# A-SHOJAEI/adverse-weather-semantic-segmentation-robustness-benchmark

Measured on AMD Instinct MI355X. Metric: images/sec (1024x2048, 5 weather conds, ensemble eval), higher is better.
Workload: dtype f32 (results float32; attention, gemm_1x1, winograd_3x3, segformer_head on 3xf16 split operands: 22-bit operands, f32 accumulate)

## Files before the change

adverse_weather_semantic_segmentation_robustness_benchmark_amd/_native.py:

```python
from __future__ import annotations

import ctypes as C
from pathlib import Path

import numpy as np
import torch

_PKG = Path(__file__).resolve().parent
LIB_PATH = _PKG / "libawseg_hip.so"

U8, I64 = 0, 1
COMBINE_WEIGHTED, COMBINE_MAXCONF, COMBINE_MEAN = 0, 1, 2
LOSS_CE, LOSS_FOCAL = 0, 1
ACT_NONE, ACT_RELU, ACT_GELU = 0, 1, 2
MAX_CLASSES = 32

c_i, c_i64, c_u64, c_f, c_d, c_p = C.c_int, C.c_int64, C.c_uint64, C.c_float, C.c_double, C.c_void_p

FOG_JOB = np.dtype([("image", "<i4"), ("_pad", "<i4"), ("beta", "<f8"), ("atmos", "<f8"), ("seed", "<u8")], align=True)
NIGHT_JOB = np.dtype([("image", "<i4"), ("_pad", "<i4"), ("brightness", "<f8"), ("intensity", "<f8"), ("seed", "<u8")], align=True)
PRIM_JOB = np.dtype([("image", "<i4"), ("prim_offset", "<i4"), ("prim_count", "<i4"), ("blur_ksize", "<i4"), ("intensity", "<f8")], align=True)
WEATHER_JOB = np.dtype([("kind", "<i4"), ("image", "<i4"), ("a", "<f8"), ("b", "<f8"), ("seed", "<u8"), ("prim_offset", "<i4"), ("prim_count", "<i4")], align=True)
WEATHER_CLEAN, WEATHER_FOG, WEATHER_RAIN, WEATHER_SNOW, WEATHER_NIGHT = 0, 1, 2, 3, 4
assert FOG_JOB.itemsize == 32 and NIGHT_JOB.itemsize == 32 and PRIM_JOB.itemsize == 24 and WEATHER_JOB.itemsize == 40

SIGNATURES = {
    "awseg_abi_version": (c_i, []),
    "awseg_header_hash": (C.c_uint64, []),
    "awseg_error_string": (C.c_char_p, [c_i]),
    "awseg_device_count": (c_i, []),
    "awseg_metrics_workspace": (c_i64, [c_i64, c_i, c_i64]),
    "awseg_confusion_accumulate": (c_i, [c_p, c_i, c_p, c_i, c_i64, c_i, c_i, c_i, c_p, c_p, c_p, c_p]),
    "awseg_argmax": (c_i, [c_p, c_i64, c_i, c_i64, c_p, c_i, c_p]),
    "awseg_combine_argmax_confusion": (c_i, [c_p, c_p, c_i64, c_i, c_i64, c_i, c_p, c_p, c_p, c_p, c_i, c_p, c_i, c_i,
                                            c_i, c_p, c_p, c_i, c_p, c_p, c_p]),
    "awseg_argmax_confusion": (c_i, [c_p, c_i64, c_i, c_i64, c_p, c_i, c_p, c_i, c_i, c_i, c_p, c_p, c_i, c_p, c_p, c_p]),
    "awseg_normalize": (c_i, [c_p, c_i64, c_i, c_i, c_p, c_i, c_p, c_p, c_p, c_p]),
    "awseg_synthetic_depth": (c_i, [c_i, c_i, c_p, c_i, c_p, c_p, c_p, c_p]),
    "awseg_conv3x3_winograd_nhwc": (c_i, [c_p, c_i, c_i, c_i, c_i, c_i, c_i, c_p, c_p, c_p, c_i, c_p, c_p, c_p, c_p]),
    "awseg_gemm_bias_act": (c_i, [c_p, c_p, c_p, c_p, c_i, c_p, c_i64, c_i, c_i, c_p, C.c_size_t, c_p]),
    "awseg_gemm_tune": (c_i, [c_p, c_p, c_p, c_i, c_i, c_p, c_i64, c_i, c_i, c_p, C.c_size_t, c_p]),
    "awseg_gemm_split_weights": (c_i, [c_p, c_i, c_i, c_p, c_p]),
    "awseg_gemm_split_weight_halfs": (c_i64, [c_i, c_i]),
    "awseg_gemm_split_bias_act": (c_i, [c_p, c_p, c_p, c_p, c_i, c_p, c_i64, c_i, c_i, c_p]),
    "awseg_gemm_bf16_weights": (c_i, [c_p, c_i, c_i, c_p, c_p]),
    "awseg_gemm_bf16_weight_halfs": (c_i64, [c_i, c_i]),
    "awseg_gemm_bf16_bias_act": (c_i, [c_p, c_p, c_p, c_p, c_i, c_p, c_i64, c_i, c_i, c_p]),
    "awseg_conv3x3_winograd_bf16_nhwc": (c_i, [c_p, c_i, c_i, c_i, c_i, c_i, c_i, c_p, c_p, c_p, c_i, c_p, c_p, c_p, c_p]),
    "awseg_attention_d32_bf16": (c_i, [c_p, c_p, c_p, c_p, c_i, c_i, c_i, c_i, c_f, c_p]),
    "awseg_attention_d32_split_workspace": (c_i64, [c_i, c_i, c_i]),
    "awseg_attention_d32_split_ws": (c_i, [c_p, c_p, c_p, c_i, c_p, c_i, c_i, c_i, c_i, c_f, c_p, c_p]),
    "awseg_attention_d32_packed_kv": (c_i, [c_p, c_p, c_p, c_i, c_i, c_i, c_i, c_f, c_i, c_p]),
    "awseg_dwconv3x3_upcat_nhwc": (c_i, [c_p, c_i, c_i, c_i, c_p, c_i, c_i64, c_i, c_i, c_p, c_p, c_p]),
    "awseg_winograd_split_weight_halfs": (c_i64, [c_i, c_i]),
    "awseg_conv3x3_winograd_split_nhwc": (c_i, [c_p, c_i, c_i, c_i, c_i, c_i, c_i, c_p, c_p, c_p, c_i, c_p, c_p, c_p, c_p]),
    "awseg_upconv_forms_floats": (c_i64, [c_i, c_i, c_i]),
    "awseg_upconv_forms": (c_i, [c_p, c_i, c_i, c_i, c_i, c_p, c_p, c_p]),
    "awseg_depth_head_fused": (c_i, [c_p, c_i, c_i, c_i, c_i, c_p, c_i, c_p, c_p, c_p, c_p, c_p]),
    "awseg_im2col_nhwc": (c_i, [c_p, c_i64, c_i, c_i, c_i, c_i, c_i, c_i, c_i, c_i, c_i, c_p, c_p]),
    "awseg_attention_d32": (c_i, [c_p, c_p, c_p, c_p, c_i, c_i, c_i, c_i, c_f, c_p]),
    "awseg_attention_d32_split": (c_i, [c_p, c_p, c_p, c_p, c_i, c_i, c_i, c_i, c_f, c_p]),
    "awseg_depth_upsample_combine": (c_i, [c_p, c_p, c_i, c_i, c_i, c_i, c_i, c_p, c_p, c_p, c_p]),
    "awseg_lut3_apply": (c_i, [c_p, c_i, c_i, c_i, c_p, c_i, c_p, c_p, c_p]),
    "awseg_local_contrast": (c_i, [c_p, c_i, c_i, c_i, c_p, c_p]),
    "awseg_depth_estimate_workspace": (C.c_size_t, [c_i]),
    "awseg_depth_estimate": (c_i, [c_p, c_i, c_i, c_i, c_p, c_p, c_p, c_p, c_p]),
    "awseg_fog_apply": (c_i, [c_p, c_i, c_i, c_p, c_i, c_p, c_p, c_p, c_p, c_p, c_p]),
    "awseg_fog_fused": (c_i, [c_p, c_i, c_i, c_p, c_i, c_p, c_p, c_p, c_p, c_p, c_p, c_p, c_p]),
    "awseg_night_apply": (c_i, [c_p, c_i, c_i, c_p, c_i, c_p, c_p, c_p, c_p, c_p, c_p, c_p]),
    "awseg_rain_apply": (c_i, [c_p, c_i, c_i, c_p, c_i, c_p, c_p, c_p, c_p, c_p, c_p, c_p]),
    "awseg_snow_apply": (c_i, [c_p, c_i, c_i, c_p, c_i, c_p, c_p, c_p, c_p, c_p, c_p, c_p]),
    "awseg_weather_batch": (c_i, [c_p, c_i, c_i, c_p, c_i, c_p, c_p, c_p, c_p, c_p, c_p, c_p, c_p, c_p, c_p]),
    "awseg_streak_workspace": (c_i64, [c_i, c_i, c_i]),
    "awseg_fog_density_field": (c_i, [c_p, c_i, c_i64, c_u64, c_p, c_p, c_p]),
    "awseg_loss_partials": (c_i64, [c_i64, c_i64]),
    "awseg_fog_ce_forward": (c_i, [c_p, c_p, c_i, c_p, c_i64, c_i, c_i64, c_i, c_f, c_p, c_p, c_p, c_p, c_p]),
    "awseg_fog_ce_backward": (c_i, [c_p, c_p, c_i, c_p, c_i64, c_i, c_i64, c_i, c_f, c_p, c_p, c_p]),
    "awseg_density_workspace": (c_i64, [c_i64, c_i64]),
    "awseg_fog_density_from_depth": (c_i, [c_p, c_i64, c_i, c_i, c_p, c_p, c_p]),
    "awseg_segformer_head_fused": (c_i, [c_p, c_i64, c_i, c_i, c_i, c_i, c_i, c_p, c_p, c_p, c_p, c_i, c_p, c_p]),
    "awseg_segformer_head_fused_split": (c_i, [c_p, c_i64, c_i, c_i, c_i, c_i, c_i, c_p, c_p, c_p, c_p, c_i, c_p, c_p]),
    "awseg_upconv3x3_bn_relu": (c_i, [c_p, c_i64, c_i, c_i, c_i, c_i, c_i, c_p, c_p, c_p, c_i, c_p]),
    "awseg_upconv3x3_linear": (c_i, [c_p, c_i64, c_i, c_i, c_i, c_i, c_i, c_p, c_p, c_i, c_p]),
    "awseg_upconv3x3_adjoint": (c_i, [c_p, c_i64, c_i, c_i, c_i, c_i, c_i, c_p, c_p]),
    "awseg_aspp_depthwise3": (c_i, [c_p, c_i64, c_i, c_i, c_i, c_p, c_i, c_i, c_i, c_p, c_p]),
    "awseg_aspp_depthwise3_mean": (c_i, [c_p, c_i64, c_i, c_i, c_i, c_p, c_i, c_i, c_i, c_p, c_p, c_p]),
    "awseg_dwconv3x3_nhwc": (c_i, [c_p, c_i64, c_i, c_i, c_i, c_i, c_p, c_p, c_i, c_p, c_p]),
    "awseg_bias_act_nhwc": (c_i, [c_p, c_i64, c_i, c_p, c_p, c_i, c_p]),
    "awseg_layernorm_rows": (c_i, [c_p, c_i64, c_i, c_p, c_p, c_f, c_p, c_p]),
    "awseg_ensemble_eval_stats": (c_i, [c_p, c_p, c_i64, c_i, c_i64, c_i, c_p, c_p, c_p, c_i, c_p, c_p, c_i, c_p, c_i, c_p, c_i,
                                       c_f, c_f, c_p, c_p]),
    "awseg_gemm_split_pieces_bias_act": (c_i, [c_p, c_i, c_i, c_p, c_p, c_p, c_i, c_p, c_i64, c_i, c_p]),
    "awseg_gemm_split_dual_bias_act": (c_i, [c_p, c_i, c_p, c_i, c_i64, c_i, c_i, c_i, c_p, c_p, c_p, c_i, c_p, c_i64, c_i, c_p]),
    "awseg_conv_gemm_split_bias_act": (c_i, [c_p, c_i64, c_i, c_i, c_i, c_i, c_i, c_i, c_i, c_i, c_p, c_p, c_p, c_i, c_p, c_i, c_p]),
    "awseg_conv_rows_gemm_split_bias_act": (c_i, [c_p, c_i64, c_i, c_i, c_i, c_i, c_i, c_i, c_i, c_p, c_p, c_p, c_i, c_p, c_i, c_p]),
    "awseg_bn_train_workspace": (c_i64, [c_i, c_i, c_i64]),
    "awseg_bn_train_stats": (c_i, [c_p, c_i, c_i, c_i64, c_p, c_p, c_p, c_p]),
    "awseg_bn_relu_dropout_forward": (c_i, [c_p, c_i, c_i, c_i64, c_p, c_p, c_p, c_p, c_p, c_p, c_p]),
    "awseg_bn_relu_dropout_backward": (c_i, [c_p, c_p, c_i, c_i, c_i64, c_p, c_p, c_p, c_p, c_p, c_p, c_p, c_p, c_p, c_i, c_p]),
    "awseg_dwconv3x3_wgrad_workspace": (c_i64, [c_i64, c_i, c_i, c_i]),
    "awseg_dwconv3x3_wgrad_nhwc": (c_i, [c_p, c_p, c_i64, c_i, c_i, c_i, c_i, c_p, c_p, c_p, c_p]),
    "awseg_mixffn_fused": (c_i, [c_p, c_i, c_i, c_i, c_i, c_p, c_p, c_f, c_p, c_i, c_p, c_p, c_p, c_p, c_i, c_p, c_p, c_p, c_p]),
    "awseg_maxpool3x3s2_nhwc": (c_i, [c_p, c_i64, c_i, c_i, c_i, c_p, c_p]),
    "awseg_maxpool3x3s2_bias_relu_nhwc": (c_i, [c_p, c_i64, c_i, c_i, c_i, c_p, c_p, c_p]),
    "awseg_upsample_bilinear": (c_i, [c_p, c_i64, c_i, c_i, c_i, c_i, c_i, c_p, c_p]),
    "awseg_stem_image": (c_i, [c_p, c_i, c_i, c_i, c_i, c_i64, c_i64, c_i64, c_p, c_i, c_p]),
    "awseg_rowdot_sigmoid": (c_i, [c_p, c_i64, c_i, c_p, c_p, c_i, c_p, c_p]),
    "awseg_aspp_pool_branch_workspace": (c_i64, [c_i, c_i]),
    "awseg_aspp_pool_branch": (c_i, [c_p, c_i, c_i, c_p, c_p, c_i, c_p, c_p, c_i, c_p, c_p, c_p]),
    "awseg_upsample_bilinear_strided": (c_i, [c_p, c_i64, c_i, c_i, c_i, c_i64, c_i64, c_i64, c_i64, c_i, c_i, c_i, c_p, c_p]),
    "awseg_combine_confusion_stats": (c_i, [c_p, c_p, c_i64, c_i, c_i64, c_i, c_p, c_p, c_p, c_i, c_i, c_i, c_p, c_p, c_i, c_p, c_p, c_i,
                                           c_p, c_i, c_p, c_i, c_f, c_f, c_p, c_p]),
    "awseg_combine_confusion_stats_pred": (c_i, [c_p, c_p, c_i64, c_i, c_i64, c_i, c_p, c_p, c_p, c_i, c_i, c_i, c_p, c_p, c_i, c_p, c_p,
                                                c_i, c_p, c_i, c_p, c_i, c_f, c_f, c_p, c_p, c_p]),
    "awseg_consistency_workspace": (c_i64, [c_i64, c_i, c_i64]),
    "awseg_prediction_consistency": (c_i, [c_p, c_p, c_i, c_i64, c_i64, c_p, c_p, c_i, c_i, c_i, c_p, c_p, c_i, c_p, c_p, c_p]),
    "awseg_ece_accumulate": (c_i, [c_p, c_i64, c_i, c_i64, c_p, c_i, c_p, c_p, c_i, c_p, c_i, c_p, c_p]),
    "awseg_temperature_grid_stats": (c_i, [c_p, c_i64, c_i, c_i64, c_p, c_i, c_p, c_p, c_i, c_p, c_i, c_p, c_i, c_p]),
    "awseg_ensemble_temperature_grid_stats": (c_i, [c_p, c_p, c_i64, c_i, c_i64, c_i, c_p, c_p, c_p, c_i, c_p, c_p, c_i, c_p, c_i,
                                                   c_p, c_i, c_p]),
    "awseg_ensemble_weight_grid_stats": (c_i, [c_p, c_p, c_i64, c_i, c_i64, c_p, c_i, c_p, c_i, c_i, c_p, c_p, c_i, c_p]),
    "awseg_depth_eval_stats": (c_i, [c_p, c_p, c_i, c_i, c_i, c_i, c_i, c_p, c_p, c_f, c_p, c_p, c_i, c_p]),
    "awseg_ensemble_failure_stats": (c_i, [c_p, c_p, c_p, c_i64, c_i, c_i64, c_i, c_p, c_p, c_p, c_i, c_p, c_p, c_i, c_p]),
    "awseg_failure_stats": (c_i, [c_p, c_i64, c_i, c_i64, c_p, c_i, c_p, c_p, c_i, c_p]),
    "awseg_boundary_workspace": (c_i64, [c_i64, c_i, c_i, c_i, c_i]),
    "awseg_boundary_stats": (c_i, [c_p, c_p, c_i, c_i, c_i64, c_i, c_i, c_i, c_p, c_i, c_p, c_p, c_i, c_p, c_p, c_p]),
    "awseg_segment_workspace": (c_i64, [c_i64, c_i, c_i]),
    "awseg_segment_stats": (c_i, [c_p, c_p, c_i, c_i, c_i64, c_i, c_i, c_i, c_p, c_i, c_p, c_p, c_p, c_i, c_p, c_p, c_p, c_p, c_p]),
    "awseg_frame_iou_workspace": (c_i64, [c_i64, c_i, c_i64]),
    "awseg_frame_iou_counts": (c_i, [c_p, c_p, c_i, c_i, c_i64, c_i64, c_i, c_p, c_p, c_i64, c_p, c_p, c_p]),
    "awseg_bootstrap_counts": (c_i, [c_p, c_p, c_i64, c_i64, c_i64, c_i64, c_u64, c_i64, c_i64, c_p, c_p, c_p]),
    "awseg_change_strata": (c_i, [c_p, c_p, c_i, c_i64, c_i, c_i64, c_p, c_p, c_p, c_i, c_p, c_p, c_p]),
    "awseg_strata_workspace": (c_i64, [c_i64, c_i, c_i64, c_i]),
    "awseg_stratified_stats": (c_i, [c_p, c_p, c_i, c_i, c_p, c_i, c_p, c_i, c_p, c_i64, c_i64, c_i, c_p, c_p, c_i, c_p, c_p, c_p]),
    "awseg_image_quality_workspace": (c_i64, [c_i64, c_i, c_i64, c_i64]),
    "awseg_image_quality": (c_i, [c_p, c_p, c_i, c_i64, c_i, c_i64, c_i64, c_p, c_p, c_p, c_p, c_f, c_f, c_p, c_p, c_i, c_p, c_p, c_p]),
}


class AwsegError(RuntimeError):
    pass


_lib = None


def lib() -> C.CDLL:
    global _lib
    if _lib is None:
        if not LIB_PATH.exists():
            raise AwsegError(
                f"{LIB_PATH} is missing: build it with `python -m "
                "adverse_weather_semantic_segmentation_robustness_benchmark_amd.csrc.build` "
                "(there is no CPU fallback for the HIP hot path)")
        handle = C.CDLL(str(LIB_PATH))
        for name, (res, args) in SIGNATURES.items():
            fn = getattr(handle, name)
            fn.restype, fn.argtypes = res, args
        header = LIB_PATH.parent.parent / "include" / "awseg.h"
        built = int(handle.awseg_header_hash())
        if built and header.exists():
            from .csrc.build import header_hash
            if built != header_hash():
                raise AwsegError(f"{LIB_PATH} was built from another include/awseg.h than the one beside it (ABI drift): rebuild it with "
                                 "`python -m adverse_weather_semantic_segmentation_robustness_benchmark_amd.csrc.build`")
        _lib = handle
    return _lib


def check(rc: int, what: str) -> None:
    if rc != 0:
        msg = lib().awseg_error_string(rc)
        raise AwsegError(f"{what} failed with code {rc}: {msg.decode() if msg else '?'}")


launch_hook = None


# ... 69 lines not shown
```

adverse_weather_semantic_segmentation_robustness_benchmark_amd/csrc/attn.hip:

```cpp
#include "awseg_common.h"

namespace {

typedef float f32x16 __attribute__((ext_vector_type(16)));

constexpr int AT = 256;
#ifndef AWSEG_ATTN_SPLIT_WAVES
#define AWSEG_ATTN_SPLIT_WAVES 2
#endif
constexpr int D = 32;
constexpr int TK = 32;
constexpr int LDK = 36;

__device__ __forceinline__ constexpr int acc_row(int r, int hk) { return (r & 3) + 8 * (r >> 2) + 4 * hk; }

__global__ __launch_bounds__(AT, 2)
void attention_d32_kernel(const float* __restrict__ q, const float* __restrict__ k, const float* __restrict__ v,
                          float* __restrict__ out, int nq, int nkv, int heads, float scale_log2e, int kvp)
{
    __shared__ float sK[2][TK * LDK];
    __shared__ float sV[2][D * LDK];
    const int tid = threadIdx.x, lane = tid & 63, wave = tid >> 6;
    const int hk = lane >> 5, li = lane & 31;
    const int h = blockIdx.y, b = blockIdx.z;
// ... 307 lines not shown
        split8_unscaled(p + 8, ph1, pl1);
        om = __builtin_amdgcn_mfma_f32_32x32x16_f16(vh0, ph0, om, 0, 0, 0);
        oc = __builtin_amdgcn_mfma_f32_32x32x16_f16(vl0, ph0, oc, 0, 0, 0);
        om = __builtin_amdgcn_mfma_f32_32x32x16_f16(vh1, ph1, om, 0, 0, 0);
        oc = __builtin_amdgcn_mfma_f32_32x32x16_f16(vl1, ph1, oc, 0, 0, 0);
        om = __builtin_amdgcn_mfma_f32_32x32x16_f16(vh0, pl0, om, 0, 0, 0);
        om = __builtin_amdgcn_mfma_f32_32x32x16_f16(vh1, pl1, om, 0, 0, 0);
        if (t + 1 < ntiles) {
            stage(buf ^ 1, kreg, vreg);
            if (t + 2 < ntiles) {
                kreg = *reinterpret_cast<const float4*>(kb + (size_t)(t + 2) * TK * kvp + g_off);
                vreg = *reinterpret_cast<const float4*>(vb + (size_t)(t + 2) * TK * kvp + g_off);
            }
        }
        __syncthreads();
    }

    if (!SCALED && !BF16) {
        if (qmax >= kSplitLimit) atomicMax(&sMax[0], __builtin_bit_cast(unsigned, qmax));
        if (kmax >= kSplitLimit) atomicMax(&sMax[1], __builtin_bit_cast(unsigned, kmax));
        if (vmax >= kSplitLimit) atomicMax(&sMax[2], __builtin_bit_cast(unsigned, vmax));
        __syncthreads();
        if ((sMax[0] | sMax[1] | sMax[2]) != 0u) return true;
    }
    const int qi = q0 + li;
    if (qi < nq) {
        const float inv = 1.0f / l_run;
        float* op = out + ((size_t)b * nq + qi) * C + h * D;
#pragma unroll
        for (int g = 0; g < 4; ++g) {
            float4 o4 = make_float4(fmaf(oc[4 * g], kLoInv, om[4 * g]) * inv, fmaf(oc[4 * g + 1], kLoInv, om[4 * g + 1]) * inv,
                                    fmaf(oc[4 * g + 2], kLoInv, om[4 * g + 2]) * inv, fmaf(oc[4 * g + 3], kLoInv, om[4 * g + 3]) * inv);
            if (SCALED) { o4.x *= sc.bv; o4.y *= sc.bv; o4.z *= sc.bv; o4.w *= sc.bv; }
            *reinterpret_cast<float4*>(op + 8 * g + 4 * hk) = o4;
        }
    }
    return false;
}

__device__ __forceinline__ int guard_exponent(unsigned maxbits)
{
    const int ex = (int)(maxbits >> 23) & 0xff;
    if (maxbits == 0u || ex == 0xff) return 0;
    return ex - 127 - 13;
}

__global__ __launch_bounds__(AT, AWSEG_ATTN_SPLIT_WAVES)
void attention_d32_split_kernel(const float* __restrict__ q, const float* __restrict__ k, const float* __restrict__ v,
                                float* __restrict__ out, int nq, int nkv, int heads, float scale_log2e, int kvp)
{
    __shared__ __attribute__((aligned(16))) _Float16 sK[2][TK * SROW];
    __shared__ __attribute__((aligned(16))) _Float16 sV[2][D * SROW];
    __shared__ unsigned sMax[3];
    if (threadIdx.x < 3) sMax[threadIdx.x] = 0u;
    const attn_scales one = {1.f, 1.f, 1.f, 1.f, 1.f, 1.f};
    if (!attn_split_pass<false>(q, k, v, out, nq, nkv, heads, scale_log2e, kvp, sK, sV, sMax, one)) return;
    const int eq = guard_exponent(sMax[0]), ek = guard_exponent(sMax[1]), ev = guard_exponent(sMax[2]);
    auto p2 = [](int e) { return __builtin_bit_cast(float, (unsigned)(127 + e) << 23); };
    const attn_scales sc = {p2(-eq), p2(-ek), p2(-ev), p2(eq), p2(ek), p2(ev)};
    attn_split_pass<true>(q, k, v, out, nq, nkv, heads, scale_log2e, kvp, sK, sV, sMax, sc);
}

constexpr int IMG_TILE_HALFS = (TK + D) * SROW;

__device__ __forceinline__ uint32_t at_lds_addr(const void* p) { return (uint32_t)(uintptr_t)(__attribute__((address_space(3))) const void*)p; }
__device__ __forceinline__ void at_dma16(__amdgpu_buffer_rsrc_t rsrc, uint32_t voff, uint32_t soff, uint32_t lds_base)
{
    asm volatile("s_mov_b32 m0, %3\n\ts_nop 0\n\tbuffer_load_dwordx4 %0, %1, %2 offen lds" : : "v"(voff), "s"(rsrc), "s"(soff), "s"(lds_base) : "m0", "memory");
}

__global__ __launch_bounds__(AT)
void attn_kv_image_kernel(const float* __restrict__ k, const float* __restrict__ v, int kvp, int nkv, int heads,
                          _Float16* __restrict__ img, int* __restrict__ exps)
{
    __shared__ unsigned sM[2];
    const int tid = threadIdx.x, h = blockIdx.x, b = blockIdx.y;
    const float* kb = k + (size_t)b * nkv * kvp + h * D;
    const float* vb = v + (size_t)b * nkv * kvp + h * D;
    const int lkey = tid >> 3, lc = tid & 7;
    const size_t g_off = (size_t)lkey * kvp + 4 * lc;
    const int wk0 = lkey * SROW + 4 * lc;
    const int wv0 = TK * SROW + (4 * lc) * SROW + pv_slot(lkey);
    const int ntiles = nkv / TK;
    if (tid < 2) sM[tid] = 0u;
    __syncthreads();
    float kmax = 0.f, vmax = 0.f;
    for (int t = 0; t < ntiles; ++t) {
        kmax = amax4(kmax, *reinterpret_cast<const float4*>(kb + (size_t)t * TK * kvp + g_off));
        vmax = amax4(vmax, *reinterpret_cast<const float4*>(vb + (size_t)t * TK * kvp + g_off));
    }
    if (kmax >= kSplitLimit) atomicMax(&sM[0], __builtin_bit_cast(unsigned, kmax));
    if (vmax >= kSplitLimit) atomicMax(&sM[1], __builtin_bit_cast(unsigned, vmax));
    __syncthreads();
    const int ek = guard_exponent(sM[0]), ev = guard_exponent(sM[1]);
    auto p2 = [](int e) { return __builtin_bit_cast(float, (unsigned)(127 + e) << 23); };
    const float sk = p2(-ek), sv = p2(-ev);
    if (tid == 0) { exps[((size_t)b * heads + h) * 2] = ek; exps[((size_t)b * heads + h) * 2 + 1] = ev; }
    _Float16* base = img + ((size_t)b * heads + h) * ntiles * IMG_TILE_HALFS;
    for (int t = 0; t < ntiles; ++t) {
        float4 kk4 = *reinterpret_cast<const float4*>(kb + (size_t)t * TK * kvp + g_off);
        float4 vv4 = *reinterpret_cast<const float4*>(vb + (size_t)t * TK * kvp + g_off);
        kk4.x *= sk; kk4.y *= sk; kk4.z *= sk; kk4.w *= sk;
        vv4.x *= sv; vv4.y *= sv; vv4.z *= sv; vv4.w *= sv;
        _Float16* T = base + (size_t)t * IMG_TILE_HALFS;
        u32x2 H, L; unsigned hh, ll;
        split_pair(kk4.x, kk4.y, hh, ll); H[0] = hh; L[0] = ll;
        split_pair(kk4.z, kk4.w, hh, ll); H[1] = hh; L[1] = ll;
        *reinterpret_cast<u32x2*>(&T[wk0]) = H;
        *reinterpret_cast<u32x2*>(&T[wk0 + 32]) = L;
        unsigned vh01, vl01, vh23, vl23;
        split_pair(vv4.x, vv4.y, vh01, vl01);
        split_pair(vv4.z, vv4.w, vh23, vl23);
        unsigned short* sv16 = reinterpret_cast<unsigned short*>(&T[wv0]);
        sv16[0] = (unsigned short)vh01;            sv16[32] = (unsigned short)vl01;
        sv16[SROW] = (unsigned short)(vh01 >> 16); sv16[SROW + 32] = (unsigned short)(vl01 >> 16);
        sv16[2 * SROW] = (unsigned short)vh23;     sv16[2 * SROW + 32] = (unsigned short)vl23;
        sv16[3 * SROW] = (unsigned short)(vh23 >> 16); sv16[3 * SROW + 32] = (unsigned short)(vl23 >> 16);
    }
}

template <bool SCALED, bool QGUARD>
__device__ __forceinline__ bool attn_split_pass_img(const float* __restrict__ q, const _Float16* __restrict__ img_bh, float* __restrict__ out,
                                                    int nq, int nkv, int heads, float scale_log2e, _Float16 (*sKV)[IMG_TILE_HALFS],
                                                    unsigned* sMax, const attn_scales sc)
{
    const int tid = threadIdx.x, lane = tid & 63, wave = tid >> 6;
    const int hk = lane >> 5, li = lane & 31;
    const int h = blockIdx.y, b = blockIdx.z;
    const int C = heads * D;
    const int q0 = blockIdx.x * 128 + wave * 32;
    float qmax = 0.f;
    h8 qh[2], ql[2];
    {
        const int qi = q0 + li;
        const float* qp = q + ((size_t)b * nq + (qi < nq ? qi : nq - 1)) * C + h * D;
        const float qs = SCALED ? scale_log2e * sc.sq : scale_log2e;
#pragma unroll
        for (int s = 0; s < 2; ++s) {
            const float4 a4 = *reinterpret_cast<const float4*>(qp + 16 * s + 8 * hk);
            const float4 b4 = *reinterpret_cast<const float4*>(qp + 16 * s + 8 * hk + 4);
            const float x[8] = { a4.x * qs, a4.y * qs, a4.z * qs, a4.w * qs, b4.x * qs, b4.y * qs, b4.z * qs, b4.w * qs };
            if (QGUARD) {
#pragma unroll
                for (int i = 0; i < 8; ++i) qmax = __builtin_fmaxf(qmax, __builtin_fabsf(x[i]));
            }
            split8(x, qh[s], ql[s]);
        }
    }
    const int ntiles = nkv / TK;
    const __amdgpu_buffer_rsrc_t rsrc = __builtin_amdgcn_make_buffer_rsrc((void*)img_bh, 0, ntiles * IMG_TILE_HALFS * 2, 0x00020000);
    const uint32_t lds0 = __builtin_amdgcn_readfirstlane(at_lds_addr(&sKV[0][0]));
    const uint32_t wave_u = __builtin_amdgcn_readfirstlane(wave);
    auto dma_tile = [&](int t, int buf) {
        const uint32_t so = (uint32_t)t * (uint32_t)(IMG_TILE_HALFS * 2), lb = lds0 + (uint32_t)buf * (uint32_t)(IMG_TILE_HALFS * 2);
        at_dma16(rsrc, (uint32_t)(lane * 16) + wave_u * 1024u, so, lb + wave_u * 1024u);
        at_dma16(rsrc, (uint32_t)(lane * 16) + (wave_u + 4u) * 1024u, so, lb + (wave_u + 4u) * 1024u);
        if (wave_u == 0) at_dma16(rsrc, (uint32_t)(lane * 16) + 8192u, so, lb + 8192u);
    };
    dma_tile(0, 0);
    asm volatile("s_waitcnt vmcnt(0)" ::: "memory");
    __syncthreads();

    f32x16 om, oc;
#pragma unroll
    for (int r = 0; r < 16; ++r) { om[r] = 0.f; oc[r] = 0.f; }
    float m_run = -1e30f, l_run = 0.f;
    const int a_off = li * SROW + 8 * hk;

    for (int t = 0; t < ntiles; ++t) {
        const int buf = t & 1;
        if (t + 1 < ntiles) dma_tile(t + 1, buf ^ 1);
        const h8* kr = reinterpret_cast<const h8*>(&sKV[buf][a_off]);
        const h8 kh0 = kr[0], kh1 = kr[2], kl0 = kr[4], kl1 = kr[6];
        f32x16 sm, scx;
#pragma unroll
        for (int r = 0; r < 16; ++r) { sm[r] = 0.f; scx[r] = 0.f; }
        sm = __builtin_amdgcn_mfma_f32_32x32x16_f16(kh0, qh[0], sm, 0, 0, 0);
        scx = __builtin_amdgcn_mfma_f32_32x32x16_f16(kh0, ql[0], scx, 0, 0, 0);
        sm = __builtin_amdgcn_mfma_f32_32x32x16_f16(kh1, qh[1], sm, 0, 0, 0);
        scx = __builtin_amdgcn_mfma_f32_32x32x16_f16(kh1, ql[1], scx, 0, 0, 0);
        scx = __builtin_amdgcn_mfma_f32_32x32x16_f16(kl0, qh[0], scx, 0, 0, 0);
        scx = __builtin_amdgcn_mfma_f32_32x32x16_f16(kl1, qh[1], scx, 0, 0, 0);
// ... 55 lines not shown
    return false;
}

__global__ __launch_bounds__(AT, AWSEG_ATTN_SPLIT_WAVES)
void attention_d32_split_img_kernel(const float* __restrict__ q, const _Float16* __restrict__ img, const int* __restrict__ exps,
                                    float* __restrict__ out, int nq, int nkv, int heads, float scale_log2e)
{
    __shared__ __attribute__((aligned(16))) _Float16 sKV[2][IMG_TILE_HALFS];
    __shared__ unsigned sMax[1];
    const int h = blockIdx.y, b = blockIdx.z;
    if (threadIdx.x == 0) sMax[0] = 0u;
    const _Float16* img_bh = img + ((size_t)b * heads + h) * (size_t)(nkv / TK) * IMG_TILE_HALFS;
    const int ek = exps[((size_t)b * heads + h) * 2], ev = exps[((size_t)b * heads + h) * 2 + 1];
    auto p2 = [](int e) { return __builtin_bit_cast(float, (unsigned)(127 + e) << 23); };
    attn_scales sc = {1.f, p2(-ek), p2(-ev), 1.f, p2(ek), p2(ev)};
    bool redo;
    if ((ek | ev) == 0) redo = attn_split_pass_img<false, true>(q, img_bh, out, nq, nkv, heads, scale_log2e, sKV, sMax, sc);
    else redo = attn_split_pass_img<true, true>(q, img_bh, out, nq, nkv, heads, scale_log2e, sKV, sMax, sc);
    if (!redo) return;
    const int eq = guard_exponent(sMax[0]);
    sc.sq = p2(-eq); sc.bq = p2(eq);
    __syncthreads();
    attn_split_pass_img<true, false>(q, img_bh, out, nq, nkv, heads, scale_log2e, sKV, sMax, sc);
}

__global__ __launch_bounds__(AT, 2)
void attention_d32_bf16_kernel(const float* __restrict__ q, const float* __restrict__ k, const float* __restrict__ v,
                               float* __restrict__ out, int nq, int nkv, int heads, float scale_log2e, int kvp)
{
    __shared__ __attribute__((aligned(16))) _Float16 sK[2][TK * SROW];
    __shared__ __attribute__((aligned(16))) _Float16 sV[2][D * SROW];
    __shared__ unsigned sMax[3];
    const attn_scales one = {1.f, 1.f, 1.f, 1.f, 1.f, 1.f};
    attn_split_pass<false, true>(q, k, v, out, nq, nkv, heads, scale_log2e, kvp, sK, sV, sMax, one);
}

}

namespace {
template <typename K>
int launch_attention(K kernel, const float* q, const float* k, const float* v, float* out, int batch, int heads,
                     int n_queries, int n_keys, float scale, awseg_stream_t stream, int kv_pitch = 0)
{
    if (batch == 0 || n_queries == 0) return 0;
    if (!q || !k || !v || !out || batch < 0 || heads < 1 || n_queries < 0 || n_keys < TK) return AWSEG_EINVAL;
    if (n_keys % TK) return AWSEG_ERANGE;
    if (heads > 65535 || batch > 65535) return AWSEG_ERANGE;
    if (((uintptr_t)q & 15) || ((uintptr_t)k & 15) || ((uintptr_t)v & 15) || ((uintptr_t)out & 15)) return AWSEG_EALIGN;
    if (kv_pitch == 0) kv_pitch = heads * D;
    if (kv_pitch < heads * D || (kv_pitch & 3)) return AWSEG_EINVAL;
    dim3 grid((unsigned)((n_queries + 127) / 128), (unsigned)heads, (unsigned)batch);
    hipLaunchKernelGGL(kernel, grid, dim3(AT), 0, awseg_s(stream), q, k, v, out, n_queries, n_keys, heads,
                       scale * 1.4426950408889634f, kv_pitch);
    AWSEG_LAUNCH_CHECK();
    return 0;
}
}

AWSEG_API int awseg_attention_d32(const float* q, const float* k, const float* v, float* out, int batch, int heads,
                                  int n_queries, int n_keys, float scale, awseg_stream_t stream)
{
    return launch_attention(attention_d32_kernel, q, k, v, out, batch, heads, n_queries, n_keys, scale, stream);
}

AWSEG_API int awseg_attention_d32_split(const float* q, const float* k, const float* v, float* out, int batch, int heads,
                                        int n_queries, int n_keys, float scale, awseg_stream_t stream)
{
    return launch_attention(attention_d32_split_kernel, q, k, v, out, batch, heads, n_queries, n_keys, scale, stream);
}

AWSEG_API int awseg_attention_d32_bf16(const float* q, const float* k, const float* v, float* out, int batch, int heads,
                                       int n_queries, int n_keys, float scale, awseg_stream_t stream)
{
    return launch_attention(attention_d32_bf16_kernel, q, k, v, out, batch, heads, n_queries, n_keys, scale, stream);
}

AWSEG_API int64_t awseg_attention_d32_split_workspace(int batch, int heads, int n_keys)
{
    if (batch < 0 || heads < 0 || n_keys < 0) return 0;
    const int64_t tab = ((int64_t)batch * heads * 2 * 4 + 255) / 256 * 256;
    return tab + (int64_t)batch * heads * (n_keys / TK) * IMG_TILE_HALFS * 2;
}

AWSEG_API int awseg_attention_d32_split_ws(const float* q, const float* k, const float* v, int kv_pitch, float* out, int batch, int heads,
                                           int n_queries, int n_keys, float scale, void* workspace, awseg_stream_t stream)
{
    if (batch == 0 || n_queries == 0) return 0;
    if (!q || !k || !v || !out || !workspace || batch < 0 || heads < 1 || n_queries < 0 || n_keys < TK) return AWSEG_EINVAL;
    if (n_keys % TK) return AWSEG_ERANGE;
    if (heads > 65535 || batch > 65535) return AWSEG_ERANGE;
    if (((uintptr_t)q & 15) || ((uintptr_t)k & 15) || ((uintptr_t)v & 15) || ((uintptr_t)out & 15) || ((uintptr_t)workspace & 255)) return AWSEG_EALIGN;
    if (kv_pitch == 0) kv_pitch = heads * D;
    if (kv_pitch < heads * D || (kv_pitch & 3)) return AWSEG_EINVAL;
    if ((int64_t)(n_keys / TK) * IMG_TILE_HALFS * 2 > 0x7fffffff) return AWSEG_ERANGE;
    int* exps = reinterpret_cast<int*>(workspace);
    const int64_t tab = ((int64_t)batch * heads * 2 * 4 + 255) / 256 * 256;
    _Float16* img = reinterpret_cast<_Float16*>(reinterpret_cast<char*>(workspace) + tab);
    hipLaunchKernelGGL(attn_kv_image_kernel, dim3((unsigned)heads, (unsigned)batch), dim3(AT), 0, awseg_s(stream), k, v, kv_pitch, n_keys, heads, img, exps);
    AWSEG_LAUNCH_CHECK();
    dim3 grid((unsigned)((n_queries + 127) / 128), (unsigned)heads, (unsigned)batch);
    hipLaunchKernelGGL(attention_d32_split_img_kernel, grid, dim3(AT), 0, awseg_s(stream), q, img, exps, out, n_queries, n_keys, heads,
                       scale * 1.4426950408889634f);
    AWSEG_LAUNCH_CHECK();
    return 0;
}

AWSEG_API int awseg_attention_d32_packed_kv(const float* q, const float* kv, float* out, int batch, int heads, int n_queries,
                                            int n_keys, float scale, int mode, awseg_stream_t stream)
{
    if (!kv) return AWSEG_EINVAL;
    const int c = heads * D;
    switch (mode) {
    case 0: return launch_attention(attention_d32_kernel, q, kv, kv + c, out, batch, heads, n_queries, n_keys, scale, stream, 2 * c);
    case 1: return launch_attention(attention_d32_split_kernel, q, kv, kv + c, out, batch, heads, n_queries, n_keys, scale, stream, 2 * c);
    case 2: return launch_attention(attention_d32_bf16_kernel, q, kv, kv + c, out, batch, heads, n_queries, n_keys, scale, stream, 2 * c);
    default: return AWSEG_EINVAL;
    }
}
```

adverse_weather_semantic_segmentation_robustness_benchmark_amd/csrc/awseg_common.h:

```cpp
#pragma once
#include <hip/hip_runtime.h>
#include <stdint.h>
#include <atomic>
#include <type_traits>
#include "../../include/awseg.h"

#define AWSEG_API extern "C" __attribute__((visibility("default")))

#define AWSEG_WAVE 64
#define AWSEG_CUS 256

#define AWSEG_LAUNCH_CHECK()                                  \
    do {                                                      \
        hipError_t e__ = hipGetLastError();                   \
        if (e__ != hipSuccess) return (int)e__;               \
    } while (0)

static inline hipStream_t awseg_s(awseg_stream_t s) { return (hipStream_t)s; }

inline int awseg_cu_count()
{
    static std::atomic<int> cached[16];
    int dev = 0, n_cu = 0;
    if (hipGetDevice(&dev) != hipSuccess) return AWSEG_CUS;
// ... 48 lines not shown

__device__ __forceinline__ void awseg_amax_step(float v, int c, float& best, int& bi)
{
    if (!(v <= best) && !(best != best)) { best = v; bi = c; }
}

__device__ __forceinline__ unsigned long long awseg_conf_q30(float conf) { return (unsigned long long)(conf * 1073741824.0f); }

__device__ __forceinline__ int awseg_ece_find_bin(float conf, const float* s_edges, int n_bins)
{
    int b = (int)ceilf(conf * (float)n_bins) - 1;
    b = b < 0 ? 0 : (b > n_bins - 1 ? n_bins - 1 : b);
    if (!(conf > s_edges[b])) b = b > 0 ? b - 1 : 0;
    else if (!(conf <= s_edges[b + 1])) b = b < n_bins - 1 ? b + 1 : b;
    if (conf > s_edges[b] && conf <= s_edges[b + 1]) return b;
    for (int k = 0; k < n_bins; ++k)
        if (conf > s_edges[k] && conf <= s_edges[k + 1]) return k;
    return -1;
}

inline int awseg_blocks_per_image(int64_t lane_items, int threads, int64_t batch, int resident_per_cu)
{
    int64_t want = (lane_items + threads - 1) / threads;
    int64_t cap = (AWSEG_CUS * resident_per_cu + batch - 1) / batch;
    if (cap < 1) cap = 1;
    if (want > cap) want = cap;
    if (want < 1) want = 1;
    return (int)want;
}

template <typename F> inline auto awseg_by_label(int label_dtype, F&& f)
{
    if (label_dtype == AWSEG_U8) return f(std::integral_constant<int, AWSEG_U8>());
    return f(std::integral_constant<int, AWSEG_I64>());
}
template <typename F> inline auto awseg_by_flag(bool flag, F&& f)
{
    if (flag) return f(std::true_type());
    return f(std::false_type());
}
template <typename F> inline auto awseg_by_combine_mode(int mode, F&& f)
{
    if (mode == AWSEG_COMBINE_WEIGHTED) return f(std::integral_constant<int, 0>());
    return f(std::integral_constant<int, 2>());
}

struct awseg_philox {
    __device__ __forceinline__ static void gen(uint64_t seed, uint64_t ctr, uint32_t stream, uint32_t out[4])
    {
        const uint32_t M0 = 0xD2511F53u, M1 = 0xCD9E8D57u;
        uint32_t c0 = (uint32_t)ctr, c1 = (uint32_t)(ctr >> 32), c2 = stream, c3 = 0x9E3779B9u;
        uint32_t k0 = (uint32_t)seed, k1 = (uint32_t)(seed >> 32);
#pragma unroll
        for (int r = 0; r < 7; ++r) {
            uint32_t hi0 = __umulhi(M0, c0), lo0 = M0 * c0;
            uint32_t hi1 = __umulhi(M1, c2), lo1 = M1 * c2;
            uint32_t n0 = hi1 ^ c1 ^ k0, n2 = hi0 ^ c3 ^ k1;
            c0 = n0; c1 = lo1; c2 = n2; c3 = lo0;
            k0 += 0x9E3779B9u; k1 += 0xBB67AE85u;
        }
        out[0] = c0; out[1] = c1; out[2] = c2; out[3] = c3;
    }
};
__device__ __forceinline__ void awseg_box_muller(uint32_t a, uint32_t b, float& n0, float& n1)
{
    float u1 = ((float)(a >> 8) + 0.5f) * (1.0f / 16777216.0f);
    float u2 = (float)(b >> 8) * (1.0f / 16777216.0f);
    float r = __builtin_amdgcn_sqrtf(-1.38629436111989061883f * __builtin_amdgcn_logf(u1));
    n0 = r * __builtin_amdgcn_cosf(u2);
    n1 = r * __builtin_amdgcn_sinf(u2);
}
__device__ __forceinline__ void awseg_box_muller16(uint32_t a, float& n0, float& n1)
{
    float u1 = ((float)(a & 0xFFFFu) + 0.5f) * (1.0f / 65536.0f);
    float u2 = (float)(a >> 16) * (1.0f / 65536.0f);
    float r = __builtin_amdgcn_sqrtf(-1.38629436111989061883f * __builtin_amdgcn_logf(u1));
    n0 = r * __builtin_amdgcn_cosf(u2);
    n1 = r * __builtin_amdgcn_sinf(u2);
}
__device__ __forceinline__ float awseg_u01(uint32_t a) { return (float)(a >> 8) * (1.0f / 16777216.0f); }

int awseg_gemm_split3_weights(const float* w, int n, int k, uint16_t* w3, const unsigned* trailer, hipStream_t stream);
bool awseg_gemm_split3_eligible(int64_t m, int n, int k, const void* x, const void* out, const void* residual, const void* bias);
struct awseg_g3_dual { const float* x2; int k1; int h, w, stride, ho, wo; int64_t bytes; const float* x3 = nullptr; const float* x4 = nullptr; };
int awseg_gemm_split3_launch(const float* x, const uint16_t* w3, const unsigned* trailer, const float* bias, const float* residual,
                             int act, float* out, int64_t m, int n, int k, int cus, hipStream_t stream, const int* conv = nullptr,
                             bool bf16 = false, const awseg_g3_dual* dual = nullptr);
int awseg_gemm_split3_bn(int n);
int64_t awseg_gemm_split3_image_rows(int n);
int awseg_gemm_bf16_3_weights(const float* w, int n, int k, uint16_t* w3, hipStream_t stream);
```

adverse_weather_semantic_segmentation_robustness_benchmark_amd/csrc/gemm_split.hip:

```cpp
#include "awseg_common.h"

namespace {

typedef float f32x16 __attribute__((ext_vector_type(16)));
typedef _Float16 h8 __attribute__((ext_vector_type(8)));
typedef _Float16 h2 __attribute__((ext_vector_type(2)));
typedef unsigned u32x2 __attribute__((ext_vector_type(2)));
typedef unsigned u32x4 __attribute__((ext_vector_type(4)));

constexpr int GT = 512;
constexpr int SWT = 256;
constexpr int GKT = 32;
constexpr int GROW = 72;
constexpr float kLoScale = 2048.0f, kLoInv = 1.0f / 2048.0f;

__device__ __forceinline__ void split_pair(float a, float b, unsigned& hi, unsigned& lo)
{
    const auto hp = __builtin_amdgcn_cvt_pkrtz(a, b);
    const h2 hh = __builtin_bit_cast(h2, hp);
    const float ra = (a - (float)hh.x) * kLoScale, rb = (b - (float)hh.y) * kLoScale;
    hi = __builtin_bit_cast(unsigned, hp);
    lo = __builtin_bit_cast(unsigned, __builtin_amdgcn_cvt_pkrtz(ra, rb));
}

// ... 296 lines not shown
        const bool rescale = oe != 0;

        {
            const int64_t tile_off = m0 * a.N + n0;
            const int64_t rem = ((int64_t)a.M * a.N - tile_off) * 4;
            const int nrec = rem > 0x7fffffff ? 0x7fffffff : (int)rem;
            const __amdgpu_buffer_rsrc_t o_rsrc = __builtin_amdgcn_make_buffer_rsrc((void*)(a.out + tile_off), 0, nrec, 0x00020000);
            const __amdgpu_buffer_rsrc_t r_rsrc = __builtin_amdgcn_make_buffer_rsrc((void*)((a.residual ? a.residual : a.out) + tile_off), 0, nrec, 0x00020000);
            const bool has_res = a.residual != nullptr;
            const bool ragged = m0 + BM > a.M;
            const int mleft = ragged ? (int)(a.M - m0) : BM;
            const int vrow = (wm * 32 * MT + 4 * hk) * a.N;
#pragma unroll
            for (int j = 0; j < NT; ++j) {
                const int nl = wn * 32 * NT + j * 32 + li;
                const bool n_ok = n0 + nl < a.N;
                const float bv = (a.bias && n_ok) ? a.bias[n0 + nl] : 0.f;
                const int voff = n_ok ? (vrow + nl) * 4 : (int)0x80000000;
#pragma unroll
                for (int i = 0; i < MT; ++i) {
#pragma unroll
                    for (int half = 0; half < 2; ++half) {
                        float rv[8]; int vo[8], so[8];
#pragma unroll
                        for (int r8 = 0; r8 < 8; ++r8) {
                            const int r = 8 * half + r8;
                            const int rowc = i * 32 + (r & 3) + 8 * (r >> 2);
                            if (ragged) {
                                vo[r8] = (wm * 32 * MT + 4 * hk + rowc < mleft) ? voff + rowc * a.N * 4 : (int)0x80000000;
                                so[r8] = 0;
                            } else { vo[r8] = voff; so[r8] = rowc * a.N * 4; }
                            rv[r8] = has_res ? __builtin_bit_cast(float, __builtin_amdgcn_raw_buffer_load_b32(r_rsrc, vo[r8], so[r8], 0)) : 0.f;
                        }
#pragma unroll
                        for (int r8 = 0; r8 < 8; ++r8) {
                            const int r = 8 * half + r8;
                            float vv = fmaf(ac2[i][j][r], kLoInv, am[i][j][r]);
                            if (rescale) vv = vv * os1 * os2;
                            vv = vv + bv + rv[r8];
                            if (a.act == 1) vv = fmaxf(vv, 0.f);
                            __builtin_amdgcn_raw_buffer_store_b32(__builtin_bit_cast(uint32_t, vv), o_rsrc, vo[r8], so[r8], 0);
                        }
                    }
                }
            }
        }
        if (!has_next) break;
        slot = nslot; m0 = nm0; n0 = nn0;
        scaled = false; sx = 1.0f; xe = 0;
    }
}

}

AWSEG_API int awseg_gemm_split_weights(const float* w, int n, int k, uint16_t* w_split, awseg_stream_t stream)
{
    if (n == 0 || k == 0) return 0;
    if (!w || !w_split || n < 0 || k < 0) return AWSEG_EINVAL;
    const int64_t ne = (int64_t)n * k;
    const int64_t blocks = (ne / 2 + SWT) / SWT;
    unsigned* trailer = reinterpret_cast<unsigned*>(w_split + 2 * ne);
    if ((uintptr_t)trailer & 3) return AWSEG_EALIGN;
    hipError_t e = hipMemsetAsync(trailer, 0, 16, awseg_s(stream));
    if (e != hipSuccess) return (int)e;
    const int64_t rb = (ne + SWT - 1) / SWT;
    hipLaunchKernelGGL(weights_absmax_kernel, dim3((unsigned)(rb < 1024 ? rb : 1024)), dim3(SWT), 0, awseg_s(stream), w, ne, trailer);
    AWSEG_LAUNCH_CHECK();
    hipLaunchKernelGGL(split_weights_kernel, dim3((unsigned)blocks), dim3(SWT), 0, awseg_s(stream), w, ne, w_split, trailer);
    AWSEG_LAUNCH_CHECK();
    if (awseg_gemm_split3_bn(n) && k % 8 == 0) return awseg_gemm_split3_weights(w, n, k, w_split + 2 * ne + 8, trailer, awseg_s(stream));
    return 0;
}

AWSEG_API int64_t awseg_gemm_split_weight_halfs(int n, int k)
{
    if (n < 1 || k < 1) return -1;
    const int64_t ne = (int64_t)n * k;
    return 2 * ne + 8 + ((awseg_gemm_split3_bn(n) && k % 8 == 0) ? 2 * awseg_gemm_split3_image_rows(n) * ((k + 31) / 32 * 32) : 0);
}

namespace {
struct conv_desc { int H, W, C, Ho, Wo, kw, stride, pad, dil; int64_t batch; int pitch = 0, padx = -1; };

int gemm_launch(bool bf16, const float* x, const uint16_t* w_split, const float* bias, const float* residual,
                int act, float* out, int64_t m, int n, int k, awseg_stream_t stream, const conv_desc* cv = nullptr)
{
    if (m == 0 || n == 0) return 0;
    if (!x || !w_split || !out || m < 0 || n < 0 || k < 8 || act < 0 || act > 1) return AWSEG_EINVAL;
    if (k % 8) return AWSEG_ERANGE;
    if (((uintptr_t)x & 15) || ((uintptr_t)w_split & 15)) return AWSEG_EALIGN;
    gemm_args a;
    a.x = x; a.wh = reinterpret_cast<const _Float16*>(w_split); a.wl = a.wh + (int64_t)n * k;
    a.trailer = reinterpret_cast<const unsigned*>(w_split + 2 * (int64_t)n * k);
    a.bias = bias; a.residual = residual; a.out = out; a.M = m; a.N = n; a.K = k; a.act = act;
    a.conv = cv ? 1 : 0;
    if (cv) { a.cH = cv->H; a.cW = cv->W; a.cC = cv->C; a.cHo = cv->Ho; a.cWo = cv->Wo; a.ckw = cv->kw; a.cs = cv->stride; a.cp = cv->pad; a.cd = cv->dil; }
    else { a.cH = a.cW = a.cC = a.cHo = a.cWo = a.ckw = a.cs = 1; a.cp = 0; a.cd = 1; }
    const int cus = awseg_cu_count();
    if (awseg_gemm_split3_eligible(m, n, k, cv ? nullptr : x, out, residual, bias) && !(bf16 && (cv || n % 256)) &&
        (!cv || (cv->C % 32 == 0 && (int64_t)cv->batch * cv->H * cv->W * (cv->pitch > 0 ? cv->pitch : cv->C) * 4 <= 0x7fffffff)) &&
        (((m + 255) / 256) * (int64_t)((n + awseg_gemm_split3_bn(n) - 1) / awseg_gemm_split3_bn(n)) >= (int64_t)cus / 2 ||
         (!bf16 && ((m + 127) / 128) * (int64_t)((n + 127) / 128) >= (int64_t)cus / 2))) {
        const int cdesc[12] = { cv ? cv->H : 0, cv ? cv->W : 0, cv ? cv->C : 0, cv ? cv->Ho : 0, cv ? cv->Wo : 0, cv ? cv->kw : 0,
                                cv ? cv->stride : 0, cv ? cv->pad : 0, cv ? cv->dil : 0, cv ? (int)cv->batch : 0, cv ? cv->pitch : 0, cv ? cv->padx : -1 };
        return awseg_gemm_split3_launch(x, w_split + 2 * (int64_t)n * k + 8, a.trailer, bias, residual, act, out, m, n, k, cus, awseg_s(stream),
                                        cv ? cdesc : nullptr, bf16);
    }
    if (cv && cv->pitch > 0) return AWSEG_ERANGE;
    const bool wide = n % 256 == 0 && ((m + 127) / 128) * (int64_t)(n / 256) >= cus;
    const int bn = wide ? 256 : 128, bm = 128;
    const int64_t ntm = (m + bm - 1) / bm;
    a.ntn = (n + bn - 1) / bn;
    const int64_t ntm8 = (ntm + 7) / 8 * 8;
    if (ntm8 * a.ntn > 0x7fffffff || (int64_t)bm * n > 0x7fffffff) return AWSEG_ERANGE;
    a.ntm = (int)ntm; a.ntm8 = (int)ntm8;
    const int64_t slots = ntm8 * a.ntn;
    int64_t blocks = (int64_t)cus * (wide ? 1 : 2) / 8 * 8;
    if (blocks < 8) blocks = 8;
    if (blocks > slots) blocks = slots;
    const dim3 grid((unsigned)blocks), block(GT);
#define GEMM_GO(MT_, NT_, WM_, WN_)                                                                                    \
    do {                                                                                                              \
        if (bf16) {                                                                                                   \
            if (k % GKT) hipLaunchKernelGGL((gemm_split_kernel<MT_, NT_, WM_, WN_, true, true>), grid, block, 0, awseg_s(stream), a);   \
            else hipLaunchKernelGGL((gemm_split_kernel<MT_, NT_, WM_, WN_, false, true>), grid, block, 0, awseg_s(stream), a);         \
        } else {                                                                                                      \
            if (k % GKT) hipLaunchKernelGGL((gemm_split_kernel<MT_, NT_, WM_, WN_, true, false>), grid, block, 0, awseg_s(stream), a);  \
            else hipLaunchKernelGGL((gemm_split_kernel<MT_, NT_, WM_, WN_, false, false>), grid, block, 0, awseg_s(stream), a);        \
        }                                                                                                             \
    } while (0)
    if (wide) GEMM_GO(2, 2, 2, 4); else GEMM_GO(1, 2, 4, 2);
#undef GEMM_GO
    AWSEG_LAUNCH_CHECK();
    return 0;
}

__global__ __launch_bounds__(SWT)
void bf16_weights_kernel(const float* __restrict__ w, int64_t n_elems, uint16_t* __restrict__ out, unsigned* __restrict__ trailer)
{
    if (blockIdx.x == 0 && threadIdx.x == 0) { trailer[0] = 0u; trailer[1] = 0u; trailer[2] = 0u; trailer[3] = 0u; }
    const int64_t i = ((int64_t)blockIdx.x * SWT + threadIdx.x) * 2;
    if (i >= n_elems) return;
    const unsigned p = pack_bf16(w[i], (i + 1 < n_elems) ? w[i + 1] : 0.f);
    out[i] = (uint16_t)p;
    if (i + 1 < n_elems) out[i + 1] = (uint16_t)(p >> 16);
}
}

AWSEG_API int awseg_gemm_split_bias_act(const float* x, const uint16_t* w_split, const float* bias, const float* residual,
                                        int act, float* out, int64_t m, int n, int k, awseg_stream_t stream)
{
    return gemm_launch(false, x, w_split, bias, residual, act, out, m, n, k, stream);
}

AWSEG_API int awseg_gemm_split_dual_bias_act(const float* x, int k1, const float* x2, int k2, int64_t batch, int x2_height, int x2_width,
                                             int x2_stride, const uint16_t* w_split, const float* bias, const float* residual, int act,
                                             float* out, int64_t m, int n, awseg_stream_t stream)
{
    if (m == 0 || n == 0) return 0;
    if (!x || !x2 || !w_split || !out || m < 0 || n < 0 || k1 < 32 || k2 < 32 || act < 0 || act > 1 || x2_stride < 0) return AWSEG_EINVAL;
    if (k1 % 32 || k2 % 32) return AWSEG_ERANGE;
    if (((uintptr_t)x & 15) || ((uintptr_t)x2 & 15) || ((uintptr_t)w_split & 15)) return AWSEG_EALIGN;
    const int k = k1 + k2;
    if (!awseg_gemm_split3_eligible(m, n, k, x, out, residual, bias)) return AWSEG_ERANGE;
    awseg_g3_dual d;
    d.x2 = x2; d.k1 = k1; d.stride = x2_stride; d.h = d.w = d.ho = d.wo = 1;
    if (x2_stride > 0) {
        if (batch < 1 || x2_height < 1 || x2_width < 1) return AWSEG_EINVAL;
        d.h = x2_height; d.w = x2_width; d.ho = (x2_height - 1) / x2_stride + 1; d.wo = (x2_width - 1) / x2_stride + 1;
        if (batch * d.ho * d.wo != m) return AWSEG_EINVAL;
        d.bytes = batch * (int64_t)x2_height * x2_width * k2 * 4;
    } else {
        d.bytes = m * (int64_t)k2 * 4;
    }
    if (d.bytes > 0x7fffffff) return AWSEG_ERANGE;
    return awseg_gemm_split3_launch(x, w_split + 2 * (int64_t)n * k + 8, reinterpret_cast<const unsigned*>(w_split + 2 * (int64_t)n * k), bias, residual,
                                    act, out, m, n, k, awseg_cu_count(), awseg_s(stream), nullptr, false, &d);
}

AWSEG_API int awseg_gemm_split_pieces_bias_act(const float* const* pieces, int n_pieces, int k_piece, const uint16_t* w_split, const float* bias,
                                               const float* residual, int act, float* out, int64_t m, int n, awseg_stream_t stream)
{
    if (m == 0 || n == 0) return 0;
    if (!pieces || n_pieces < 2 || n_pieces > 4 || !w_split || !out || m < 0 || n < 0 || k_piece < 32 || act < 0 || act > 1) return AWSEG_EINVAL;
    if (k_piece % 32) return AWSEG_ERANGE;
    for (int i = 0; i < n_pieces; ++i) {
        if (!pieces[i]) return AWSEG_EINVAL;
        if ((uintptr_t)pieces[i] & 15) return AWSEG_EALIGN;
    }
    if ((uintptr_t)w_split & 15) return AWSEG_EALIGN;
    const int k = n_pieces * k_piece;
    if (!awseg_gemm_split3_eligible(m, n, k, pieces[0], out, residual, bias)) return AWSEG_ERANGE;
    awseg_g3_dual d;
    d.x2 = pieces[1]; d.k1 = k_piece; d.stride = 0; d.h = d.w = d.ho = d.wo = 1;
    d.bytes = m * (int64_t)k_piece * 4;
    d.x3 = n_pieces > 2 ? pieces[2] : nullptr; d.x4 = n_pieces > 3 ? pieces[3] : nullptr;
    if (d.bytes > 0x7fffffff) return AWSEG_ERANGE;
    return awseg_gemm_split3_launch(pieces[0], w_split + 2 * (int64_t)n * k + 8, reinterpret_cast<const unsigned*>(w_split + 2 * (int64_t)n * k), bias, residual,
                                    act, out, m, n, k, awseg_cu_count(), awseg_s(stream), nullptr, false, &d);
}

AWSEG_API int awseg_conv_gemm_split_bias_act(const float* x, int64_t batch, int height, int width, int channels, int kernel_h,
                                             int kernel_w, int stride, int pad, int dilation, const uint16_t* w_split,
                                             const float* bias, const float* residual, int act, float* out, int n,
                                             awseg_stream_t stream)
{
    if (batch == 0) return 0;
    if (batch < 0 || height < 1 || width < 1 || channels < 32 || kernel_h < 1 || kernel_w < 1 || stride < 1 || pad < 0 || dilation < 1) return AWSEG_EINVAL;
    if (channels % 32) return AWSEG_ERANGE;
    const int ho = (height + 2 * pad - dilation * (kernel_h - 1) - 1) / stride + 1;
    const int wo = (width + 2 * pad - dilation * (kernel_w - 1) - 1) / stride + 1;
    if (ho < 1 || wo < 1) return AWSEG_ERANGE;
    const int64_t k = (int64_t)kernel_h * kernel_w * channels;
    if (k > 0x7fffffff || batch * height > 0x7fffffff) return AWSEG_ERANGE;
    const conv_desc cv = { height, width, channels, ho, wo, kernel_w, stride, pad, dilation, batch };
    return gemm_launch(false, x, w_split, bias, residual, act, out, batch * ho * wo, n, (int)k, stream, &cv);
}

AWSEG_API int awseg_conv_rows_gemm_split_bias_act(const float* x, int64_t batch, int height, int width_padded, int pixel_floats,
                                                  int kernel_h, int stride, int pad_y, int out_width, const uint16_t* w_split,
                                                  const float* bias, const float* residual, int act, float* out, int n,
                                                  awseg_stream_t stream)
{
    if (batch == 0) return 0;
    if (batch < 0 || height < 1 || width_padded < 8 || kernel_h < 1 || stride < 1 || pad_y < 0 || out_width < 1) return AWSEG_EINVAL;
    if (pixel_floats < 4 || pixel_floats % 4 || 32 % pixel_floats) return AWSEG_ERANGE;
    if ((int64_t)(out_width - 1) * stride * pixel_floats + 32 > (int64_t)width_padded * pixel_floats) return AWSEG_ERANGE;
    const int ho = (height + 2 * pad_y - kernel_h) / stride + 1;
    if (ho < 1 || batch * height > 0x7fffffff) return AWSEG_ERANGE;
    conv_desc cv = { height, width_padded, 32, ho, out_width, 1, stride, pad_y, 1, batch };
    cv.pitch = pixel_floats; cv.padx = 0;
    return gemm_launch(false, x, w_split, bias, residual, act, out, batch * ho * out_width, n, kernel_h * 32, stream, &cv);
}

AWSEG_API int awseg_gemm_bf16_weights(const float* w, int n, int k, uint16_t* w_bf16, awseg_stream_t stream)
{
    if (n == 0 || k == 0) return 0;
    if (!w || !w_bf16 || n < 0 || k < 0) return AWSEG_EINVAL;
    const int64_t ne = (int64_t)n * k;
    unsigned* trailer = reinterpret_cast<unsigned*>(w_bf16 + 2 * ne);
    if ((uintptr_t)trailer & 3) return AWSEG_EALIGN;
    hipLaunchKernelGGL(bf16_weights_kernel, dim3((unsigned)((ne / 2 + SWT) / SWT)), dim3(SWT), 0, awseg_s(stream), w, ne, w_bf16, trailer);
    AWSEG_LAUNCH_CHECK();
    if (n % 64 == 0 && k % 8 == 0) return awseg_gemm_bf16_3_weights(w, n, k, w_bf16 + 2 * ne + 8, awseg_s(stream));
    return 0;
}

AWSEG_API int64_t awseg_gemm_bf16_weight_halfs(int n, int k)
{
    if (n < 1 || k < 1) return -1;
    const int64_t ne = (int64_t)n * k;
    return 2 * ne + 8 + ((n % 64 == 0 && k % 8 == 0) ? (int64_t)n * ((k + 31) / 32 * 32) : 0);
}

AWSEG_API int awseg_gemm_bf16_bias_act(const float* x, const uint16_t* w_bf16, const float* bias, const float* residual,
                                       int act, float* out, int64_t m, int n, int k, awseg_stream_t stream)
{
    return gemm_launch(true, x, w_bf16, bias, residual, act, out, m, n, k, stream);
}
```

adverse_weather_semantic_segmentation_robustness_benchmark_amd/csrc/gemm_split3.hip:

```cpp
#include "awseg_common.h"

namespace {

typedef float f32x16 __attribute__((ext_vector_type(16)));
typedef float f32x4 __attribute__((ext_vector_type(4)));
typedef _Float16 h8 __attribute__((ext_vector_type(8)));
typedef unsigned u32x4 __attribute__((ext_vector_type(4)));

constexpr int G3M_MAX = 256, G3K = 32;
constexpr int g3_lds(int wv, int nt) { return 2 * (32 * wv * 128) + 2 * (wv == 8 ? 32 * wv * 128 : 32 * nt * 128) + 64; }
constexpr float kActScale0 = 16.0f;
constexpr int kActExp0 = -4;
constexpr float kSplitLimit3 = 2048.0f;
constexpr float kSmallLimit3 = 0.0078125f;

__device__ __forceinline__ float pow2f3(int e) { return __builtin_bit_cast(float, (unsigned)(127 + e) << 23); }

__device__ __forceinline__ uint32_t lds_addr3(const void* p)
{
    return (uint32_t)(uintptr_t)(__attribute__((address_space(3))) const void*)p;
}
__device__ __forceinline__ void dma16(__amdgpu_buffer_rsrc_t rsrc, uint32_t voff, uint32_t soff, uint32_t lds_base)
{
    asm volatile("s_mov_b32 m0, %3\n\ts_nop 0\n\tbuffer_load_dwordx4 %0, %1, %2 offen lds" : : "v"(voff), "s"(rsrc), "s"(soff), "s"(lds_base) : "m0", "memory");
}

__device__ __forceinline__ void split2(float a, float b, float s, unsigned& hi, unsigned& lo)
{
    asm("v_fma_mixlo_f16 %0, %2, %4, 0\n\t"
        "v_fma_mixhi_f16 %0, %3, %4, 0\n\t"
        "v_fma_mixlo_f16 %1, %2, %4, -%0 op_sel_hi:[0,0,1]\n\t"
        "v_fma_mixhi_f16 %1, %3, %4, -%0 op_sel:[0,0,1] op_sel_hi:[0,0,1]\n\t"
        "s_nop 1"
        : "=&v"(hi), "=&v"(lo) : "v"(a), "v"(b), "s"(s));
}

#ifdef AWSEG_G3_STAMP
__device__ unsigned long long g_g3_stamp[2][8];
#define G3_T(v) const unsigned long long v = __builtin_readcyclecounter()
#else
#define G3_T(v)
#endif

struct g3_args {
    const float* x; const uint16_t* w3; const float* bias; const float* residual; float* out;
    const unsigned* trailer;
    int64_t M; int N, K, act, ntm, ntm8, ntn;
    int img_bn;
    int cH, cW, cC, cHo, cWo, ckw, cs, cp, cd;
    int cpitch, cpx;
    int64_t x_bytes;
    const float* x2; int K1, x2H, x2W, x2s, x2Ho, x2Wo;
    int64_t x2_bytes;
    const float* x3; const float* x4; int K2;
};

typedef __bf16 bf8_3 __attribute__((ext_vector_type(8)));
typedef __bf16 bf2_3 __attribute__((ext_vector_type(2)));
typedef float f2_3 __attribute__((ext_vector_type(2)));
__device__ __forceinline__ unsigned pack_bf16_3(float x, float y) { return __builtin_bit_cast(unsigned, __builtin_convertvector(f2_3{x, y}, bf2_3)); }

template <bool CONV, int = 0, bool BF16 = false, int NT = 8, int WV = 8, bool DUAL = false>
__global__ __launch_bounds__(64 * WV, 2)
void gemm_split3_kernel(g3_args a)
{
    static_assert(NT <= WV, "a weight stage must fit an activation stage");
    static_assert(!DUAL || (!CONV && !BF16), "two A sources: the plain split-operand form only");
    constexpr int G3M = 32 * WV, G3_STAGE = G3M * 128, G3_A0 = 0, G3_B0 = 2 * G3_STAGE;
    constexpr int G3_BSTAGE = WV == 8 ? G3_STAGE : 32 * NT * 128;
    constexpr int BN = 32 * NT;
    constexpr int ROWB = BF16 ? 64 : 128;
    constexpr int NBI_ALL = BN * ROWB / 1024;
    constexpr int NBI = NBI_ALL >= WV ? NBI_ALL / WV : 1;
    extern __shared__ __attribute__((aligned(16))) unsigned char smem[];
    unsigned* sMax = reinterpret_cast<unsigned*>(smem + 2 * G3_STAGE + 2 * G3_BSTAGE);
    const int tid = threadIdx.x, lane = tid & 63, wave = tid >> 6;
    const int hk = lane >> 5, li = lane & 31;
    const int K = a.K, nkt = (K + G3K - 1) / G3K, kb = nkt;
    const int ktail = K % G3K;
    const int ntiles = a.ntm8 * a.ntn;

    auto tile_of = [&](int slot, int64_t& m0, int& n0) -> bool {
        const int xcd = slot & 7, jj = slot >> 3;
        const int nt_i = jj % a.ntn, mt_i = (jj / a.ntn) * 8 + xcd;
        m0 = (int64_t)mt_i * G3M; n0 = nt_i * BN;
        return mt_i < a.ntm;
    };

    const int rl = lane >> 3, sl = lane & 7;
    uint32_t a_voff[4], a_voff_last[4], b_voff[4];
    uint32_t a_voff2[4];
    const int KA = DUAL ? a.K1 : a.K;
    const int kt1 = KA / G3K;
    int cby[4], cy0[4], cx0[4];
    const uint32_t lds0 = __builtin_amdgcn_readfirstlane(lds_addr3(smem));
    const uint32_t wave_u = __builtin_amdgcn_readfirstlane(wave);
    __amdgpu_buffer_rsrc_t x_rsrc, w_rsrc, x2_rsrc, x3_rsrc, x4_rsrc;
    auto point = [&](int64_t m0, int n0) {
        const int64_t rows_left = a.M - m0;
        const int64_t xbytes = rows_left * (int64_t)KA * 4;
        if (CONV) x_rsrc = __builtin_amdgcn_make_buffer_rsrc((void*)a.x, 0, (int)a.x_bytes, 0x00020000);
        else x_rsrc = __builtin_amdgcn_make_buffer_rsrc((void*)(a.x + m0 * KA), 0, (int)(xbytes > 0x7fffffff ? 0x7fffffff : xbytes), 0x00020000);
        if (DUAL) {
            x2_rsrc = __builtin_amdgcn_make_buffer_rsrc((void*)a.x2, 0, (int)a.x2_bytes, 0x00020000);
            x3_rsrc = __builtin_amdgcn_make_buffer_rsrc((void*)(a.x3 ? a.x3 : a.x2), 0, (int)a.x2_bytes, 0x00020000);
            x4_rsrc = __builtin_amdgcn_make_buffer_rsrc((void*)(a.x4 ? a.x4 : a.x2), 0, (int)a.x2_bytes, 0x00020000);
        }
        const int IB = a.img_bn, nr = n0 % IB;
        w_rsrc = __builtin_amdgcn_make_buffer_rsrc((void*)(a.w3 + ((int64_t)(n0 - nr) * kb + nr) * (ROWB / 2)), 0, (IB * kb - nr) * ROWB, 0x00020000);
#pragma unroll
        for (int j = 0; j < 4; ++j) {
            const int row = 8 * (4 * wave + j) + rl;
            const int c = sl ^ ((row >> 1) & 7);
            a_voff[j] = (uint32_t)(row * KA * 4 + c * 16);
            a_voff_last[j] = (ktail == 0 || c * 4 < ktail) ? a_voff[j] : 0x80000000u;
            if (DUAL) {
                const int64_t m = m0 + row;
                const int k2 = a.K2;
                int64_t pix = m;
                if (a.x2s > 0) {
                    const int b = (int)(m / ((int64_t)a.x2Ho * a.x2Wo));
                    const int rem = (int)(m - (int64_t)b * a.x2Ho * a.x2Wo);
                    const int oy = rem / a.x2Wo, ox = rem - oy * a.x2Wo;
                    pix = ((int64_t)b * a.x2H + oy * a.x2s) * a.x2W + ox * a.x2s;
                }
                a_voff2[j] = m < a.M ? (uint32_t)(pix * k2 * 4 + c * 16) : 0x80000000u;
            }
            {
                const int qi = wave * NBI + j;
                if (BF16) {
                    const int brow = 16 * qi + (lane >> 2);
                    b_voff[j] = (uint32_t)(brow * 64 + (((lane & 3) ^ ((brow >> 2) & 3)) * 16));
                } else {
                    const int brow = 8 * qi + rl;
                    b_voff[j] = (uint32_t)(brow * 128 + ((sl ^ ((brow >> 1) & 7)) * 16));
                }
            }
            if (CONV) {
                a_voff[j] = (uint32_t)(c * 16);
                const int64_t m = m0 + row;
                const int b = (int)(m / ((int64_t)a.cHo * a.cWo));
                const int rem = (int)(m - (int64_t)b * a.cHo * a.cWo);
                const int oy = rem / a.cWo, ox = rem - oy * a.cWo;
                cby[j] = m < a.M ? b * a.cH : -1; cy0[j] = oy * a.cs - a.cp; cx0[j] = ox * a.cs - a.cpx;
            }
        }
    };
    auto issue = [&](int kt, int stage) {
        const uint32_t la = lds0 + (uint32_t)(G3_A0 + stage * G3_STAGE) + wave_u * 4096u;
        if (CONV) {
            const int k0 = kt * G3K, tap = k0 / a.cC, c0 = k0 - tap * a.cC;
            const int ky = tap / a.ckw, kx = tap - ky * a.ckw;
#pragma unroll
            for (int j = 0; j < 4; ++j) {
                const int iy = cy0[j] + ky * a.cd, ix = cx0[j] + kx * a.cd;
                const bool ok = cby[j] >= 0 && (unsigned)iy < (unsigned)a.cH && (unsigned)ix < (unsigned)a.cW;
                const uint32_t vo = ok ? (uint32_t)((((cby[j] + iy) * a.cW + ix) * a.cpitch + c0) * 4) + a_voff[j] : 0x80000000u;
                dma16(x_rsrc, vo, 0u, la + (uint32_t)(j * 1024));
            }
        } else {
        if (DUAL && kt >= kt1) {
            const int kt2 = a.K2 / G3K;
            const int piece = __builtin_amdgcn_readfirstlane((kt - kt1) / kt2);
            const uint32_t ko = (uint32_t)__builtin_amdgcn_readfirstlane(((kt - kt1) - piece * kt2) * 128);
            if (piece == 0) {
#pragma unroll
                for (int j = 0; j < 4; ++j) dma16(x2_rsrc, a_voff2[j], ko, la + (uint32_t)(j * 1024));
            } else if (piece == 1) {
#pragma unroll
                for (int j = 0; j < 4; ++j) dma16(x3_rsrc, a_voff2[j], ko, la + (uint32_t)(j * 1024));
            } else {
#pragma unroll
                for (int j = 0; j < 4; ++j) dma16(x4_rsrc, a_voff2[j], ko, la + (uint32_t)(j * 1024));
            }
        } else {
#pragma unroll
            for (int j = 0; j < 4; ++j) dma16(x_rsrc, kt == nkt - 1 ? a_voff_last[j] : a_voff[j], (uint32_t)(kt * 128), la + (uint32_t)(j * 1024));
        }
        }
        {
            const uint32_t lbw = lds0 + (uint32_t)(G3_B0 + stage * G3_BSTAGE) + wave_u * (uint32_t)(NBI * 1024);
            if (NBI_ALL >= WV || (int)wave_u < NBI_ALL) {
#pragma unroll
                for (int j = 0; j < NBI; ++j) dma16(w_rsrc, b_voff[j], (uint32_t)(kt * a.img_bn * ROWB), lbw + (uint32_t)(j * 1024));
            }
        }
    };

    const int sw = (li >> 1) & 7;
    int fa[2][2], fb[2][2];
#pragma unroll
    for (int ks = 0; ks < 2; ++ks) {
#pragma unroll
        for (int e = 0; e < 2; ++e) fa[ks][e] = G3_A0 + (wave * 32 + li) * 128 + (((4 * ks + 2 * hk + e) ^ sw) * 16);
        fb[ks][0] = BF16 ? G3_B0 + li * 64 + (((2 * ks + hk) ^ ((li >> 2) & 3)) * 16) : G3_B0 + li * 128 + (((2 * ks + hk) ^ sw) * 16);
        fb[ks][1] = G3_B0 + li * 128 + (((4 + 2 * ks + hk) ^ sw) * 16);
    }

    int slot = blockIdx.x;
    int64_t m0 = 0; int n0 = 0;
    while (slot < ntiles && !tile_of(slot, m0, n0)) slot += gridDim.x;
    if (slot >= ntiles) return;
    if (tid < 4) sMax[tid] = 0u;
    int par = 0;
    const int we = (int)a.trailer[1];
    float amax = 0.f, sx = kActScale0;
    int xe = kActExp0;
    bool scaled = false;
    bool stores_pending = false;
    int g = 0;
#ifdef AWSEG_G3_STAMP
    unsigned long long g3s[6] = {0, 0, 0, 0, 0, 0};
    G3_T(sb0);
#endif
    point(m0, n0);
    issue(0, 0);

    while (true) {
        int nslot = slot + gridDim.x;
        int64_t nm0 = 0; int nn0 = 0;
        while (nslot < ntiles && !tile_of(nslot, nm0, nn0)) nslot += gridDim.x;
        const bool has_next = nslot < ntiles;

        f32x16 acc[NT];
#pragma unroll
        for (int j = 0; j < NT; ++j)
#pragma unroll
            for (int r = 0; r < 16; ++r) acc[j][r] = 0.f;
        amax = 0.f;

        for (int t = 0; t < nkt; ++t, ++g) {
            const int st = g & 1;
            G3_T(s0);
            if (t == 0 && stores_pending) asm volatile("s_waitcnt vmcnt(%0)" : : "n"(16 * NT < 63 ? 16 * NT : 63) : "memory");
            else asm volatile("s_waitcnt vmcnt(0)" ::: "memory");
            __builtin_amdgcn_s_barrier();
            const bool issue_late = wave_u >= 4;
            G3_T(s1);
            if (t + 1 < nkt && !issue_late) issue(t + 1, st ^ 1);
            G3_T(s2);
            if (t == 0 && tid == 0) { sMax[par ^ 1] = 0u; sMax[2 + (par ^ 1)] = 0u; }
            const unsigned char* sa = smem + st * G3_STAGE;
            const unsigned char* sbw = smem + st * G3_BSTAGE;
#pragma unroll
            for (int ks = 0; ks < 2; ++ks) {
#ifdef AWSEG_G3_STAMP
                if (ks == 1) { G3_T(s3); g3s[2] += s3 - s2; g3s[5] = s3; }
#endif
                if (ks == 1 && t + 1 < nkt && issue_late) issue(t + 1, st ^ 1);
                const f32x4 p = *reinterpret_cast<const f32x4*>(sa + fa[ks][0]);
                const f32x4 q = *reinterpret_cast<const f32x4*>(sa + fa[ks][1]);
                h8 Bh[NT], Bl[NT];
#pragma unroll
                for (int j = 0; j < NT; ++j) {
                    if (BF16) { Bh[j] = *reinterpret_cast<const h8*>(sbw + fb[ks][0] + j * 2048); Bl[j] = Bh[j]; continue; }
                    Bh[j] = *reinterpret_cast<const h8*>(sbw + fb[ks][0] + j * 4096);
                    Bl[j] = *reinterpret_cast<const h8*>(sbw + fb[ks][1] + j * 4096);
                }
                u32x4 H, L; unsigned h, l;
                if (BF16) {
                    H[0] = pack_bf16_3(p[0], p[1]); H[1] = pack_bf16_3(p[2], p[3]); H[2] = pack_bf16_3(q[0], q[1]); H[3] = pack_bf16_3(q[2], q[3]);
                    const bf8_3 Ab = __builtin_bit_cast(bf8_3, H);
#pragma unroll
                    for (int j = 0; j < NT; ++j) acc[j] = __builtin_amdgcn_mfma_f32_32x32x16_bf16(Ab, __builtin_bit_cast(bf8_3, Bh[j]), acc[j], 0, 0, 0);
                    continue;
                }
                amax = __builtin_fmaxf(__builtin_fmaxf(amax, __builtin_fabsf(p[0])), __builtin_fabsf(p[1]));
                amax = __builtin_fmaxf(__builtin_fmaxf(amax, __builtin_fabsf(p[2])), __builtin_fabsf(p[3]));
                amax = __builtin_fmaxf(__builtin_fmaxf(amax, __builtin_fabsf(q[0])), __builtin_fabsf(q[1]));
                amax = __builtin_fmaxf(__builtin_fmaxf(amax, __builtin_fabsf(q[2])), __builtin_fabsf(q[3]));
                split2(p[0], p[1], sx, h, l); H[0] = h; L[0] = l;
                split2(p[2], p[3], sx, h, l); H[1] = h; L[1] = l;
                split2(q[0], q[1], sx, h, l); H[2] = h; L[2] = l;
                split2(q[2], q[3], sx, h, l); H[3] = h; L[3] = l;
                const h8 Ah = __builtin_bit_cast(h8, H), Al = __builtin_bit_cast(h8, L);
#pragma unroll
                for (int j = 0; j < NT; ++j) {
                    acc[j] = __builtin_amdgcn_mfma_f32_32x32x16_f16(Ah, Bh[j], acc[j], 0, 0, 0);
                    acc[j] = __builtin_amdgcn_mfma_f32_32x32x16_f16(Ah, Bl[j], acc[j], 0, 0, 0);
                    acc[j] = __builtin_amdgcn_mfma_f32_32x32x16_f16(Al, Bh[j], acc[j], 0, 0, 0);
                }
            }
#ifdef AWSEG_G3_STAMP
            { G3_T(s4); g3s[0] += s1 - s0; g3s[1] += s2 - s1; g3s[3] += s4 - g3s[5]; g3s[4] += 1; }
#endif
        }

        if (!BF16 && !scaled) {
            const bool not_small = __ballot(amax >= kSmallLimit3) != 0ull;
            if (amax >= kSplitLimit3 || !not_small) atomicMax(&sMax[par], __builtin_bit_cast(unsigned, amax));
            if (not_small && (tid & 63) == 0) sMax[2 + par] = 1u;
        }
        asm volatile("s_waitcnt lgkmcnt(0)" ::: "memory");
        __builtin_amdgcn_s_barrier();
        const unsigned mx = sMax[par];
        const bool small = !BF16 && sMax[2 + par] == 0u;
        par ^= 1;
        bool again = false;
        constexpr unsigned kBig = __builtin_bit_cast(unsigned, kSplitLimit3), kSmall = __builtin_bit_cast(unsigned, kSmallLimit3);
        if (!scaled && (mx >= kBig || (small && mx >= 0x00800000u && mx < kSmall))) {
            const int ex = (int)(mx >> 23) & 0xff;
            if (ex != 0xff) {
                xe = ex - 127 - 13;
                xe = xe < -127 ? -127 : xe;
                sx = pow2f3(-xe);
                scaled = true; again = true;
            }
        }
        if (again) {
            stores_pending = false;
            issue(0, g & 1);
            continue;
        }
        const int64_t em0 = m0; const int en0 = n0;
        if (has_next) { point(nm0, nn0); issue(0, g & 1); }

        const int oe = BF16 ? 0 : we + xe;
        const int oe1 = oe / 2, oe2 = oe - oe1;
        const float os1 = pow2f3(oe1 < -126 ? -126 : (oe1 > 127 ? 127 : oe1)), os2 = pow2f3(oe2 < -126 ? -126 : (oe2 > 127 ? 127 : oe2));

        {
            const int64_t tile_off = em0 * a.N + en0;
            const int64_t rem = ((int64_t)a.M * a.N - tile_off) * 4;
            const int nrec = rem > 0x7fffffff ? 0x7fffffff : (int)rem;
            const __amdgpu_buffer_rsrc_t o_rsrc = __builtin_amdgcn_make_buffer_rsrc((void*)(a.out + tile_off), 0, nrec, 0x00020000);
            const __amdgpu_buffer_rsrc_t r_rsrc = __builtin_amdgcn_make_buffer_rsrc((void*)((a.residual ? a.residual : a.out) + tile_off), 0, a.residual ? nrec : 0, 0x00020000);
            const int ncols = a.N - en0 < BN ? a.N - en0 : BN;
            const __amdgpu_buffer_rsrc_t b_rsrc = __builtin_amdgcn_make_buffer_rsrc((void*)((a.bias ? a.bias : a.out) + en0), 0, a.bias ? ncols * 4 : 0, 0x00020000);
            const int voff = ((wave * 32 + 4 * hk) * a.N + li) * 4;
            int vcol[NT];
#pragma unroll
            for (int j = 0; j < NT; ++j) vcol[j] = j * 32 + li < ncols ? voff + j * 128 : (int)0x80000000;
            const float relu_floor = a.act == 1 ? 0.f : -__builtin_inff();
            const int rowb = a.N * 4;
            const bool has_res = a.residual != nullptr;
            float bv[NT], bld[NT];
#pragma unroll
            for (int j = 0; j < NT; ++j) bld[j] = __builtin_bit_cast(float, __builtin_amdgcn_raw_buffer_load_b32(b_rsrc, (j * 32 + li) * 4, 0, 0));
#pragma unroll
            for (int j = 0; j < NT; ++j) asm volatile("v_mov_b32 %0, %1" : "=v"(bv[j]) : "v"(bld[j]));
            auto res_load = [&](int g, float (&rv)[8]) {
                const int j = g >> 1, half = g & 1;
#pragma unroll
                for (int r8 = 0; r8 < 8; ++r8) {
                    const int r = 8 * half + r8, rowc = (r & 3) + 8 * (r >> 2);
                    rv[r8] = __builtin_bit_cast(float, __builtin_amdgcn_raw_buffer_load_b32(r_rsrc, vcol[j], rowc * rowb, 0));
                }
            };
            auto group_store = [&](int g, const float (&rv)[8], bool with_res) {
                const int j = g >> 1, half = g & 1;
#pragma unroll
                for (int r8 = 0; r8 < 8; ++r8) {
                    const int r = 8 * half + r8, rowc = (r & 3) + 8 * (r >> 2);
                    float vv = acc[j][r] * os1 * os2;
                    vv = vv + bv[j];
                    if (with_res) vv = vv + rv[r8];
                    vv = __builtin_fmaxf(vv, relu_floor);
                    __builtin_amdgcn_raw_buffer_store_b32(__builtin_bit_cast(uint32_t, vv), o_rsrc, vcol[j], rowc * rowb, 0);
                }
            };
            if (has_res) {
                float rva[8], rvb[8];
                res_load(0, rva);
#pragma unroll
                for (int g = 0; g < 2 * NT; g += 2) {
                    res_load(g + 1, rvb);
                    group_store(g, rva, true);
                    if (g + 2 < 2 * NT) res_load(g + 2, rva);
                    group_store(g + 1, rvb, true);
                }
            } else {
                const float none[8] = {0.f, 0.f, 0.f, 0.f, 0.f, 0.f, 0.f, 0.f};
#pragma unroll
                for (int g = 0; g < 2 * NT; ++g) group_store(g, none, false);
            }
        }
        if (!has_next) break;
        stores_pending = true;
        slot = nslot; m0 = nm0; n0 = nn0;
        scaled = false; sx = kActScale0; xe = kActExp0;
    }
    asm volatile("s_waitcnt vmcnt(0)" ::: "memory");
#ifdef AWSEG_G3_STAMP
    if (blockIdx.x == 0 && (tid == 0 || tid == 256)) {
        G3_T(sb1);
        for (int i = 0; i < 5; ++i) g_g3_stamp[tid >> 8][i] += g3s[i];
        g_g3_stamp[tid >> 8][5] += sb1 - sb0;
    }
#endif
}

__global__ __launch_bounds__(256)
void split3_weights_kernel(const float* __restrict__ w, int n_rows, int k_dim, int kb, int bn, uint16_t* __restrict__ out, const unsigned* __restrict__ trailer)
{
    const int e = (int)trailer[1];
    const int e1 = e / 2, e2 = e - e1;
    const float s1 = pow2f3(-e1), s2 = pow2f3(-e2);
    const int64_t i = ((int64_t)blockIdx.x * 256 + threadIdx.x) * 2;
    const int kp = kb * 32;
    if (i >= (int64_t)n_rows * kp) return;
    const int64_t n = i / kp;
    const int k = (int)(i - n * kp);
    const float x0 = k < k_dim ? w[n * k_dim + k] * s1 * s2 : 0.f, x1 = k + 1 < k_dim ? w[n * k_dim + k + 1] * s1 * s2 : 0.f;
    const _Float16 h0 = (_Float16)x0, h1 = (_Float16)x1;
    const _Float16 l0 = (_Float16)(x0 - (float)h0), l1 = (_Float16)(x1 - (float)h1);
    uint16_t* d = out + (((n / bn) * kb + (k >> 5)) * bn + (n % bn)) * 64 + (k & 31);
    d[0] = __builtin_bit_cast(uint16_t, h0); d[1] = __builtin_bit_cast(uint16_t, h1);
    d[32] = __builtin_bit_cast(uint16_t, l0); d[33] = __builtin_bit_cast(uint16_t, l1);
}

__global__ __launch_bounds__(256)
void bf16_3_weights_kernel(const float* __restrict__ w, int n_rows, int k_dim, int kb, int bn, uint16_t* __restrict__ out)
{
    const int64_t i = ((int64_t)blockIdx.x * 256 + threadIdx.x) * 2;
    const int kp = kb * 32;
    if (i >= (int64_t)n_rows * kp) return;
    const int64_t n = i / kp;
    const int k = (int)(i - n * kp);
    const unsigned pr = pack_bf16_3(k < k_dim ? w[n * k_dim + k] : 0.f, k + 1 < k_dim ? w[n * k_dim + k + 1] : 0.f);
    uint16_t* d = out + (((n / bn) * kb + (k >> 5)) * bn + (n % bn)) * 32 + (k & 31);
    d[0] = (uint16_t)pr; d[1] = (uint16_t)(pr >> 16);
}

}

int awseg_gemm_split3_bn(int n) { return n % 256 == 0 ? 256 : (n % 128 == 0 ? 128 : (n >= 8 ? 64 : 0)); }
int64_t awseg_gemm_split3_image_rows(int n) { const int bn = awseg_gemm_split3_bn(n); return bn ? (int64_t)(n + bn - 1) / bn * bn : 0; }

int awseg_gemm_bf16_3_weights(const float* w, int n, int k, uint16_t* w3, hipStream_t stream)
{
    const int kb = (k + 31) / 32;
    const int64_t ne = (int64_t)n * kb * 32;
    hipLaunchKernelGGL(bf16_3_weights_kernel, dim3((unsigned)((ne / 2 + 255) / 256)), dim3(256), 0, stream, w, n, k, kb, awseg_gemm_split3_bn(n), w3);
    AWSEG_LAUNCH_CHECK();
    return 0;
}

int awseg_gemm_split3_weights(const float* w, int n, int k, uint16_t* w3, const unsigned* trailer, hipStream_t stream)
{
    const int kb = (k + 31) / 32;
    const int64_t ne = (int64_t)n * kb * 32;
    const int64_t rows = awseg_gemm_split3_image_rows(n);
    if (rows != n) {
        hipError_t e = hipMemsetAsync(w3, 0, (size_t)rows * kb * 32 * 2 * sizeof(uint16_t), stream);
        if (e != hipSuccess) return (int)e;
    }
    hipLaunchKernelGGL(split3_weights_kernel, dim3((unsigned)((ne / 2 + 255) / 256)), dim3(256), 0, stream, w, n, k, kb, awseg_gemm_split3_bn(n), w3, trailer);
    AWSEG_LAUNCH_CHECK();
    return 0;
}

bool awseg_gemm_split3_eligible(int64_t m, int n, int k, const void* x, const void* out, const void* residual, const void* bias)
{
    if (awseg_gemm_split3_bn(n) == 0 || k % 8 || k < 32 || m < 1) return false;
    if (((uintptr_t)x | (uintptr_t)out | (uintptr_t)residual | (uintptr_t)bias) & 15) return false;
    if ((int64_t)G3M_MAX * n * 4 > 0x7fffffff || (int64_t)G3M_MAX * (k + 32) * 4 > 0x7fffffff) return false;
    return true;
}

int awseg_gemm_split3_launch(const float* x, const uint16_t* w3, const unsigned* trailer, const float* bias, const float* residual,
                             int act, float* out, int64_t m, int n, int k, int cus, hipStream_t stream, const int* conv, bool bf16,
                             const awseg_g3_dual* dual)
{
    g3_args a;
    a.x2 = nullptr; a.K1 = k; a.x2H = a.x2W = a.x2Ho = a.x2Wo = 1; a.x2s = 0; a.x2_bytes = 0; a.x3 = a.x4 = nullptr; a.K2 = 0;
    if (dual) {
        const int pieces = 1 + (dual->x3 ? 1 : 0) + (dual->x4 ? 1 : 0);
        if (conv || bf16 || dual->k1 % G3K || dual->k1 < G3K || (k - dual->k1) % pieces || dual->bytes > 0x7fffffff) return AWSEG_ERANGE;
        const int k2 = (k - dual->k1) / pieces;
        if (k2 % G3K || k2 < G3K || (pieces > 1 && dual->stride > 0) || (dual->x4 && !dual->x3)) return AWSEG_ERANGE;
        a.x2 = dual->x2; a.K1 = dual->k1; a.x2H = dual->h; a.x2W = dual->w; a.x2s = dual->stride; a.x2Ho = dual->ho; a.x2Wo = dual->wo;
        a.x2_bytes = dual->bytes; a.x3 = dual->x3; a.x4 = dual->x4; a.K2 = k2;
    }
    a.cH = a.cW = a.cC = a.cHo = a.cWo = a.ckw = a.cs = 1; a.cp = 0; a.cd = 1; a.x_bytes = 0; a.cpitch = 1; a.cpx = 0;
    if (conv) {
        a.cH = conv[0]; a.cW = conv[1]; a.cC = conv[2]; a.cHo = conv[3]; a.cWo = conv[4]; a.ckw = conv[5]; a.cs = conv[6]; a.cp = conv[7]; a.cd = conv[8];
        a.cpitch = conv[10] > 0 ? conv[10] : a.cC; a.cpx = conv[11] >= 0 ? conv[11] : a.cp;
        a.x_bytes = (int64_t)conv[9] * a.cH * a.cW * a.cpitch * 4;
        if (a.cC % G3K || a.x_bytes > 0x7fffffff) return AWSEG_ERANGE;
    }
    a.x = x; a.w3 = w3; a.bias = bias; a.residual = residual; a.out = out; a.trailer = trailer;
    a.M = m; a.N = n; a.K = k; a.act = act;
    const int img_bn = awseg_gemm_split3_bn(n);
    a.img_bn = img_bn;
    const int bn_half = img_bn >= 128 ? 128 : 64;
    const bool few = ((m + 255) / 256) * (int64_t)((n + img_bn - 1) / img_bn) < (int64_t)cus;
    const bool half = !bf16 && (few || ((k <= 128 || (img_bn <= 128 && k <= 512)) &&
                                        ((m + 127) / 128) * (int64_t)((n + bn_half - 1) / bn_half) >= 4 * (int64_t)cus));
    const int rows = half ? 128 : 256;
    const int bn = half ? bn_half : img_bn;
    const int64_t ntm = (m + rows - 1) / rows;
    a.ntn = (n + bn - 1) / bn;
    const int64_t ntm8 = (ntm + 7) / 8 * 8;
    if (ntm8 * a.ntn > 0x7fffffff) return AWSEG_ERANGE;
    a.ntm = (int)ntm; a.ntm8 = (int)ntm8;
    const int64_t slots = ntm8 * a.ntn;
    int64_t blocks = (int64_t)cus * (half ? (bn == 64 ? 3 : 2) : 1) / 8 * 8;
    if (blocks < 8) blocks = 8;
    if (blocks > slots) blocks = slots;
#define G3_GO(CONV_, BF_, NT_, WV_, DUAL_)                                                                                             \
    do {                                                                                                                              \
        auto kf = gemm_split3_kernel<CONV_, 0, BF_, NT_, WV_, DUAL_>;                                                                 \
        hipError_t e = hipFuncSetAttribute(reinterpret_cast<const void*>(kf), hipFuncAttributeMaxDynamicSharedMemorySize, g3_lds(WV_, NT_)); \
        if (e != hipSuccess) return (int)e;                                                                                           \
        hipLaunchKernelGGL(kf, dim3((unsigned)blocks), dim3(64 * WV_), g3_lds(WV_, NT_), stream, a);                                   \
    } while (0)
#define G3_BY_NT(CONV_, BF_, DUAL_) do { if (bn == 256) G3_GO(CONV_, BF_, 8, 8, DUAL_); else if (bn == 128) G3_GO(CONV_, BF_, 4, 8, DUAL_); else G3_GO(CONV_, BF_, 2, 8, DUAL_); } while (0)
#define G3_HALF(CONV_, DUAL_) do { if (bn == 128) G3_GO(CONV_, false, 4, 4, DUAL_); else G3_GO(CONV_, false, 2, 4, DUAL_); } while (0)
    if (dual) { if (half) G3_HALF(false, true); else G3_BY_NT(false, false, true); }
    else if (bf16) G3_BY_NT(false, true, false);
    else if (half && conv) G3_HALF(true, false);
    else if (half) G3_HALF(false, false);
    else if (conv) G3_BY_NT(true, false, false);
    else G3_BY_NT(false, false, false);
#undef G3_HALF
#undef G3_BY_NT
#undef G3_GO
    AWSEG_LAUNCH_CHECK();
    return 0;
}

#ifdef AWSEG_G3_STAMP
AWSEG_API int awseg_debug_g3_stamps(unsigned long long* out16, int reset)
{
    hipError_t e = hipMemcpyFromSymbol(out16, HIP_SYMBOL(g_g3_stamp), sizeof(unsigned long long) * 16);
    if (e == hipSuccess && reset) { unsigned long long z[16] = {}; e = hipMemcpyToSymbol(HIP_SYMBOL(g_g3_stamp), z, sizeof z); }
    return (int)e;
}
#endif
```

adverse_weather_semantic_segmentation_robustness_benchmark_amd/models/deeplab.py:

```python
from __future__ import annotations

import os

from typing import List

import torch
import torch.nn as nn
import torch.nn.functional as F

from .. import ops


class Conv2d(nn.Conv2d):

    linear_in_training = True
    keep_channels_last = os.environ.get("AWSEG_TRAIN_KEEP_CL", "1") != "0"
    matmul_nchw = os.environ.get("AWSEG_TRAIN_MATMUL_NCHW", "1") != "0"

    def forward(self, x: torch.Tensor) -> torch.Tensor:
        if (Conv2d.linear_in_training and x.is_cuda and torch.is_grad_enabled() and self.kernel_size == (1, 1) and self.groups == 1
                and self.padding == (0, 0) and x.dim() == 4 and x.shape[2] * x.shape[3] > 1):
            if self.stride != (1, 1):
                x = x[:, :, ::self.stride[0], ::self.stride[1]]
            b, c, h, w = x.shape
# ... 141 lines not shown
        mods += [ASPPSeparableConv(in_ch, out_ch, r) for r in self.rates]
        mods.append(ASPPPooling(in_ch, out_ch))
        self.convs = nn.ModuleList(mods)
        self.project = nn.Sequential(Conv2d(5 * out_ch, out_ch, 1, bias=False), nn.BatchNorm2d(out_ch), nn.ReLU(),
                                     nn.Dropout(0.5))

    def forward(self, x):
        return self.project(torch.cat([conv(x) for conv in self.convs], dim=1))


def _bn_fold(bn: nn.BatchNorm2d):
    inv = torch.rsqrt(bn.running_var + bn.eps)
    scale = bn.weight * inv
    return scale, bn.bias - bn.running_mean * scale


class DeepLabV3PlusDecoder(nn.Module):
    def __init__(self, encoder_channels, out_channels=256, atrous_rates=(12, 24, 36), output_stride=16):
        super().__init__()
        self.out_channels = out_channels
        self.aspp = nn.Sequential(ASPP(encoder_channels[-1], out_channels, atrous_rates),
                                  SeparableConv2d(out_channels, out_channels, 3, padding=1, bias=False),
                                  nn.BatchNorm2d(out_channels), nn.ReLU())
        self.up = nn.UpsamplingBilinear2d(scale_factor=2 if output_stride == 8 else 4)
        self.block1 = nn.Sequential(Conv2d(encoder_channels[-4], 48, 1, bias=False), nn.BatchNorm2d(48), nn.ReLU())
        self.block2 = nn.Sequential(SeparableConv2d(48 + out_channels, out_channels, 3, padding=1, bias=False),
                                    nn.BatchNorm2d(out_channels), nn.ReLU())

    def forward(self, *features):
        a = self.up(self.aspp(features[-1]))
        hi = self.block1(features[-4])
        return self.block2(torch.cat([a, hi], dim=1))

    @torch.no_grad()
    def aspp_fused(self, x: torch.Tensor) -> torch.Tensor:
        aspp: ASPP = self.aspp[0]
        B, Cin, h, w = x.shape
        xl = x.permute(0, 2, 3, 1).contiguous()
        flat = xl.view(B * h * w, Cin)
        Cout = self.out_channels
        P = aspp.project[0].weight.view(Cout, 5 * Cout)

        def branch(inp, wmat, bn):
            from . import fused
            want = ops.gemm_wants_split(inp.shape[0], wmat.shape[0], wmat.shape[1])

            def fold():
                s, b = _bn_fold(bn)
                wf = (wmat * s[:, None]).contiguous()
                return wf, b.contiguous(), (ops.gemm_split_weights(wf) if want else None)
            wf, b, ws = fused.cached(bn, "aspp_fold%d" % int(want), (wmat, bn.weight, bn.bias, bn.running_mean, bn.running_var), fold)
            return ops.gemm_bias_act(inp, wf, b, 1, w_split=ws)

        pbn = aspp.project[1]

        def fold_proj():
            ps, pb = _bn_fold(pbn)
            Pf = (P * ps[:, None]).contiguous()
            parts = [Pf[:, i * Cout:(i + 1) * Cout].contiguous() for i in range(5)]
            want = ops.gemm_wants_split(B * h * w, Cout, Cout)
            return parts, [ops.gemm_split_weights(pp) if want else None for pp in parts[:4]], torch.zeros(Cout, device=P.device), pb.contiguous()
        from . import fused
        parts, psplit, zero_bias, pb = fused.cached(aspp.project[0], "proj_fold%d" % int(ops.gemm_wants_split(B * h * w, Cout, Cout)),
                                                (aspp.project[0].weight, pbn.weight, pbn.bias, pbn.running_mean, pbn.running_var), fold_proj)
        dws = [aspp.convs[1 + r][0][0].weight for r in range(3)]
        wdw = fused.cached(aspp, "dw3taps", dws, lambda: torch.stack([t_.view(Cin, 9).t() for t_ in dws]).contiguous())
        if xl.is_cuda and xl.dtype == torch.float32:
            dw, gmean = ops.aspp_depthwise3_mean(xl, wdw, aspp.rates)
        else:
            dw, gmean = ops.aspp_depthwise3(xl, wdw, aspp.rates), None
        dw = dw.view(3, B * h * w, Cin)
        if gmean is None:
            gmean = xl.mean(dim=(1, 2))
        pool = aspp.convs[4]
        pw_, pbn_ = pool[1].weight.view(Cout, Cin), pool[2]
        if xl.is_cuda and xl.dtype == torch.float32:
            def fold_pool():
                s_, b_ = _bn_fold(pbn_)
                return (pw_ * s_[:, None]).contiguous(), b_.contiguous()
            w1f, b1f = fused.cached(pbn_, "aspp_pool_fold", (pw_, pbn_.weight, pbn_.bias, pbn_.running_mean, pbn_.running_var), fold_pool)
            g2 = ops.aspp_pool_branch(gmean, w1f, b1f, parts[4], pb)
        else:
            g2 = branch(gmean, pw_, pbn_) @ parts[4].t() + pb
        acc = g2[:, None, :].expand(B, h * w, Cout).contiguous().view(B * h * w, Cout)
        ys = [branch(flat, aspp.convs[0][0].weight.view(Cout, Cin), aspp.convs[0][1])]
        for r in range(3):
            mod = aspp.convs[1 + r]
            ys.append(branch(dw[r], mod[0][1].weight.view(Cout, Cin), mod[1]))
        done = None
        if ops.ASPP_PIECES and ops.GEMM_SPLIT and ops.PRECISION != "bf16" and acc.is_cuda and Cout % 32 == 0:
            wcat = fused.cached(aspp.project[0], "proj_pieces", (parts[0], parts[1], parts[2], parts[3]),
                                lambda: ops.gemm_split_weights(torch.cat(parts[:4], dim=1).contiguous()))
            done = ops.gemm_split_pieces(ys, wcat, zero_bias, 1, residual=acc, out=acc)
        if done is None:
            for i, y in enumerate(ys):
                ops.gemm_bias_act(y, parts[i], zero_bias, 1 if i == 3 else 0, residual=acc, out=acc, w_split=psplit[i])
        out = acc
        return out.view(B, h, w, Cout).permute(0, 3, 1, 2)

    @torch.no_grad()
    def forward_fused(self, *features):
        from . import fused
        from .. import _native as N
        a = self.aspp_fused(features[-1])
        a = fused.separable_bn_relu(a, self.aspp[1], self.aspp[2])
        hi = fused.conv_bn_act(features[-4], self.block1[0], self.block1[1], N.ACT_RELU)
        dwc, pwc = self.block2[0][0], self.block2[0][1]
        d = ops.dwconv3x3_upcat(fused.nhwc_view(a), fused.nhwc_view(hi), fused.dw_taps(dwc))
        B, H4, W4, Cc = d.shape
        w, shift = fused.folded_conv_bn(pwc, self.block2[1])
        w2 = w.view(w.shape[0], Cc)
        y = ops.gemm_bias_act(d.view(B * H4 * W4, Cc), w2, shift, N.ACT_RELU, w_split=fused.split_weights(pwc, w2, B * H4 * W4))
        return y.view(B, H4, W4, -1).permute(0, 3, 1, 2)


class SegmentationHead(nn.Sequential):
    def __init__(self, in_ch, out_ch, kernel_size=1, upsampling=4):
        super().__init__(Conv2d(in_ch, out_ch, kernel_size, padding=kernel_size // 2),
                         nn.UpsamplingBilinear2d(scale_factor=upsampling) if upsampling > 1 else nn.Identity(),
                         nn.Identity())


class DeepLabV3Plus(nn.Module):

    def __init__(self, encoder_name="resnet50", classes=19, encoder_output_stride=16, decoder_channels=256,
                 decoder_atrous_rates=(12, 24, 36), upsampling=4):
        super().__init__()
        self.encoder = ResNetEncoder(encoder_name, encoder_output_stride)
        self.decoder = DeepLabV3PlusDecoder(self.encoder.out_channels, decoder_channels, decoder_atrous_rates,
                                            encoder_output_stride)
        self.segmentation_head = SegmentationHead(decoder_channels, classes, 1, upsampling)
        for m in list(self.decoder.modules()) + list(self.segmentation_head.modules()):
            if isinstance(m, nn.Conv2d):
                nn.init.kaiming_uniform_(m.weight, mode="fan_in", nonlinearity="relu")
                if m.bias is not None:
                    nn.init.constant_(m.bias, 0)
            elif isinstance(m, nn.BatchNorm2d):
                nn.init.constant_(m.weight, 1)
                nn.init.constant_(m.bias, 0)
        nn.init.xavier_uniform_(self.segmentation_head[0].weight)

    def forward(self, x):
        feats = self.encoder(x)
        return self.segmentation_head(self.decoder(*feats))

    @torch.no_grad()
    def forward_fused(self, x, return_features=False):
        from . import fused
        feats = fused.resnet_features(self.encoder, x)
        dec = self.decoder.forward_fused(*feats)
        head = self.segmentation_head[0]
        if head.kernel_size == (1, 1):
            dl = fused.nhwc_view(dec)
            Bq, H4, W4, Cd = dl.shape
            y2 = ops.gemm_bias_act(dl.reshape(Bq * H4 * W4, Cd), head.weight.view(head.out_channels, Cd), head.bias, 0,
                                   w_split=fused.split_weights(head, head.weight.view(head.out_channels, Cd), Bq * H4 * W4))
            low = y2.view(Bq, H4, W4, -1).permute(0, 3, 1, 2)
        else:
            low = head(dec).contiguous()
        up = self.segmentation_head[1]
        if isinstance(up, nn.UpsamplingBilinear2d) and low.is_cuda and low.dtype == torch.float32:
            f = int(up.scale_factor)
            out = ops.upsample_bilinear(low, (low.shape[2] * f, low.shape[3] * f), True)
        else:
            out = up(low)
        return (out, feats[-1]) if return_features else out
```

adverse_weather_semantic_segmentation_robustness_benchmark_amd/models/fused.py:

```python
from __future__ import annotations

import contextlib
import os
from typing import List

import torch
import torch.nn as nn
import torch.nn.functional as F

from .. import _native as N
from .. import ops

CL = torch.channels_last


def _pair(v):
    return (v, v) if isinstance(v, int) else tuple(v)


def _versions(*tensors):
    return tuple((t.data_ptr(), t._version) for t in tensors if t is not None)


DERIVED = ("wsplit", "wbf16", "wsplit_small", "kvsplit", "proj_pieces", "stemrows")
# ... 151 lines not shown
def conv_bn_act(x: torch.Tensor, conv: nn.Conv2d, bn: nn.BatchNorm2d, act: int, residual: torch.Tensor = None,
                residual_is_scratch: bool = False) -> torch.Tensor:
    w, shift = folded_conv_bn(conv, bn)
    if _is_pointwise(conv) and x.is_contiguous(memory_format=CL):
        if conv.stride == (2, 2):
            Bq, Cq, Hq, Wq = x.shape
            mq = Bq * ((Hq - 1) // 2 + 1) * ((Wq - 1) // 2 + 1)
            wq = w.view(w.shape[0], Cq)
            wsq = split_weights(conv, wq, mq) if (ops.CONV_GATHER and Cq % 32 == 0 and residual is None and act in (N.ACT_RELU, N.ACT_NONE)) else None
            if wsq is not None and not getattr(wsq, "_awseg_bf16", False):
                return ops.conv_gemm_split(nhwc_view(x), wsq, shift, act, 1, 1, 2, 0).permute(0, 3, 1, 2)
            x = x[:, :, ::2, ::2].contiguous(memory_format=CL)
        B, Cin, H, W = x.shape
        Cout = w.shape[0]
        x2 = x.permute(0, 2, 3, 1).reshape(B * H * W, Cin)
        w2 = w.view(Cout, Cin)
        if act in (N.ACT_RELU, N.ACT_NONE):
            r2 = None if residual is None else nhwc_view(residual).reshape(B * H * W, Cout)
            y2 = ops.gemm_bias_act(x2, w2, shift, act, residual=r2, out=r2 if (r2 is not None and residual_is_scratch) else None,
                                   w_split=split_weights(conv, w2, B * H * W))
        else:
            y2 = torch.addmm(shift, x2, w2.t()) if residual is None else torch.addmm(nhwc_view(residual).reshape(B * H * W, Cout), x2, w2.t())
            ops.bias_act_nhwc_(y2, torch.zeros_like(shift) if residual is None else shift, None, act)
        return y2.view(B, H, W, Cout).permute(0, 3, 1, 2)
    if _is_patch_gemm(conv) and residual is None and act in (N.ACT_NONE, N.ACT_RELU):
        def build():
            inv = torch.rsqrt(bn.running_var + bn.eps)
            scale = bn.weight * inv
            sh = bn.bias - bn.running_mean * scale
            if conv.bias is not None:
                sh = sh + conv.bias * scale
            return patch_weights(conv, scale), sh.contiguous()
        w2, sh = cached(conv, "patch", [conv.weight, conv.bias, bn.weight, bn.bias, bn.running_mean, bn.running_var], build)
        return conv_gemm_nhwc(nhwc_view(x), conv, w2, sh, act).permute(0, 3, 1, 2)
    if _is_winograd(conv) and act in (N.ACT_NONE, N.ACT_RELU):
        y = conv3x3_winograd_bn(nhwc_view(x), conv, bn, act, None if residual is None else nhwc_view(residual))
        return y.permute(0, 3, 1, 2)
    y = F.conv2d(x, w, None, conv.stride, conv.padding, conv.dilation, conv.groups)
    if not y.is_contiguous(memory_format=CL):
        y = y.contiguous(memory_format=CL)
    ops.bias_act_nhwc_(y.permute(0, 2, 3, 1), shift, None if residual is None else nhwc_view(residual), act)
    return y


STEM_ROWS = os.environ.get("AWSEG_STEM_ROWS", "1") != "0"
_stem_pad = {}
_stem_scope = None


@contextlib.contextmanager
def stem_scope():
    global _stem_scope
    prev, _stem_scope = _stem_scope, {}
    try:
        yield
    finally:
        _stem_scope = prev


def stem_image_ok(x: torch.Tensor) -> bool:
    return STEM_ROWS and ops.GEMM_SPLIT and x.is_cuda and x.dtype == torch.float32 and x.dim() == 4 and x.shape[1] <= 4 and ops.PRECISION != "bf16"


def stem_image(x: torch.Tensor) -> torch.Tensor:
    B, C, H, W = x.shape
    wp_any = max(W + 3, ((W + 6 - 7) // 2) * 2 + 8, ((W + 6 - 7) // 4) * 4 + 8)
    skey = (x.data_ptr(), tuple(x.shape), tuple(x.stride()))
    xp = _stem_scope.get(skey) if _stem_scope is not None else None
    if xp is None:
        key = (str(x.device), B, H, W, C, wp_any)
        xp = _stem_pad.get(key)
        if xp is None:
            _stem_pad.clear()
            xp = _stem_pad[key] = torch.zeros(B, H, wp_any, 4, dtype=torch.float32, device=x.device)
        if x.stride(3) == 1 and x.stride(2) >= W and min(x.stride()) >= 0:
            ops.stem_image_fill(x, xp)
        else:
            xp[:, :, 3:3 + W, :C] = x.permute(0, 2, 3, 1)
        if _stem_scope is not None:
            _stem_scope[skey] = xp
    return xp


def _stem_rows(x: torch.Tensor, conv: nn.Conv2d, w: torch.Tensor, bias: torch.Tensor = None):
    st = conv.stride[0]
    if not (STEM_ROWS and ops.GEMM_SPLIT and x.is_cuda and x.dtype == torch.float32 and conv.kernel_size == (7, 7) and conv.stride in ((2, 2), (4, 4))
            and conv.padding == (3, 3) and conv.dilation == (1, 1) and conv.groups == 1 and conv.in_channels <= 4
            and (conv.out_channels % 64 == 0 or 8 <= conv.out_channels < 64) and ops.PRECISION != "bf16"):
        return None
    B, C, H, W = x.shape
    wo = (W + 6 - 7) // st + 1
    wp = max(W + 3, (wo - 1) * st + 8)
    xp = stem_image(x)
    assert wp <= xp.shape[2]
    ws = cached(conv, "stemrows", [w], lambda: ops.gemm_split_weights(ops.stem_rows_weights(w)))
    return ops.conv_rows_gemm_split(xp, ws, bias, N.ACT_NONE, 7, st, 3, wo)


def _bottleneck_tail_dual(out: torch.Tensor, y: torch.Tensor, blk):
    c3, cd, bn3, bnd = blk.conv3, blk.downsample[0], blk.bn3, blk.downsample[1]
    if not (ops.DUAL_TAIL and ops.GEMM_SPLIT and ops.PRECISION != "bf16" and out.is_cuda and out.dtype == torch.float32
            and c3.kernel_size == (1, 1) and cd.kernel_size == (1, 1) and c3.stride == (1, 1) and c3.groups == 1 and cd.groups == 1
            and cd.stride[0] == cd.stride[1] and cd.padding == (0, 0) and c3.padding == (0, 0)
            and c3.in_channels % 32 == 0 and cd.in_channels % 32 == 0 and isinstance(bnd, nn.BatchNorm2d)):
        return None
    ol, yl = nhwc_view(out), nhwc_view(y)
    B, Ho, Wo, k1 = ol.shape
    _, H, W, k2 = yl.shape
    st = cd.stride[0]
    if (H - 1) // st + 1 != Ho or (W - 1) // st + 1 != Wo:
        return None
    n = c3.out_channels

    def build():
        w3, b3 = folded_conv_bn(c3, bn3)
        wd, bd = folded_conv_bn(cd, bnd)
        return ops.gemm_split_weights(torch.cat([w3.reshape(n, k1), wd.reshape(n, k2)], dim=1).contiguous()), (b3 + bd).contiguous()
    ws, bias = cached(blk, "dualtail", [c3.weight, bn3.weight, bn3.bias, bn3.running_mean, bn3.running_var,
                                        cd.weight, bnd.weight, bnd.bias, bnd.running_mean, bnd.running_var], build)
    y2 = ops.gemm_split_dual(ol.view(B * Ho * Wo, k1), yl if st > 1 else yl.view(B * H * W, k2), ws, bias, N.ACT_RELU, stride=st if st > 1 else 0)
    return None if y2 is None else y2.view(B, Ho, Wo, n).permute(0, 3, 1, 2)


@torch.no_grad()
def resnet_features(enc, x: torch.Tensor, stem_feature: bool = False) -> List[torch.Tensor]:
    feats = [x]
    if stem_feature:
        x = x.contiguous(memory_format=CL)
        feats = [x]
        y = conv_bn_act(x, enc.conv1, enc.bn1, N.ACT_RELU)
        feats.append(y)
        y = enc.maxpool(y)
    else:
        w, shift = folded_conv_bn(enc.conv1, enc.bn1)
        y = _stem_rows(x, enc.conv1, w)
        y = y.permute(0, 3, 1, 2) if y is not None else F.conv2d(x.contiguous(memory_format=CL), w, None, enc.conv1.stride, enc.conv1.padding)
        mp = enc.maxpool
        if (y.is_cuda and y.dtype == torch.float32 and y.is_contiguous(memory_format=CL) and y.shape[1] % 4 == 0
                and _pair(mp.kernel_size) == (3, 3) and _pair(mp.stride) == (2, 2) and _pair(mp.padding) == (1, 1)
                and _pair(mp.dilation) == (1, 1) and not mp.ceil_mode):
            y = ops.maxpool3x3s2_nhwc(nhwc_view(y), shift=shift).permute(0, 3, 1, 2)
        else:
            y = mp(y)
            if not y.is_contiguous(memory_format=CL):
                y = y.contiguous(memory_format=CL)
            ops.bias_act_nhwc_(y.permute(0, 2, 3, 1), shift, None, N.ACT_RELU)
        feats.append(None)
    for layer in (enc.layer1, enc.layer2, enc.layer3, enc.layer4):
        for blk in layer:
            out = conv_bn_act(y, blk.conv1, blk.bn1, N.ACT_RELU)
            out = conv_bn_act(out, blk.conv2, blk.bn2, N.ACT_RELU)
            if blk.downsample is not None:
                y2 = _bottleneck_tail_dual(out, y, blk)
                if y2 is not None:
                    y = y2
                    continue
            idn = y if blk.downsample is None else conv_bn_act(y, blk.downsample[0], blk.downsample[1], N.ACT_NONE)
            scratch = not any(idn is f for f in feats)
            y = conv_bn_act(out, blk.conv3, blk.bn3, N.ACT_RELU, residual=idn, residual_is_scratch=scratch)
        feats.append(y)
    return feats


@torch.no_grad()
def separable_bn_relu(x: torch.Tensor, sep, bn: nn.BatchNorm2d) -> torch.Tensor:
    dwc, pwc = sep[0], sep[1]
    xl = nhwc_view(x)
    B, H, W, C = xl.shape
    d = ops.dwconv3x3_nhwc(xl, dw_taps(dwc), None, N.ACT_NONE, dilation=dwc.dilation[0])
    w, shift = folded_conv_bn(pwc, bn)
    w2 = w.view(w.shape[0], C)
    y = ops.gemm_bias_act(d.view(B * H * W, C), w2, shift, N.ACT_RELU, w_split=split_weights(pwc, w2, B * H * W))
    return y.view(B, H, W, -1).permute(0, 3, 1, 2)


def _ln(t, ln: nn.LayerNorm):
    c = t.shape[-1]
    if c % 4 == 0 and c <= 1024 and ln.weight is not None and ln.bias is not None:
        return ops.layernorm_rows(t, ln.weight, ln.bias, ln.eps)
    return F.layer_norm(t, (c,), ln.weight, ln.bias, ln.eps)


LINEAR_SPLIT = os.environ.get("AWSEG_LINEAR_SPLIT", "1") != "0"


def _linear(x: torch.Tensor, lin: nn.Linear) -> torch.Tensor:
    k = x.shape[-1]
    m = x.numel() // k
    if lin.bias is not None and x.is_contiguous() and (ops.gemm_wants_bf16(m, lin.out_features, k) or
                                                       (LINEAR_SPLIT and ops.gemm_wants_split(m, lin.out_features, k))):
        y = ops.gemm_bias_act(x.view(m, k), lin.weight, lin.bias, N.ACT_NONE, w_split=split_weights(lin, lin.weight, m))
        return y.view(*x.shape[:-1], lin.out_features)
    return F.linear(x, lin.weight, lin.bias)


def _linear_residual(x2: torch.Tensor, lin: nn.Linear, tok: torch.Tensor) -> torch.Tensor:
    if lin.bias is None or not tok.is_contiguous():
        return tok + F.linear(x2, lin.weight, lin.bias).view_as(tok)
    t2 = tok.view(-1, tok.shape[-1])
    ops.gemm_bias_act(x2, lin.weight, lin.bias, N.ACT_NONE, residual=t2, out=t2, w_split=split_weights(lin, lin.weight, x2.shape[0]))
    return tok


def _kv_packed(kv: torch.Tensor, a) -> torch.Tensor:
    kp, vp = a.k_proj, a.v_proj
    wkv, bkv = cached(a, "kvpack", [kp.weight, kp.bias, vp.weight, vp.bias],
                      lambda: (torch.cat([kp.weight, vp.weight]).contiguous(), torch.cat([kp.bias, vp.bias]).contiguous()))
    c = kv.shape[-1]
    m = kv.numel() // c
    if ops.gemm_wants_bf16(m, 2 * c, c) or ops.gemm_wants_split(m, 2 * c, c):
        y = ops.gemm_bias_act(kv.view(m, c), wkv, bkv, N.ACT_NONE, w_split=split_weights(a, wkv, m))
    else:
        ws = cached(a, "kvsplit", (wkv,), lambda: ops.gemm_split_weights(wkv))
        y = ops.gemm_bias_act(kv.view(m, c), wkv, bkv, N.ACT_NONE, w_split=ws, split=True)
    return y.view(*kv.shape[:-1], 2 * c)


@torch.no_grad()
def mit_features_nhwc(seg, x: torch.Tensor) -> torch.Tensor:
    if not hasattr(seg, "stages"):
        return seg(x).last_hidden_state.permute(0, 2, 3, 1).contiguous()
    t = x
    tok = None
    for st in seg.stages:
        pe = st.patch_embeddings
        if _is_patch_gemm(pe.proj) and pe.proj.bias is not None:
            w2 = cached(pe.proj, "patch", [pe.proj.weight], lambda: patch_weights(pe.proj))
            y = conv_gemm_nhwc(nhwc_view(t), pe.proj, w2, pe.proj.bias, N.ACT_NONE)
        else:
# ... 63 lines not shown
```

adverse_weather_semantic_segmentation_robustness_benchmark_amd/ops.py:

```python
from __future__ import annotations

import math
import os

import ctypes as C
from typing import Optional, Sequence

import numpy as np
import torch

from . import _native as N

IMAGENET_MEAN = np.array([0.485, 0.456, 0.406], dtype=np.float32)
IMAGENET_STD = np.array([0.229, 0.224, 0.225], dtype=np.float32)
NIGHT_GAINS = np.array([0.8, 0.85, 1.2], dtype=np.float32)
CONDITIONS = ("clean", "fog", "rain", "snow", "night")


def gaussian_taps(sigma: float = 2.0, truncate: float = 4.0) -> np.ndarray:
    radius = int(truncate * float(sigma) + 0.5)
    x = np.arange(-radius, radius + 1)
    phi = np.exp(-0.5 / (sigma * sigma) * x ** 2)
    return phi / phi.sum()

# ... 1329 lines not shown
                                     N.ptr(ws), GEMM_WORKSPACE_BYTES, N.stream())
        if rc < 0:
            N.check(rc, "awseg_gemm_tune")
        del scratch
    if out is None:
        out = torch.empty(m, n, dtype=torch.float32, device=x.device)
    N.call("awseg_gemm_bias_act", N.ptr(x), N.ptr(w), N.ptr(bias), N.ptr(residual), act, N.ptr(out), m, n, k,
           N.ptr(ws), GEMM_WORKSPACE_BYTES, N.stream())
    return out


GEMM_SPLIT = os.environ.get("AWSEG_GEMM_SPLIT", "1") != "0"
GEMM_SPLIT_MIN_M, GEMM_SPLIT_MIN_N, GEMM_SPLIT_MIN_K = 128, 128, 64
GEMM_SPLIT_N64 = os.environ.get("AWSEG_GEMM_SPLIT_N64", "1") != "0"


GEMM_SPLIT_NARROW = os.environ.get("AWSEG_GEMM_SPLIT_NARROW", "1") != "0"
STRIDED_UPSAMPLE = os.environ.get("AWSEG_STRIDED_UPSAMPLE", "0") != "0"
KV_PACKED = os.environ.get("AWSEG_KV_PACKED", "1") != "0"
SMALL_CONV_SPLIT = os.environ.get("AWSEG_SMALL_CONV_SPLIT", "1") != "0"


def gemm_wants_split(m: int, n: int, k: int) -> bool:
    if not GEMM_SPLIT or k % 8:
        return False
    if GEMM_SPLIT_NARROW and 8 <= n < 64 and k >= 32 and m >= (1 << 18):
        return True
    if GEMM_SPLIT_NARROW and n % 64 == 0 and k == 32 and m >= (1 << 18):
        return True
    if m < GEMM_SPLIT_MIN_M or k < GEMM_SPLIT_MIN_K:
        return False
    return n >= GEMM_SPLIT_MIN_N or (n == 64 and GEMM_SPLIT_N64 and ((m + 255) // 256) >= 128)


def gemm_split_weights(w: torch.Tensor) -> torch.Tensor:
    w = w.contiguous()
    n, k = w.shape
    buf = torch.empty(int(N.lib().awseg_gemm_split_weight_halfs(n, k)), dtype=torch.int16, device=w.device)
    N.call("awseg_gemm_split_weights", N.ptr(w), n, k, N.ptr(buf), N.stream())
    return buf[:2 * n * k].view(2, n, k)


def _split_weights_intact(w_split: torch.Tensor, n: int, k: int) -> bool:
    return w_split.untyped_storage().nbytes() - w_split.storage_offset() * 2 >= int(N.lib().awseg_gemm_split_weight_halfs(n, k)) * 2


def gemm_split_bias_act(x: torch.Tensor, w_split: torch.Tensor, bias: Optional[torch.Tensor], act: int = 0,
                        residual: Optional[torch.Tensor] = None, out: Optional[torch.Tensor] = None) -> torch.Tensor:
    x = x.contiguous()
    m, k = x.shape
    n = w_split.shape[1]
    if not _split_weights_intact(w_split, n, k):
        raise N.AwsegError("w_split lost its 16-byte trailer (weight exponent): pass the tensor gemm_split_weights returned, not a copy")
    if out is None:
        out = torch.empty(m, n, dtype=torch.float32, device=x.device)
    N.call("awseg_gemm_split_bias_act", N.ptr(x), N.ptr(w_split), N.ptr(bias), N.ptr(residual), act, N.ptr(out), m, n, k, N.stream())
    return out


def stem_rows_weights(w: torch.Tensor) -> torch.Tensor:
    n, c, kh, kw = w.shape
    if c > 4 or kw > 8:
        raise N.AwsegError("stem_rows_weights: at most 4 input channels and 8 kernel columns")
    m = torch.zeros(n, kh, 8, 4, dtype=torch.float32, device=w.device)
    m[:, :, :kw, :c] = w.permute(0, 2, 3, 1)
    return m.view(n, kh * 32)


def conv_rows_gemm_split(x_padded: torch.Tensor, w_split: torch.Tensor, bias: Optional[torch.Tensor], act: int, kernel_h: int,
                         stride: int, pad_y: int, out_width: int) -> Optional[torch.Tensor]:
    b, h, wp, pf = x_padded.shape
    n, k = w_split.shape[1], w_split.shape[2]
    if k != kernel_h * 32 or not x_padded.is_contiguous():
        raise N.AwsegError("conv_rows_gemm_split: weights must be [N, kernel_h * 32] and the image contiguous")
    if not _split_weights_intact(w_split, n, k):
        raise N.AwsegError("w_split lost its 16-byte trailer (weight exponent): pass the tensor gemm_split_weights returned, not a copy")
    ho = (h + 2 * pad_y - kernel_h) // stride + 1
    out = torch.empty(b, ho, out_width, n, dtype=torch.float32, device=x_padded.device)
    rc = N.try_call("awseg_conv_rows_gemm_split_bias_act", N.ptr(x_padded), b, h, wp, pf, kernel_h, stride, pad_y, out_width,
                    N.ptr(w_split), N.ptr(bias), None, act, N.ptr(out), n, N.stream())
    return out if rc == 0 else None


CONV_GATHER = os.environ.get("AWSEG_CONV_GATHER", "1") != "0"


ASPP_PIECES = os.environ.get("AWSEG_ASPP_PIECES", "1") != "0"
DUAL_TAIL = os.environ.get("AWSEG_DUAL_TAIL", "1") != "0"


def gemm_split_dual(x: torch.Tensor, x2: torch.Tensor, w_split: torch.Tensor, bias: Optional[torch.Tensor], act: int = 0, stride: int = 0,
                    residual: Optional[torch.Tensor] = None) -> Optional[torch.Tensor]:
    x, x2 = x.contiguous(), x2.contiguous()
    m, k1 = x.shape
    k2 = x2.shape[-1]
    n = w_split.shape[1]
    if w_split.shape[2] != k1 + k2:
        raise N.AwsegError(f"gemm_split_dual: weights have K = {w_split.shape[2]}, the operands {k1} + {k2}")
    if not _split_weights_intact(w_split, n, k1 + k2):
        raise N.AwsegError("w_split lost its 16-byte trailer (weight exponent): pass the tensor gemm_split_weights returned, not a copy")
    if stride > 0:
        b, h, w = x2.shape[0], x2.shape[1], x2.shape[2]
    else:
        b, h, w = 1, 1, 1
        if x2.numel() != m * k2:
            raise N.AwsegError("gemm_split_dual: x2 has a different row count than x")
    out = torch.empty(m, n, dtype=torch.float32, device=x.device)
    rc = N.try_call("awseg_gemm_split_dual_bias_act", N.ptr(x), k1, N.ptr(x2), k2, b, h, w, int(stride), N.ptr(w_split), N.ptr(bias),
                    N.ptr(residual), act, N.ptr(out), m, n, N.stream())
    return out if rc == 0 else None


def gemm_split_pieces(pieces, w_split: torch.Tensor, bias: Optional[torch.Tensor], act: int = 0, residual: Optional[torch.Tensor] = None,
                      out: Optional[torch.Tensor] = None) -> Optional[torch.Tensor]:
    import ctypes
    pieces = [p_.contiguous() for p_ in pieces]
    m, kp = pieces[0].shape
    n = w_split.shape[1]
    if any(p_.shape != (m, kp) for p_ in pieces) or w_split.shape[2] != kp * len(pieces):
        raise N.AwsegError("gemm_split_pieces: the pieces must be equally shaped and the weights [N, pieces * k]")
    if not _split_weights_intact(w_split, n, kp * len(pieces)):
        raise N.AwsegError("w_split lost its 16-byte trailer (weight exponent): pass the tensor gemm_split_weights returned, not a copy")
    if out is None:
        out = torch.empty(m, n, dtype=torch.float32, device=pieces[0].device)
    arr = (ctypes.c_void_p * len(pieces))(*[p_.data_ptr() for p_ in pieces])
    rc = N.try_call("awseg_gemm_split_pieces_bias_act", ctypes.cast(arr, ctypes.c_void_p), len(pieces), kp, N.ptr(w_split), N.ptr(bias),
                    N.ptr(residual), act, N.ptr(out), m, n, N.stream())
    return out if rc == 0 else None


def conv_gemm_split(x: torch.Tensor, w_split: torch.Tensor, bias: Optional[torch.Tensor], act: int, kh: int, kw: int, stride: int,
                    pad: int, dilation: int = 1, residual: Optional[torch.Tensor] = None) -> torch.Tensor:
    x = x.contiguous()
    b, h, w, c = x.shape
    n, k = w_split.shape[1], w_split.shape[2]
    if k != kh * kw * c:
        raise N.AwsegError(f"conv_gemm_split: weights have K = {k}, the convolution needs {kh * kw * c}")
    if not _split_weights_intact(w_split, n, k):
        raise N.AwsegError("w_split lost its 16-byte trailer (weight exponent): pass the tensor gemm_split_weights returned, not a copy")
    ho = (h + 2 * pad - dilation * (kh - 1) - 1) // stride + 1
    wo = (w + 2 * pad - dilation * (kw - 1) - 1) // stride + 1
    out = torch.empty(b, ho, wo, n, dtype=torch.float32, device=x.device)
    N.call("awseg_conv_gemm_split_bias_act", N.ptr(x), b, h, w, c, kh, kw, stride, pad, dilation, N.ptr(w_split), N.ptr(bias),
           N.ptr(residual), act, N.ptr(out), n, N.stream())
    return out


def im2col_nhwc(x: torch.Tensor, kh: int, kw: int, stride: int, pad: int, dilation: int = 1, k_padded: Optional[int] = None):
    x = x.contiguous()
    b, h, w, c = x.shape
    k = kh * kw * c
    kp = k if k_padded is None else int(k_padded)
    ho = (h + 2 * pad - dilation * (kh - 1) - 1) // stride + 1
    wo = (w + 2 * pad - dilation * (kw - 1) - 1) // stride + 1
    cols = torch.empty(b * ho * wo, kp, dtype=torch.float32, device=x.device)
    N.call("awseg_im2col_nhwc", N.ptr(x), b, h, w, c, kh, kw, stride, pad, dilation, kp, N.ptr(cols), N.stream())
    return cols, ho, wo


def dwconv3x3_upcat(a: torch.Tensor, hi: torch.Tensor, w9: torch.Tensor) -> torch.Tensor:
    a, hi = a.contiguous(), hi.contiguous()
    b, h, w, ca = a.shape
    _, H, W, ch = hi.shape
    out = torch.empty(b, H, W, ca + ch, dtype=torch.float32, device=a.device)
    N.call("awseg_dwconv3x3_upcat_nhwc", N.ptr(a), h, w, ca, N.ptr(hi), ch, b, H, W, N.ptr(w9.contiguous()), N.ptr(out), N.stream())
    return out


ATTENTION_SPLIT = os.environ.get("AWSEG_ATTN_SPLIT", "1") != "0"


def attention_d32(q: torch.Tensor, k: torch.Tensor, v: torch.Tensor, heads: int, scale: float,
                  split: Optional[bool] = None) -> torch.Tensor:
    q, k, v = q.contiguous(), k.contiguous(), v.contiguous()
    b, nq, c = q.shape
    out = torch.empty_like(q)
    if split is None and PRECISION == "bf16":
        sym = "awseg_attention_d32_bf16"
    else:
        sym = "awseg_attention_d32_split" if (ATTENTION_SPLIT if split is None else split) else "awseg_attention_d32"
    if sym == "awseg_attention_d32_split" and _wants_kv_image(nq, k.shape[1]):
        _attention_split_ws(q, k, v, 0, out, b, heads, nq, k.shape[1], scale)
        return out
    N.call(sym, N.ptr(q), N.ptr(k), N.ptr(v), N.ptr(out), b, heads, nq, k.shape[1], float(scale), N.stream())
    return out


ATTN_KV_IMAGE = os.environ.get("AWSEG_ATTN_KV_IMAGE", "1") != "0"


def _wants_kv_image(nq: int, nkv: int) -> bool:
    return ATTN_KV_IMAGE and nq >= 8 * nkv


def _attention_split_ws(q, k, v, pitch, out, b, heads, nq, nkv, scale):
    nbytes = int(N.lib().awseg_attention_d32_split_workspace(b, heads, nkv))
    ws = N.workspace.get(q.device, nbytes, tag="attn%d" % torch.cuda.current_stream(q.device).cuda_stream)
    N.call("awseg_attention_d32_split_ws", N.ptr(q), N.ptr_strided(k), N.ptr_strided(v), int(pitch), N.ptr(out), b, heads, nq, nkv, float(scale),
           N.ptr(ws), N.stream())


def attention_d32_packed_kv(q: torch.Tensor, kv: torch.Tensor, heads: int, scale: float, split: Optional[bool] = None) -> torch.Tensor:
    q, kv = q.contiguous(), kv.contiguous()
    b, nq, c = q.shape
    assert kv.shape[-1] == 2 * c
    out = torch.empty_like(q)
    mode = 2 if (split is None and PRECISION == "bf16") else (1 if (ATTENTION_SPLIT if split is None else split) else 0)
    if mode == 1 and _wants_kv_image(nq, kv.shape[1]):
        _attention_split_ws(q, kv, kv[..., c:], 2 * c, out, b, heads, nq, kv.shape[1], scale)
        return out
# ... 144 lines not shown
```

include/awseg.h:

```cpp
#ifndef AWSEG_H
#define AWSEG_H

#include <stddef.h>
#include <stdint.h>

#ifdef __cplusplus
extern "C" {
#endif

typedef void* awseg_stream_t;

#define AWSEG_EINVAL   (-1)
#define AWSEG_ERANGE   (-2)
#define AWSEG_EALIGN   (-3)

#define AWSEG_U8   0
#define AWSEG_I64  1

#define AWSEG_COMBINE_WEIGHTED  0
#define AWSEG_COMBINE_MAXCONF   1
#define AWSEG_COMBINE_MEAN      2

#define AWSEG_LOSS_CE     0
#define AWSEG_LOSS_FOCAL  1
// ... 122 lines not shown
                     const awseg_prim_job* jobs, int n_jobs, const int32_t* flakes,
                     uint8_t* out, float* norm_out,
                     const float* mean_host, const float* std_host,
                     void* workspace, awseg_stream_t stream);

int awseg_fog_density_field(const float* scale_offset, int batch, int64_t hw, uint64_t seed,
                            const float* uniform, float* density, awseg_stream_t stream);

int64_t awseg_loss_partials(int64_t batch, int64_t hw);
int awseg_fog_ce_forward(const float* logits, const void* label, int label_dtype,
                         const float* density, int64_t batch, int num_classes, int64_t hw,
                         int base_loss, float sensitivity,
                         float* pixel_loss, double* partials, float* loss_mean,
                         int64_t* oob, awseg_stream_t stream);
int awseg_fog_ce_backward(const float* logits, const void* label, int label_dtype,
                          const float* density, int64_t batch, int num_classes, int64_t hw,
                          int base_loss, float sensitivity, const float* grad_scale,
                          float* grad_logits, awseg_stream_t stream);

int64_t awseg_density_workspace(int64_t batch, int64_t hw);
int awseg_fog_density_from_depth(const float* depth, int64_t batch, int height, int width,
                                 float* density, void* workspace, awseg_stream_t stream);

int awseg_segformer_head_fused(const float* g9, int64_t batch, int cmid, int h, int w,
                               int height, int width,
                               const float* scale, const float* shift,
                               const float* w2, const float* b2, int cout,
                               float* out, awseg_stream_t stream);

int awseg_segformer_head_fused_split(const float* g9, int64_t batch, int cmid, int h, int w,
                                     int height, int width,
                                     const float* scale, const float* shift,
                                     const float* w2, const float* b2, int cout,
                                     float* out, awseg_stream_t stream);

int awseg_upconv3x3_bn_relu(const float* g9, int64_t batch, int cmid, int h, int w,
                            int height, int width,
                            const float* scale, const float* shift,
                            float* out, int channels_last, awseg_stream_t stream);

int awseg_aspp_depthwise3(const float* x, int64_t batch, int h, int w, int channels,
                          const float* wdw, int rate0, int rate1, int rate2,
                          float* out, awseg_stream_t stream);
int awseg_aspp_depthwise3_mean(const float* x, int64_t batch, int h, int w, int channels, const float* wdw,
                               int rate0, int rate1, int rate2, float* out, float* mean_out, awseg_stream_t stream);

#define AWSEG_ACT_NONE 0
#define AWSEG_ACT_RELU 1
#define AWSEG_ACT_GELU 2
int awseg_dwconv3x3_nhwc(const float* x, int64_t batch, int height, int width, int channels, int dilation,
                         const float* w9, const float* bias, int act, float* out, awseg_stream_t stream);

int awseg_conv3x3_winograd_nhwc(const float* x, int batch, int height, int width, int cin, int cout, int dilation,
                                const float* u, const float* shift, const float* residual, int act,
                                const float* w2, const float* b2, float* out, awseg_stream_t stream);

int awseg_gemm_bias_act(const float* x, const float* w, const float* bias, const float* residual, int act,
                        float* out, int64_t m, int n, int k, void* workspace, size_t workspace_bytes,
                        awseg_stream_t stream);

int awseg_gemm_tune(const float* x, const float* w, const float* bias, int has_residual, int act,
                    float* scratch_out, int64_t m, int n, int k, void* workspace, size_t workspace_bytes,
                    awseg_stream_t stream);

int64_t awseg_gemm_split_weight_halfs(int n, int k);
int awseg_gemm_split_weights(const float* w, int n, int k, uint16_t* w_split, awseg_stream_t stream);
int awseg_gemm_split_bias_act(const float* x, const uint16_t* w_split, const float* bias, const float* residual, int act,
                              float* out, int64_t m, int n, int k, awseg_stream_t stream);

int awseg_dwconv3x3_upcat_nhwc(const float* a, int a_height, int a_width, int a_channels, const float* hi, int hi_channels,
                               int64_t batch, int height, int width, const float* w9, float* out, awseg_stream_t stream);

int64_t awseg_winograd_split_weight_halfs(int cin, int cout);

int64_t awseg_upconv_forms_floats(int h, int w, int cmid);
int awseg_upconv_forms(const float* g9, int batch, int cmid, int h, int w, const float* shift, float* forms, awseg_stream_t stream);
int awseg_depth_head_fused(const float* forms, int batch, int h, int w, int cmid, const uint16_t* u_split, int u_is_bf16,
                           const float* shift2, const float* w2, const float* b2, float* out, awseg_stream_t stream);
int awseg_conv3x3_winograd_split_nhwc(const float* x, int batch, int height, int width, int cin, int cout, int dilation,
                                      const uint16_t* u_split, const float* shift, const float* residual, int act,
                                      const float* w2, const float* b2, float* out, awseg_stream_t stream);

int awseg_gemm_split_pieces_bias_act(const float* const* pieces, int n_pieces, int k_piece, const uint16_t* w_split, const float* bias,
                                     const float* residual, int act, float* out, int64_t m, int n, awseg_stream_t stream);

int awseg_gemm_split_dual_bias_act(const float* x, int k1, const float* x2, int k2, int64_t batch, int x2_height, int x2_width,
                                   int x2_stride, const uint16_t* w_split, const float* bias, const float* residual, int act,
                                   float* out, int64_t m, int n, awseg_stream_t stream);

int awseg_conv_gemm_split_bias_act(const float* x, int64_t batch, int height, int width, int channels,
                                   int kernel_h, int kernel_w, int stride, int pad, int dilation,
                                   const uint16_t* w_split, const float* bias, const float* residual, int act,
                                   float* out, int n, awseg_stream_t stream);

int awseg_conv_rows_gemm_split_bias_act(const float* x, int64_t batch, int height, int width_padded, int pixel_floats,
                                        int kernel_h, int stride, int pad_y, int out_width, const uint16_t* w_split,
                                        const float* bias, const float* residual, int act, float* out, int n,
                                        awseg_stream_t stream);

int64_t awseg_gemm_bf16_weight_halfs(int n, int k);
int awseg_gemm_bf16_weights(const float* w, int n, int k, uint16_t* w_bf16, awseg_stream_t stream);
int awseg_gemm_bf16_bias_act(const float* x, const uint16_t* w_bf16, const float* bias, const float* residual, int act,
                             float* out, int64_t m, int n, int k, awseg_stream_t stream);
int awseg_conv3x3_winograd_bf16_nhwc(const float* x, int batch, int height, int width, int cin, int cout, int dilation,
                                     const uint16_t* u_bf16, const float* shift, const float* residual, int act,
                                     const float* w2, const float* b2, float* out, awseg_stream_t stream);
int awseg_attention_d32_bf16(const float* q, const float* k, const float* v, float* out, int batch, int heads,
                             int n_queries, int n_keys, float scale, awseg_stream_t stream);
int64_t awseg_attention_d32_split_workspace(int batch, int heads, int n_keys);
int awseg_attention_d32_split_ws(const float* q, const float* k, const float* v, int kv_pitch, float* out, int batch, int heads,
                                 int n_queries, int n_keys, float scale, void* workspace, awseg_stream_t stream);

int awseg_attention_d32_packed_kv(const float* q, const float* kv, float* out, int batch, int heads, int n_queries,
                                  int n_keys, float scale, int mode, awseg_stream_t stream);

int awseg_upconv3x3_linear(const float* g9, int64_t batch, int cmid, int h, int w, int height, int width,
                           const float* bias, float* out, int channels_last, awseg_stream_t stream);
int awseg_upconv3x3_adjoint(const float* dz, int64_t batch, int cmid, int h, int w, int height, int width,
                            float* dg9, awseg_stream_t stream);

int awseg_im2col_nhwc(const float* x, int64_t batch, int height, int width, int channels, int kernel_h, int kernel_w,
                      int stride, int pad, int dilation, int k_padded, float* cols, awseg_stream_t stream);

int awseg_attention_d32(const float* q, const float* k, const float* v, float* out, int batch, int heads,
                        int n_queries, int n_keys, float scale, awseg_stream_t stream);

int awseg_attention_d32_split(const float* q, const float* k, const float* v, float* out, int batch, int heads,
                              int n_queries, int n_keys, float scale, awseg_stream_t stream);

int64_t awseg_bn_train_workspace(int batch, int channels, int64_t hw);
int awseg_bn_train_stats(const float* x, int batch, int channels, int64_t hw, void* workspace, float* mean, float* var, awseg_stream_t stream);
int awseg_bn_relu_dropout_forward(const float* x, int batch, int channels, int64_t hw, const float* mean, const float* invstd,
                                  const float* gamma, const float* beta, const float* noise, float* out, awseg_stream_t stream);
int awseg_bn_relu_dropout_backward(const float* x, const float* grad_out, int batch, int channels, int64_t hw, const float* mean,
                                   const float* invstd, const float* gamma, const float* beta, const float* noise, void* workspace,
                                   float* dgamma, float* dbeta, float* dx, int dx_channels_last, awseg_stream_t stream);

int64_t awseg_dwconv3x3_wgrad_workspace(int64_t batch, int height, int width, int channels);
int awseg_dwconv3x3_wgrad_nhwc(const float* x, const float* dy, int64_t batch, int height, int width, int channels, int dilation,
                               void* workspace, float* dw9, float* db, awseg_stream_t stream);

int awseg_mixffn_fused(const float* tok, int batch, int height, int width, int channels, const float* ln_gamma, const float* ln_beta,
                       float ln_eps, const uint16_t* w1_split, int w1_exp, const float* b1, const float* dw_taps, const float* dw_bias,
                       const uint16_t* w2_split, int w2_exp, const float* w2, const float* b2, float* out, awseg_stream_t stream);

int awseg_maxpool3x3s2_nhwc(const float* x, int64_t batch, int height, int width, int channels, float* out,
                            awseg_stream_t stream);
int awseg_maxpool3x3s2_bias_relu_nhwc(const float* x, int64_t batch, int height, int width, int channels, const float* shift,
                                      float* out, awseg_stream_t stream);

int awseg_upsample_bilinear(const float* low, int64_t planes, int low_height, int low_width,
                            int height, int width, int align_corners, float* out, awseg_stream_t stream);
int awseg_upsample_bilinear_strided(const float* low, int64_t batch, int channels, int low_height, int low_width,
                                    int64_t stride_b, int64_t stride_c, int64_t stride_y, int64_t stride_x,
                                    int height, int width, int align_corners, float* out, awseg_stream_t stream);

int awseg_rowdot_sigmoid(const float* x, int64_t rows, int k, const float* w, const float* bias, int sigmoid, float* out,
                         awseg_stream_t stream);

int64_t awseg_aspp_pool_branch_workspace(int batch, int cmid);
int awseg_aspp_pool_branch(const float* mean, int batch, int cin, const float* w1, const float* b1, int cmid, const float* w2,
                           const float* b2, int cout, void* workspace, float* out, awseg_stream_t stream);

int awseg_stem_image(const float* x, int batch, int channels, int height, int width, int64_t stride_b, int64_t stride_c,
                     int64_t stride_y, float* image, int padded_width, awseg_stream_t stream);

int awseg_depth_upsample_combine(const float* d1, const float* d2_low, int batch, int low_height, int low_width,
                                 int height, int width, const float* weights, float* d2_full, float* d_out,
                                 awseg_stream_t stream);

int awseg_bias_act_nhwc(float* x, int64_t n_pixels, int channels, const float* bias, const float* residual,
                        int act, awseg_stream_t stream);

int awseg_layernorm_rows(const float* x, int64_t n_rows, int channels, const float* gamma, const float* beta,
                         float eps, float* out, awseg_stream_t stream);

int awseg_ece_accumulate(const float* logits, int64_t batch, int num_classes, int64_t hw,
                         const void* label, int label_dtype, const int32_t* cond,
                         const float* edges, int n_bins,
                         void* bins, int n_slots, void* workspace, awseg_stream_t stream);

int awseg_ensemble_eval_stats(const float* seg1, const float* seg2, int64_t batch, int num_classes, int64_t hw,
                              int mode, const float* weights, const float* temperature,
                              const void* label, int label_dtype, const int32_t* cond,
                              const float* edges, int n_bins, void* ece_bins, int n_slots,
                              int64_t* auroc_hist, int n_hist, float hist_lo, float hist_hi,
                              void* workspace, awseg_stream_t stream);

int awseg_combine_confusion_stats(const float* seg1, const float* seg2, int64_t batch, int num_classes, int64_t hw,
                                  int mode, const float* weights, const float* temperature, const void* label,
                                  int label_dtype, int ignore_index, int label_wrap_u8, const int32_t* cond,
                                  int64_t* counts, int count_slots, int64_t* oob, const float* edges, int n_bins,
// ... 132 lines not shown
```

Baseline: 232.9.

## Split KV-image build across blocks, add per-image GEMM bias and fused stem-pool GEMM

The attention KV-image conversion kernel now runs over a third grid dimension, so each block converts only a slice of key tiles. This gives more parallelism when batch*heads is small. The split GEMM pieces path gains a per-image bias, with tile mapping aligned to image boundaries, which can replace a broadcast bias add. A new fused stem conv plus maxpool GEMM kernel is added but sits behind an opt-in env flag that defaults to off. Every block in the split KV build still rescans all tiles to find the max, so that part of the work is duplicated.

```diff
diff --git a/adverse_weather_semantic_segmentation_robustness_benchmark_amd/_native.py b/adverse_weather_semantic_segmentation_robustness_benchmark_amd/_native.py
--- a/adverse_weather_semantic_segmentation_robustness_benchmark_amd/_native.py
+++ b/adverse_weather_semantic_segmentation_robustness_benchmark_amd/_native.py
@@ -49,6 +49,7 @@
     "awseg_conv3x3_winograd_bf16_nhwc": (c_i, [c_p, c_i, c_i, c_i, c_i, c_i, c_i, c_p, c_p, c_p, c_i, c_p, c_p, c_p, c_p]),
     "awseg_attention_d32_bf16": (c_i, [c_p, c_p, c_p, c_p, c_i, c_i, c_i, c_i, c_f, c_p]),
     "awseg_attention_d32_split_workspace": (c_i64, [c_i, c_i, c_i]),
+    "awseg_attention_d32_kv_image": (c_i, [c_p, c_p, c_i, c_i, c_i, c_i, c_p, c_i, c_p]),
     "awseg_attention_d32_split_ws": (c_i, [c_p, c_p, c_p, c_i, c_p, c_i, c_i, c_i, c_i, c_f, c_p, c_p]),
     "awseg_attention_d32_packed_kv": (c_i, [c_p, c_p, c_p, c_i, c_i, c_i, c_i, c_f, c_i, c_p]),
     "awseg_dwconv3x3_upcat_nhwc": (c_i, [c_p, c_i, c_i, c_i, c_p, c_i, c_i64, c_i, c_i, c_p, c_p, c_p]),
@@ -90,10 +91,11 @@
     "awseg_layernorm_rows": (c_i, [c_p, c_i64, c_i, c_p, c_p, c_f, c_p, c_p]),
     "awseg_ensemble_eval_stats": (c_i, [c_p, c_p, c_i64, c_i, c_i64, c_i, c_p, c_p, c_p, c_i, c_p, c_p, c_i, c_p, c_i, c_p, c_i,
                                        c_f, c_f, c_p, c_p]),
-    "awseg_gemm_split_pieces_bias_act": (c_i, [c_p, c_i, c_i, c_p, c_p, c_p, c_i, c_p, c_i64, c_i, c_p]),
+    "awseg_gemm_split_pieces_bias_act": (c_i, [c_p, c_i, c_i, c_p, c_p, c_p, c_i, c_p, c_i64, c_i, c_i64, c_p]),
     "awseg_gemm_split_dual_bias_act": (c_i, [c_p, c_i, c_p, c_i, c_i64, c_i, c_i, c_i, c_p, c_p, c_p, c_i, c_p, c_i64, c_i, c_p]),
     "awseg_conv_gemm_split_bias_act": (c_i, [c_p, c_i64, c_i, c_i, c_i, c_i, c_i, c_i, c_i, c_i, c_p, c_p, c_p, c_i, c_p, c_i, c_p]),
     "awseg_conv_rows_gemm_split_bias_act": (c_i, [c_p, c_i64, c_i, c_i, c_i, c_i, c_i, c_i, c_i, c_p, c_p, c_p, c_i, c_p, c_i, c_p]),
+    "awseg_conv_rows_pool_gemm_split": (c_i, [c_p, c_i64, c_i, c_i, c_i, c_i, c_i, c_i, c_i, c_p, c_p, c_p, c_i, c_p]),
     "awseg_bn_train_workspace": (c_i64, [c_i, c_i, c_i64]),
     "awseg_bn_train_stats": (c_i, [c_p, c_i, c_i, c_i64, c_p, c_p, c_p, c_p]),
     "awseg_bn_relu_dropout_forward": (c_i, [c_p, c_i, c_i, c_i64, c_p, c_p, c_p, c_p, c_p, c_p, c_p]),
diff --git a/adverse_weather_semantic_segmentation_robustness_benchmark_amd/csrc/attn.hip b/adverse_weather_semantic_segmentation_robustness_benchmark_amd/csrc/attn.hip
--- a/adverse_weather_semantic_segmentation_robustness_benchmark_amd/csrc/attn.hip
+++ b/adverse_weather_semantic_segmentation_robustness_benchmark_amd/csrc/attn.hip
@@ -413,9 +413,11 @@
     const int wk0 = lkey * SROW + 4 * lc;
     const int wv0 = TK * SROW + (4 * lc) * SROW + pv_slot(lkey);
     const int ntiles = nkv / TK;
+    const int t_lo = (int)((int64_t)ntiles * blockIdx.z / gridDim.z), t_hi = (int)((int64_t)ntiles * (blockIdx.z + 1) / gridDim.z);
     if (tid < 2) sM[tid] = 0u;
     __syncthreads();
     float kmax = 0.f, vmax = 0.f;
+#pragma unroll 8
     for (int t = 0; t < ntiles; ++t) {
         kmax = amax4(kmax, *reinterpret_cast<const float4*>(kb + (size_t)t * TK * kvp + g_off));
         vmax = amax4(vmax, *reinterpret_cast<const float4*>(vb + (size_t)t * TK * kvp + g_off));
@@ -426,9 +428,10 @@
     const int ek = guard_exponent(sM[0]), ev = guard_exponent(sM[1]);
     auto p2 = [](int e) { return __builtin_bit_cast(float, (unsigned)(127 + e) << 23); };
     const float sk = p2(-ek), sv = p2(-ev);
-    if (tid == 0) { exps[((size_t)b * heads + h) * 2] = ek; exps[((size_t)b * heads + h) * 2 + 1] = ev; }
+    if (tid == 0 && blockIdx.z == 0) { exps[((size_t)b * heads + h) * 2] = ek; exps[((size_t)b * heads + h) * 2 + 1] = ev; }
     _Float16* base = img + ((size_t)b * heads + h) * ntiles * IMG_TILE_HALFS;
-    for (int t = 0; t < ntiles; ++t) {
+#pragma unroll 2
+    for (int t = t_lo; t < t_hi; ++t) {
         float4 kk4 = *reinterpret_cast<const float4*>(kb + (size_t)t * TK * kvp + g_off);
         float4 vv4 = *reinterpret_cast<const float4*>(vb + (size_t)t * TK * kvp + g_off);
         kk4.x *= sk; kk4.y *= sk; kk4.z *= sk; kk4.w *= sk;
@@ -650,6 +653,35 @@
     return tab + (int64_t)batch * heads * (n_keys / TK) * IMG_TILE_HALFS * 2;
 }
 
+static int kv_image_splits(int batch, int heads, int n_keys)
+{
+    const int64_t bh = (int64_t)batch * heads;
+    const int64_t s = (64 + bh - 1) / bh;
+    const int ntiles = n_keys / TK;
+    return (int)(s < 1 ? 1 : (s > ntiles ? ntiles : s));
+}
+
+AWSEG_API int awseg_attention_d32_kv_image(const float* k, const float* v, int kv_pitch, int batch, int heads, int n_keys, void* workspace,
+                                           int splits, awseg_stream_t stream)
+{
+    if (batch == 0) return 0;
+    if (!k || !v || !workspace || batch < 0 || heads < 1 || n_keys < TK || splits < 0) return AWSEG_EINVAL;
+    if (n_keys % TK || heads > 65535 || batch > 65535) return AWSEG_ERANGE;
+    if (((uintptr_t)k & 15) || ((uintptr_t)v & 15) || ((uintptr_t)workspace & 255)) return AWSEG_EALIGN;
+    if (kv_pitch == 0) kv_pitch = heads * D;
+    if (kv_pitch < heads * D || (kv_pitch & 3)) return AWSEG_EINVAL;
+    if ((int64_t)(n_keys / TK) * IMG_TILE_HALFS * 2 > 0x7fffffff) return AWSEG_ERANGE;
+    int* exps = reinterpret_cast<int*>(workspace);
+    const int64_t tab = ((int64_t)batch * heads * 2 * 4 + 255) / 256 * 256;
+    _Float16* img = reinterpret_cast<_Float16*>(reinterpret_cast<char*>(workspace) + tab);
+    if (splits == 0) splits = kv_image_splits(batch, heads, n_keys);
+    if (splits > n_keys / TK) splits = n_keys / TK;
+    hipLaunchKernelGGL(attn_kv_image_kernel, dim3((unsigned)heads, (unsigned)batch, (unsigned)splits), dim3(AT), 0, awseg_s(stream), k, v, kv_pitch,
+                       n_keys, heads, img, exps);
+    AWSEG_LAUNCH_CHECK();
+    return 0;
+}
+
 AWSEG_API int awseg_attention_d32_split_ws(const float* q, const float* k, const float* v, int kv_pitch, float* out, int batch, int heads,
                                            int n_queries, int n_keys, float scale, void* workspace, awseg_stream_t stream)
 {
@@ -664,8 +696,8 @@
     int* exps = reinterpret_cast<int*>(workspace);
     const int64_t tab = ((int64_t)batch * heads * 2 * 4 + 255) / 256 * 256;
     _Float16* img = reinterpret_cast<_Float16*>(reinterpret_cast<char*>(workspace) + tab);
-    hipLaunchKernelGGL(attn_kv_image_kernel, dim3((unsigned)heads, (unsigned)batch), dim3(AT), 0, awseg_s(stream), k, v, kv_pitch, n_keys, heads, img, exps);
-    AWSEG_LAUNCH_CHECK();
+    const int rc = awseg_attention_d32_kv_image(k, v, kv_pitch, batch, heads, n_keys, workspace, 0, stream);
+    if (rc) return rc;
     dim3 grid((unsigned)((n_queries + 127) / 128), (unsigned)heads, (unsigned)batch);
     hipLaunchKernelGGL(attention_d32_split_img_kernel, grid, dim3(AT), 0, awseg_s(stream), q, img, exps, out, n_queries, n_keys, heads,
                        scale * 1.4426950408889634f);
diff --git a/adverse_weather_semantic_segmentation_robustness_benchmark_amd/csrc/awseg_common.h b/adverse_weather_semantic_segmentation_robustness_benchmark_amd/csrc/awseg_common.h
--- a/adverse_weather_semantic_segmentation_robustness_benchmark_amd/csrc/awseg_common.h
+++ b/adverse_weather_semantic_segmentation_robustness_benchmark_amd/csrc/awseg_common.h
@@ -154,10 +154,12 @@
 
 int awseg_gemm_split3_weights(const float* w, int n, int k, uint16_t* w3, const unsigned* trailer, hipStream_t stream);
 bool awseg_gemm_split3_eligible(int64_t m, int n, int k, const void* x, const void* out, const void* residual, const void* bias);
-struct awseg_g3_dual { const float* x2; int k1; int h, w, stride, ho, wo; int64_t bytes; const float* x3 = nullptr; const float* x4 = nullptr; };
+struct awseg_g3_dual { const float* x2; int k1; int h, w, stride, ho, wo; int64_t bytes; const float* x3 = nullptr; const float* x4 = nullptr; int bias_rpi = 0; };
 int awseg_gemm_split3_launch(const float* x, const uint16_t* w3, const unsigned* trailer, const float* bias, const float* residual,
                              int act, float* out, int64_t m, int n, int k, int cus, hipStream_t stream, const int* conv = nullptr,
                              bool bf16 = false, const awseg_g3_dual* dual = nullptr);
+int awseg_gemm_split3_pool_launch(const float* x, const uint16_t* w3, const unsigned* trailer, const float* shift, float* out, int k,
+                                  const int* conv, int cus, hipStream_t stream);
 int awseg_gemm_split3_bn(int n);
 int64_t awseg_gemm_split3_image_rows(int n);
 int awseg_gemm_bf16_3_weights(const float* w, int n, int k, uint16_t* w3, hipStream_t stream);
diff --git a/adverse_weather_semantic_segmentation_robustness_benchmark_amd/csrc/gemm_split.hip b/adverse_weather_semantic_segmentation_robustness_benchmark_amd/csrc/gemm_split.hip
--- a/adverse_weather_semantic_segmentation_robustness_benchmark_amd/csrc/gemm_split.hip
+++ b/adverse_weather_semantic_segmentation_robustness_benchmark_amd/csrc/gemm_split.hip
@@ -402,6 +402,12 @@
 namespace {
 struct conv_desc { int H, W, C, Ho, Wo, kw, stride, pad, dil; int64_t batch; int pitch = 0, padx = -1; };
 
+bool g3_fills(int64_t m, int n, bool bf16, int cus)
+{
+    return ((m + 255) / 256) * (int64_t)((n + awseg_gemm_split3_bn(n) - 1) / awseg_gemm_split3_bn(n)) >= (int64_t)cus / 2 ||
+           (!bf16 && ((m + 127) / 128) * (int64_t)((n + 127) / 128) >= (int64_t)cus / 2);
+}
+
 int gemm_launch(bool bf16, const float* x, const uint16_t* w_split, const float* bias, const float* residual,
                 int act, float* out, int64_t m, int n, int k, awseg_stream_t stream, const conv_desc* cv = nullptr)
 {
@@ -419,8 +425,7 @@
     const int cus = awseg_cu_count();
     if (awseg_gemm_split3_eligible(m, n, k, cv ? nullptr : x, out, residual, bias) && !(bf16 && (cv || n % 256)) &&
         (!cv || (cv->C % 32 == 0 && (int64_t)cv->batch * cv->H * cv->W * (cv->pitch > 0 ? cv->pitch : cv->C) * 4 <= 0x7fffffff)) &&
-        (((m + 255) / 256) * (int64_t)((n + awseg_gemm_split3_bn(n) - 1) / awseg_gemm_split3_bn(n)) >= (int64_t)cus / 2 ||
-         (!bf16 && ((m + 127) / 128) * (int64_t)((n + 127) / 128) >= (int64_t)cus / 2))) {
+        g3_fills(m, n, bf16, cus)) {
         const int cdesc[12] = { cv ? cv->H : 0, cv ? cv->W : 0, cv ? cv->C : 0, cv ? cv->Ho : 0, cv ? cv->Wo : 0, cv ? cv->kw : 0,
                                 cv ? cv->stride : 0, cv ? cv->pad : 0, cv ? cv->dil : 0, cv ? (int)cv->batch : 0, cv ? cv->pitch : 0, cv ? cv->padx : -1 };
         return awseg_gemm_split3_launch(x, w_split + 2 * (int64_t)n * k + 8, a.trailer, bias, residual, act, out, m, n, k, cus, awseg_s(stream),
@@ -499,9 +504,11 @@
 }
 
 AWSEG_API int awseg_gemm_split_pieces_bias_act(const float* const* pieces, int n_pieces, int k_piece, const uint16_t* w_split, const float* bias,
-                                               const float* residual, int act, float* out, int64_t m, int n, awseg_stream_t stream)
+                                               const float* residual, int act, float* out, int64_t m, int n, int64_t rows_per_image,
+                                               awseg_stream_t stream)
 {
     if (m == 0 || n == 0) return 0;
+    if (rows_per_image < 0 || (rows_per_image > 0 && !bias)) return AWSEG_EINVAL;
     if (!pieces || n_pieces < 2 || n_pieces > 4 || !w_split || !out || m < 0 || n < 0 || k_piece < 32 || act < 0 || act > 1) return AWSEG_EINVAL;
     if (k_piece % 32) return AWSEG_ERANGE;
     for (int i = 0; i < n_pieces; ++i) {
@@ -515,6 +522,7 @@
     d.x2 = pieces[1]; d.k1 = k_piece; d.stride = 0; d.h = d.w = d.ho = d.wo = 1;
     d.bytes = m * (int64_t)k_piece * 4;
     d.x3 = n_pieces > 2 ? pieces[2] : nullptr; d.x4 = n_pieces > 3 ? pieces[3] : nullptr;
+    d.bias_rpi = rows_per_image > 0 && rows_per_image < m ? (int)rows_per_image : 0;
     if (d.bytes > 0x7fffffff) return AWSEG_ERANGE;
     return awseg_gemm_split3_launch(pieces[0], w_split + 2 * (int64_t)n * k + 8, reinterpret_cast<const unsigned*>(w_split + 2 * (int64_t)n * k), bias, residual,
                                     act, out, m, n, k, awseg_cu_count(), awseg_s(stream), nullptr, false, &d);
@@ -553,6 +561,26 @@
     return gemm_launch(false, x, w_split, bias, residual, act, out, batch * ho * out_width, n, kernel_h * 32, stream, &cv);
 }
 
+AWSEG_API int awseg_conv_rows_pool_gemm_split(const float* x, int64_t batch, int height, int width_padded, int pixel_floats, int kernel_h,
+                                              int stride, int pad_y, int out_width, const uint16_t* w_split, const float* shift, float* out,
+                                              int n, awseg_stream_t stream)
+{
+    if (batch == 0) return 0;
+    if (!x || !w_split || !shift || !out || batch < 0 || height < 1 || width_padded < 8 || kernel_h < 1 || stride < 1 || pad_y < 0 || out_width < 1) return AWSEG_EINVAL;
+    if (pixel_floats < 4 || pixel_floats % 4 || 32 % pixel_floats) return AWSEG_ERANGE;
+    if ((int64_t)(out_width - 1) * stride * pixel_floats + 32 > (int64_t)width_padded * pixel_floats) return AWSEG_ERANGE;
+    if (((uintptr_t)x & 15) || ((uintptr_t)w_split & 15)) return AWSEG_EALIGN;
+    const int ho = (height + 2 * pad_y - kernel_h) / stride + 1;
+    if (ho < 1 || batch * height > 0x7fffffff || n != 64) return AWSEG_ERANGE;
+    const int64_t m = batch * ho * out_width;
+    const int k = kernel_h * 32, cus = awseg_cu_count();
+    if (!awseg_gemm_split3_eligible(m, n, k, nullptr, nullptr, nullptr, nullptr) || !g3_fills(m, n, false, cus) ||
+        batch * height * width_padded * pixel_floats * 4 > 0x7fffffff) return AWSEG_ERANGE;
+    const int cdesc[8] = { height, width_padded, ho, out_width, stride, pad_y, (int)batch, pixel_floats };
+    return awseg_gemm_split3_pool_launch(x, w_split + 2 * (int64_t)n * k + 8, reinterpret_cast<const unsigned*>(w_split + 2 * (int64_t)n * k), shift, out, k,
+                                         cdesc, cus, awseg_s(stream));
+}
+
 AWSEG_API int awseg_gemm_bf16_weights(const float* w, int n, int k, uint16_t* w_bf16, awseg_stream_t stream)
 {
     if (n == 0 || k == 0) return 0;
diff --git a/adverse_weather_semantic_segmentation_robustness_benchmark_amd/csrc/gemm_split3.hip b/adverse_weather_semantic_segmentation_robustness_benchmark_amd/csrc/gemm_split3.hip
--- a/adverse_weather_semantic_segmentation_robustness_benchmark_amd/csrc/gemm_split3.hip
+++ b/adverse_weather_semantic_segmentation_robustness_benchmark_amd/csrc/gemm_split3.hip
@@ -53,6 +53,7 @@
     const float* x2; int K1, x2H, x2W, x2s, x2Ho, x2Wo;
     int64_t x2_bytes;
     const float* x3; const float* x4; int K2;
+    int bias_rpi, bias_tpi;
 };
 
 typedef __bf16 bf8_3 __attribute__((ext_vector_type(8)));
@@ -80,11 +81,17 @@
     const int ktail = K % G3K;
     const int ntiles = a.ntm8 * a.ntn;
 
-    auto tile_of = [&](int slot, int64_t& m0, int& n0) -> bool {
+    auto tile_of = [&](int slot, int64_t& m0, int& n0, int64_t& mend, int& img) -> bool {
         const int xcd = slot & 7, jj = slot >> 3;
         const int nt_i = jj % a.ntn, mt_i = (jj / a.ntn) * 8 + xcd;
-        m0 = (int64_t)mt_i * G3M; n0 = nt_i * BN;
-        return mt_i < a.ntm;
+        m0 = (int64_t)mt_i * G3M; n0 = nt_i * BN; mend = a.M; img = 0;
+        if (DUAL && a.bias_rpi > 0) {
+            img = mt_i / a.bias_tpi;
+            m0 = (int64_t)img * a.bias_rpi + (int64_t)(mt_i - img * a.bias_tpi) * G3M;
+            const int64_t e = (int64_t)(img + 1) * a.bias_rpi;
+            mend = e < a.M ? e : a.M;
+        }
+        return mt_i < a.ntm && m0 < mend;
     };
 
     const int rl = lane >> 3, sl = lane & 7;
@@ -96,8 +103,8 @@
     const uint32_t lds0 = __builtin_amdgcn_readfirstlane(lds_addr3(smem));
     const uint32_t wave_u = __builtin_amdgcn_readfirstlane(wave);
     __amdgpu_buffer_rsrc_t x_rsrc, w_rsrc, x2_rsrc, x3_rsrc, x4_rsrc;
-    auto point = [&](int64_t m0, int n0) {
-        const int64_t rows_left = a.M - m0;
+    auto point = [&](int64_t m0, int n0, int64_t mend) {
+        const int64_t rows_left = mend - m0;
         const int64_t xbytes = rows_left * (int64_t)KA * 4;
         if (CONV) x_rsrc = __builtin_amdgcn_make_buffer_rsrc((void*)a.x, 0, (int)a.x_bytes, 0x00020000);
         else x_rsrc = __builtin_amdgcn_make_buffer_rsrc((void*)(a.x + m0 * KA), 0, (int)(xbytes > 0x7fffffff ? 0x7fffffff : xbytes), 0x00020000);
@@ -124,7 +131,7 @@
                     const int oy = rem / a.x2Wo, ox = rem - oy * a.x2Wo;
                     pix = ((int64_t)b * a.x2H + oy * a.x2s) * a.x2W + ox * a.x2s;
                 }
-                a_voff2[j] = m < a.M ? (uint32_t)(pix * k2 * 4 + c * 16) : 0x80000000u;
+                a_voff2[j] = m < mend ? (uint32_t)(pix * k2 * 4 + c * 16) : 0x80000000u;
             }
             {
                 const int qi = wave * NBI + j;
@@ -198,8 +205,8 @@
     }
 
     int slot = blockIdx.x;
-    int64_t m0 = 0; int n0 = 0;
-    while (slot < ntiles && !tile_of(slot, m0, n0)) slot += gridDim.x;
+    int64_t m0 = 0, mend = 0; int n0 = 0, img = 0;
+    while (slot < ntiles && !tile_of(slot, m0, n0, mend, img)) slot += gridDim.x;
     if (slot >= ntiles) return;
     if (tid < 4) sMax[tid] = 0u;
     int par = 0;
@@ -213,13 +220,13 @@
     unsigned long long g3s[6] = {0, 0, 0, 0, 0, 0};
     G3_T(sb0);
 #endif
-    point(m0, n0);
+    point(m0, n0, mend);
     issue(0, 0);
 
     while (true) {
         int nslot = slot + gridDim.x;
-        int64_t nm0 = 0; int nn0 = 0;
-        while (nslot < ntiles && !tile_of(nslot, nm0, nn0)) nslot += gridDim.x;
+        int64_t nm0 = 0, nmend = 0; int nn0 = 0, nimg = 0;
+        while (nslot < ntiles && !tile_of(nslot, nm0, nn0, nmend, nimg)) nslot += gridDim.x;
         const bool has_next = nslot < ntiles;
 
         f32x16 acc[NT];
@@ -312,8 +319,8 @@
             issue(0, g & 1);
             continue;
         }
-        const int64_t em0 = m0; const int en0 = n0;
-        if (has_next) { point(nm0, nn0); issue(0, g & 1); }
+        const int64_t em0 = m0, emend = mend; const int en0 = n0, eimg = img;
+        if (has_next) { point(nm0, nn0, nmend); issue(0, g & 1); }
 
         const int oe = BF16 ? 0 : we + xe;
         const int oe1 = oe / 2, oe2 = oe - oe1;
@@ -321,12 +328,12 @@
 
         {
             const int64_t tile_off = em0 * a.N + en0;
-            const int64_t rem = ((int64_t)a.M * a.N - tile_off) * 4;
+            const int64_t rem = (emend * a.N - tile_off) * 4;
             const int nrec = rem > 0x7fffffff ? 0x7fffffff : (int)rem;
             const __amdgpu_buffer_rsrc_t o_rsrc = __builtin_amdgcn_make_buffer_rsrc((void*)(a.out + tile_off), 0, nrec, 0x00020000);
             const __amdgpu_buffer_rsrc_t r_rsrc = __builtin_amdgcn_make_buffer_rsrc((void*)((a.residual ? a.residual : a.out) + tile_off), 0, a.residual ? nrec : 0, 0x00020000);
             const int ncols = a.N - en0 < BN ? a.N - en0 : BN;
-            const __amdgpu_buffer_rsrc_t b_rsrc = __builtin_amdgcn_make_buffer_rsrc((void*)((a.bias ? a.bias : a.out) + en0), 0, a.bias ? ncols * 4 : 0, 0x00020000);
+            const __amdgpu_buffer_rsrc_t b_rsrc = __builtin_amdgcn_make_buffer_rsrc((void*)((a.bias ? a.bias : a.out) + (int64_t)eimg * a.N + en0), 0, a.bias ? ncols * 4 : 0, 0x00020000);
             const int voff = ((wave * 32 + 4 * hk) * a.N + li) * 4;
             int vcol[NT];
 #pragma unroll
@@ -377,7 +384,7 @@
         }
         if (!has_next) break;
         stores_pending = true;
-        slot = nslot; m0 = nm0; n0 = nn0;
+        slot = nslot; m0 = nm0; n0 = nn0; mend = nmend; img = nimg;
         scaled = false; sx = kActScale0; xe = kActExp0;
     }
     asm volatile("s_waitcnt vmcnt(0)" ::: "memory");
@@ -388,6 +395,246 @@
         g_g3_stamp[tid >> 8][5] += sb1 - sb0;
     }
 #endif
+}
+
+struct g3p_args {
+    const float* x; const uint16_t* w3; const float* shift; float* out; const unsigned* trailer;
+    int K, cH, cW, cHo, cWo, cs, cp, cpitch;
+    int64_t x_bytes;
+    int Hp, Wp, nstrips, R, nbands, nitems;
+};
+constexpr int kPoolStrip = 63;
+constexpr int G3P_LDS = 2 * (128 * 128) + 2 * (64 * 128) + 64 + 3 * 64 * 4;
+
+__device__ __forceinline__ float nanmax3(float m, float v) { return (v > m || v != v) ? v : m; }
+
+struct g3p_pos { int it, b, s, py0, oy, oy_first, oy_last; };
+
+__global__ __launch_bounds__(256, 3)
+void gemm_split3_pool_kernel(g3p_args a)
+{
+    constexpr int NT = 2, G3_STAGE = 128 * 128, G3_BSTAGE = 64 * 128, G3_B0 = 2 * G3_STAGE;
+    extern __shared__ __attribute__((aligned(16))) unsigned char smem[];
+    unsigned* sMax = reinterpret_cast<unsigned*>(smem + 2 * G3_STAGE + 2 * G3_BSTAGE);
+    float* sEdge = reinterpret_cast<float*>(smem + 2 * G3_STAGE + 2 * G3_BSTAGE + 64);
+    const int tid = threadIdx.x, lane = tid & 63, wave = tid >> 6;
+    const int hk = lane >> 5, li = lane & 31;
+    const int nkt = a.K / G3K;
+
+    auto item_begin = [&](int it, g3p_pos& p) {
+        p.it = it;
+        p.s = it % a.nstrips;
+        const int t = it / a.nstrips, band = t % a.nbands;
+        p.b = t / a.nbands;
+        p.py0 = band * a.R;
+        const int py1 = p.py0 + a.R < a.Hp ? p.py0 + a.R : a.Hp;
+        p.oy_first = 2 * p.py0 - 1 < 0 ? 0 : 2 * p.py0 - 1;
+        p.oy_last = 2 * py1 - 1 < a.cHo - 1 ? 2 * py1 - 1 : a.cHo - 1;
+        p.oy = p.oy_first;
+    };
+    auto advance = [&](const g3p_pos& c, g3p_pos& n) -> bool {
+        if (c.oy < c.oy_last) { n = c; n.oy = c.oy + 1; return true; }
+        if (c.it + (int)gridDim.x >= a.nitems) return false;
+        item_begin(c.it + (int)gridDim.x, n);
+        return true;
+    };
+
+    const int rl = lane >> 3, sl = lane & 7;
+    uint32_t b_voff[2];
+    int colb[4];
+    int iy0 = 0, ib = 0;
+    const uint32_t lds0 = __builtin_amdgcn_readfirstlane(lds_addr3(smem));
+    const uint32_t wave_u = __builtin_amdgcn_readfirstlane(wave);
+    const __amdgpu_buffer_rsrc_t x_rsrc = __builtin_amdgcn_make_buffer_rsrc((void*)a.x, 0, (int)a.x_bytes, 0x00020000);
+    const __amdgpu_buffer_rsrc_t w_rsrc = __builtin_amdgcn_make_buffer_rsrc((void*)a.w3, 0, 64 * nkt * 128, 0x00020000);
+#pragma unroll
+    for (int j = 0; j < 2; ++j) {
+        const int brow = 8 * (wave * 2 + j) + rl;
+        b_voff[j] = (uint32_t)(brow * 128 + ((sl ^ ((brow >> 1) & 7)) * 16));
+    }
+    auto point = [&](const g3p_pos& p) {
+        ib = p.b * a.cH; iy0 = p.oy * a.cs - a.cp;
+#pragma unroll
+        for (int j = 0; j < 4; ++j) {
+            const int row = 8 * (4 * wave + j) + rl;
+            const int c = sl ^ ((row >> 1) & 7);
+            const int ox = 2 * kPoolStrip * p.s - 1 + row;
+            colb[j] = (ox >= 0 && ox < a.cWo) ? ox * a.cs * a.cpitch * 4 + c * 16 : -1;
+        }
+    };
+    auto issue = [&](int kt, int stage) {
+        const uint32_t la = lds0 + (uint32_t)(stage * G3_STAGE) + wave_u * 4096u;
+        const int iy = iy0 + kt;
+        const bool rok = (unsigned)iy < (unsigned)a.cH;
+        const uint32_t rowb = (uint32_t)((ib + iy) * a.cW * a.cpitch * 4);
+#pragma unroll
+        for (int j = 0; j < 4; ++j) dma16(x_rsrc, (rok && colb[j] >= 0) ? rowb + (uint32_t)colb[j] : 0x80000000u, 0u, la + (uint32_t)(j * 1024));
+        const uint32_t lbw = lds0 + (uint32_t)(G3_B0 + stage * G3_BSTAGE) + wave_u * 2048u;
+#pragma unroll
+        for (int j = 0; j < 2; ++j) dma16(w_rsrc, b_voff[j], (uint32_t)(kt * 64 * 128), lbw + (uint32_t)(j * 1024));
+    };
+
+    const int sw = (li >> 1) & 7;
+    int fa[2][2], fb[2][2];
+#pragma unroll
+    for (int ks = 0; ks < 2; ++ks) {
+#pragma unroll
+        for (int e = 0; e < 2; ++e) fa[ks][e] = (wave * 32 + li) * 128 + (((4 * ks + 2 * hk + e) ^ sw) * 16);
+        fb[ks][0] = G3_B0 + li * 128 + (((2 * ks + hk) ^ sw) * 16);
+        fb[ks][1] = G3_B0 + li * 128 + (((4 + 2 * ks + hk) ^ sw) * 16);
+    }
+
+    g3p_pos cur, nxt;
+    item_begin(blockIdx.x, cur);
+    nxt = cur;
+    if (tid < 4) sMax[tid] = 0u;
+    int par = 0;
+    const int we = (int)a.trailer[1];
+    const float ninf = -__builtin_inff();
+    const float shl[NT] = { a.shift[li], a.shift[32 + li] };
+    float sh[NT];
+#pragma unroll
+    for (int j = 0; j < NT; ++j) asm volatile("v_mov_b32 %0, %1" : "=v"(sh[j]) : "v"(shl[j]));
+    float amax = 0.f, sx = kActScale0;
+    int xe = kActExp0;
+    bool scaled = false;
+    int g = 0;
+    f32x16 vm[NT];
+    point(cur);
+    issue(0, 0);
+
+    while (true) {
+        const bool has_next = advance(cur, nxt);
+        f32x16 acc[NT];
+#pragma unroll
+        for (int j = 0; j < NT; ++j)
+#pragma unroll
+            for (int r = 0; r < 16; ++r) acc[j][r] = 0.f;
+        amax = 0.f;
+
+        for (int t = 0; t < nkt; ++t, ++g) {
+            const int st = g & 1;
+            asm volatile("s_waitcnt vmcnt(0)" ::: "memory");
+            __builtin_amdgcn_s_barrier();
+            if (t + 1 < nkt) issue(t + 1, st ^ 1);
+            if (t == 0 && tid == 0) { sMax[par ^ 1] = 0u; sMax[2 + (par ^ 1)] = 0u; }
+            const unsigned char* sa = smem + st * G3_STAGE;
+            const unsigned char* sbw = smem + st * G3_BSTAGE;
+#pragma unroll
+            for (int ks = 0; ks < 2; ++ks) {
+                const f32x4 p = *reinterpret_cast<const f32x4*>(sa + fa[ks][0]);
+                const f32x4 q = *reinterpret_cast<const f32x4*>(sa + fa[ks][1]);
+                h8 Bh[NT], Bl[NT];
+#pragma unroll
+                for (int j = 0; j < NT; ++j) {
+                    Bh[j] = *reinterpret_cast<const h8*>(sbw + fb[ks][0] + j * 4096);
+                    Bl[j] = *reinterpret_cast<const h8*>(sbw + fb[ks][1] + j * 4096);
+                }
+                u32x4 H, L; unsigned h, l;
+                amax = __builtin_fmaxf(__builtin_fmaxf(amax, __builtin_fabsf(p[0])), __builtin_fabsf(p[1]));
+                amax = __builtin_fmaxf(__builtin_fmaxf(amax, __builtin_fabsf(p[2])), __builtin_fabsf(p[3]));
+                amax = __builtin_fmaxf(__builtin_fmaxf(amax, __builtin_fabsf(q[0])), __builtin_fabsf(q[1]));
+                amax = __builtin_fmaxf(__builtin_fmaxf(amax, __builtin_fabsf(q[2])), __builtin_fabsf(q[3]));
+                split2(p[0], p[1], sx, h, l); H[0] = h; L[0] = l;
+                split2(p[2], p[3], sx, h, l); H[1] = h; L[1] = l;
+                split2(q[0], q[1], sx, h, l); H[2] = h; L[2] = l;
+                split2(q[2], q[3], sx, h, l); H[3] = h; L[3] = l;
+                const h8 Ah = __builtin_bit_cast(h8, H), Al = __builtin_bit_cast(h8, L);
+#pragma unroll
+                for (int j = 0; j < NT; ++j) {
+                    acc[j] = __builtin_amdgcn_mfma_f32_32x32x16_f16(Ah, Bh[j], acc[j], 0, 0, 0);
+                    acc[j] = __builtin_amdgcn_mfma_f32_32x32x16_f16(Ah, Bl[j], acc[j], 0, 0, 0);
+                    acc[j] = __builtin_amdgcn_mfma_f32_32x32x16_f16(Al, Bh[j], acc[j], 0, 0, 0);
+                }
+            }
+        }
+
+        if (!scaled) {
+            const bool not_small = __ballot(amax >= kSmallLimit3) != 0ull;
+            if (amax >= kSplitLimit3 || !not_small) atomicMax(&sMax[par], __builtin_bit_cast(unsigned, amax));
+            if (not_small && (tid & 63) == 0) sMax[2 + par] = 1u;
+        }
+        asm volatile("s_waitcnt lgkmcnt(0)" ::: "memory");
+        __builtin_amdgcn_s_barrier();
+        const unsigned mx = sMax[par];
+        const bool small = sMax[2 + par] == 0u;
+        par ^= 1;
+        bool again = false;
+        constexpr unsigned kBig = __builtin_bit_cast(unsigned, kSplitLimit3), kSmall = __builtin_bit_cast(unsigned, kSmallLimit3);
+        if (!scaled && (mx >= kBig || (small && mx >= 0x00800000u && mx < kSmall))) {
+            const int ex = (int)(mx >> 23) & 0xff;
+            if (ex != 0xff) {
+                xe = ex - 127 - 13;
+                xe = xe < -127 ? -127 : xe;
+                sx = pow2f3(-xe);
+                scaled = true; again = true;
+            }
+        }
+        if (again) {
+            issue(0, g & 1);
+            continue;
+        }
+        if (has_next) { point(nxt); issue(0, g & 1); }
+
+        const int oe = we + xe;
+        const int oe1 = oe / 2, oe2 = oe - oe1;
+        const float os1 = pow2f3(oe1 < -126 ? -126 : (oe1 > 127 ? 127 : oe1)), os2 = pow2f3(oe2 < -126 ? -126 : (oe2 > 127 ? 127 : oe2));
+
+        {
+            const int ox_w = 2 * kPoolStrip * cur.s - 1 + 32 * wave + 4 * hk;
+            const bool first = cur.oy == cur.oy_first;
+#pragma unroll
+            for (int j = 0; j < NT; ++j)
+#pragma unroll
+                for (int r = 0; r < 16; ++r) {
+                    const int ox = ox_w + 8 * (r >> 2) + (r & 3);
+                    float v = acc[j][r] * os1 * os2;
+                    v = v != v ? ninf : v;
+                    v = (ox >= 0 && ox < a.cWo) ? v : ninf;
+                    acc[j][r] = v;
+                    vm[j][r] = first ? v : nanmax3(vm[j][r], v);
+                }
+            const bool odd = (cur.oy & 1) != 0;
+            const int py = cur.oy >> 1;
+            const bool emit = odd ? py >= cur.py0 : cur.oy == a.cHo - 1;
+            if (emit) {
+                if (wave > 0 && hk == 0) { sEdge[(wave - 1) * 64 + li] = vm[0][0]; sEdge[(wave - 1) * 64 + 32 + li] = vm[1][0]; }
+                asm volatile("s_waitcnt lgkmcnt(0)" ::: "memory");
+                __builtin_amdgcn_s_barrier();
+                float edge[NT] = { ninf, ninf };
+                if (wave < 3 && hk == 1) { edge[0] = sEdge[wave * 64 + li]; edge[1] = sEdge[wave * 64 + 32 + li]; }
+                const int64_t row_off = ((int64_t)cur.b * a.Hp + py) * a.Wp * 64;
+                const __amdgpu_buffer_rsrc_t o_rsrc = __builtin_amdgcn_make_buffer_rsrc((void*)(a.out + row_off), 0, a.Wp * 256, 0x00020000);
+#pragma unroll
+                for (int j = 0; j < NT; ++j)
+#pragma unroll
+                    for (int t = 0; t < 4; ++t) {
+                        const float send = hk ? vm[j][4 * t] : vm[j][t < 3 ? 4 * t + 4 : 0];
+                        const float got = __shfl_xor(send, 32);
+                        const float nf = (hk == 1 && t == 3) ? edge[j] : got;
+                        const float ev = nanmax3(nanmax3(vm[j][4 * t], vm[j][4 * t + 1]), vm[j][4 * t + 2]);
+                        const float od = nanmax3(nanmax3(vm[j][4 * t + 2], vm[j][4 * t + 3]), nf);
+                        const int q = 2 * (8 * wave + 2 * t + hk);
+                        const int px = kPoolStrip * cur.s + q;
+#pragma unroll
+                        for (int o = 0; o < 2; ++o) {
+                            float rv = (o ? od : ev) + sh[j];
+                            rv = rv > 0.f ? rv : 0.f;
+                            const int voff = (q + o < kPoolStrip && px + o < a.Wp) ? (px + o) * 256 + (32 * j + li) * 4 : (int)0x80000000;
+                            __builtin_amdgcn_raw_buffer_store_b32(__builtin_bit_cast(uint32_t, rv), o_rsrc, voff, 0, 0);
+                        }
+                    }
+            }
+            if (odd) {
+#pragma unroll
+                for (int j = 0; j < NT; ++j) vm[j] = acc[j];
+            }
+        }
+        if (!has_next) break;
+        cur = nxt;
+        scaled = false; sx = kActScale0; xe = kActExp0;
+    }
+    asm volatile("s_waitcnt vmcnt(0)" ::: "memory");
 }
 
 __global__ __launch_bounds__(256)
@@ -463,14 +710,14 @@
                              const awseg_g3_dual* dual)
 {
     g3_args a;
-    a.x2 = nullptr; a.K1 = k; a.x2H = a.x2W = a.x2Ho = a.x2Wo = 1; a.x2s = 0; a.x2_bytes = 0; a.x3 = a.x4 = nullptr; a.K2 = 0;
+    a.x2 = nullptr; a.K1 = k; a.x2H = a.x2W = a.x2Ho = a.x2Wo = 1; a.x2s = 0; a.x2_bytes = 0; a.x3 = a.x4 = nullptr; a.K2 = 0; a.bias_rpi = 0; a.bias_tpi = 1;
     if (dual) {
         const int pieces = 1 + (dual->x3 ? 1 : 0) + (dual->x4 ? 1 : 0);
         if (conv || bf16 || dual->k1 % G3K || dual->k1 < G3K || (k - dual->k1) % pieces || dual->bytes > 0x7fffffff) return AWSEG_ERANGE;
         const int k2 = (k - dual->k1) / pieces;
         if (k2 % G3K || k2 < G3K || (pieces > 1 && dual->stride > 0) || (dual->x4 && !dual->x3)) return AWSEG_ERANGE;
         a.x2 = dual->x2; a.K1 = dual->k1; a.x2H = dual->h; a.x2W = dual->w; a.x2s = dual->stride; a.x2Ho = dual->ho; a.x2Wo = dual->wo;
-        a.x2_bytes = dual->bytes; a.x3 = dual->x3; a.x4 = dual->x4; a.K2 = k2;
+        a.x2_bytes = dual->bytes; a.x3 = dual->x3; a.x4 = dual->x4; a.K2 = k2; a.bias_rpi = bias ? dual->bias_rpi : 0;
     }
     a.cH = a.cW = a.cC = a.cHo = a.cWo = a.ckw = a.cs = 1; a.cp = 0; a.cd = 1; a.x_bytes = 0; a.cpitch = 1; a.cpx = 0;
     if (conv) {
@@ -489,7 +736,11 @@
                                         ((m + 127) / 128) * (int64_t)((n + bn_half - 1) / bn_half) >= 4 * (int64_t)cus));
     const int rows = half ? 128 : 256;
     const int bn = half ? bn_half : img_bn;
-    const int64_t ntm = (m + rows - 1) / rows;
+    int64_t ntm = (m + rows - 1) / rows;
+    if (a.bias_rpi > 0) {
+        a.bias_tpi = (a.bias_rpi + rows - 1) / rows;
+        ntm = (m + a.bias_rpi - 1) / a.bias_rpi * a.bias_tpi;
+    }
     a.ntn = (n + bn - 1) / bn;
     const int64_t ntm8 = (ntm + 7) / 8 * 8;
     if (ntm8 * a.ntn > 0x7fffffff) return AWSEG_ERANGE;
@@ -520,6 +771,38 @@
     return 0;
 }
 
+int awseg_gemm_split3_pool_launch(const float* x, const uint16_t* w3, const unsigned* trailer, const float* shift, float* out, int k,
+                                  const int* conv, int cus, hipStream_t stream)
+{
+    g3p_args a;
+    a.x = x; a.w3 = w3; a.shift = shift; a.out = out; a.trailer = trailer; a.K = k;
+    a.cH = conv[0]; a.cW = conv[1]; a.cHo = conv[2]; a.cWo = conv[3]; a.cs = conv[4]; a.cp = conv[5]; a.cpitch = conv[7];
+    const int64_t batch = conv[6];
+    a.x_bytes = batch * a.cH * a.cW * a.cpitch * 4;
+    a.Hp = (a.cHo - 1) / 2 + 1; a.Wp = (a.cWo - 1) / 2 + 1;
+    if (k % G3K || k < G3K || a.x_bytes > 0x7fffffff || batch * a.Hp * a.Wp * 256 > 0x7fffffff) return AWSEG_ERANGE;
+    a.nstrips = (a.Wp + kPoolStrip - 1) / kPoolStrip;
+    int64_t blocks = (int64_t)cus * 3;
+    if (blocks < 8) blocks = 8;
+    int best_r = 1; int64_t best = -1;
+    const int64_t cols = batch * a.nstrips;
+    for (int r = 1; r <= a.Hp; ++r) {
+        const int64_t items = cols * ((a.Hp + r - 1) / r);
+        const int64_t cost = (items + blocks - 1) / blocks * (2 * r + 1);
+        if (best < 0 || cost <= best) { best = cost; best_r = r; }
+    }
+    a.R = best_r; a.nbands = (a.Hp + best_r - 1) / best_r;
+    const int64_t items = cols * a.nbands;
+    if (items > 0x7fffffff) return AWSEG_ERANGE;
+    a.nitems = (int)items;
+    if (blocks > items) blocks = items;
+    hipError_t e = hipFuncSetAttribute(reinterpret_cast<const void*>(gemm_split3_pool_kernel), hipFuncAttributeMaxDynamicSharedMemorySize, G3P_LDS);
+    if (e != hipSuccess) return (int)e;
+    hipLaunchKernelGGL(gemm_split3_pool_kernel, dim3((unsigned)blocks), dim3(256), G3P_LDS, stream, a);
+    AWSEG_LAUNCH_CHECK();
+    return 0;
+}
+
 #ifdef AWSEG_G3_STAMP
 AWSEG_API int awseg_debug_g3_stamps(unsigned long long* out16, int reset)
 {
diff --git a/adverse_weather_semantic_segmentation_robustness_benchmark_amd/models/deeplab.py b/adverse_weather_semantic_segmentation_robustness_benchmark_amd/models/deeplab.py
--- a/adverse_weather_semantic_segmentation_robustness_benchmark_amd/models/deeplab.py
+++ b/adverse_weather_semantic_segmentation_robustness_benchmark_amd/models/deeplab.py
@@ -247,17 +247,18 @@
             g2 = ops.aspp_pool_branch(gmean, w1f, b1f, parts[4], pb)
         else:
             g2 = branch(gmean, pw_, pbn_) @ parts[4].t() + pb
-        acc = g2[:, None, :].expand(B, h * w, Cout).contiguous().view(B * h * w, Cout)
         ys = [branch(flat, aspp.convs[0][0].weight.view(Cout, Cin), aspp.convs[0][1])]
         for r in range(3):
             mod = aspp.convs[1 + r]
             ys.append(branch(dw[r], mod[0][1].weight.view(Cout, Cin), mod[1]))
         done = None
-        if ops.ASPP_PIECES and ops.GEMM_SPLIT and ops.PRECISION != "bf16" and acc.is_cuda and Cout % 32 == 0:
+        if ops.ASPP_PIECES and ops.GEMM_SPLIT and ops.PRECISION != "bf16" and g2.is_cuda and g2.dtype == torch.float32 and Cout % 32 == 0:
             wcat = fused.cached(aspp.project[0], "proj_pieces", (parts[0], parts[1], parts[2], parts[3]),
                                 lambda: ops.gemm_split_weights(torch.cat(parts[:4], dim=1).contiguous()))
-            done = ops.gemm_split_pieces(ys, wcat, zero_bias, 1, residual=acc, out=acc)
+            done = ops.gemm_split_pieces(ys, wcat, g2, 1, rows_per_image=h * w)
+        acc = done
         if done is None:
+            acc = g2[:, None, :].expand(B, h * w, Cout).contiguous().view(B * h * w, Cout)
             for i, y in enumerate(ys):
                 ops.gemm_bias_act(y, parts[i], zero_bias, 1 if i == 3 else 0, residual=acc, out=acc, w_split=psplit[i])
         out = acc
diff --git a/adverse_weather_semantic_segmentation_robustness_benchmark_amd/models/fused.py b/adverse_weather_semantic_segmentation_robustness_benchmark_amd/models/fused.py
--- a/adverse_weather_semantic_segmentation_robustness_benchmark_amd/models/fused.py
+++ b/adverse_weather_semantic_segmentation_robustness_benchmark_amd/models/fused.py
@@ -257,18 +257,24 @@
     return xp
 
 
-def _stem_rows(x: torch.Tensor, conv: nn.Conv2d, w: torch.Tensor, bias: torch.Tensor = None):
+def _stem_rows(x: torch.Tensor, conv: nn.Conv2d, w: torch.Tensor, bias: torch.Tensor = None, pool_shift: torch.Tensor = None,
+               pool_or_plain: bool = False):
     st = conv.stride[0]
     if not (STEM_ROWS and ops.GEMM_SPLIT and x.is_cuda and x.dtype == torch.float32 and conv.kernel_size == (7, 7) and conv.stride in ((2, 2), (4, 4))
             and conv.padding == (3, 3) and conv.dilation == (1, 1) and conv.groups == 1 and conv.in_channels <= 4
             and (conv.out_channels % 64 == 0 or 8 <= conv.out_channels < 64) and ops.PRECISION != "bf16"):
-        return None
+        return (None, False) if pool_or_plain else None
     B, C, H, W = x.shape
     wo = (W + 6 - 7) // st + 1
     wp = max(W + 3, (wo - 1) * st + 8)
     xp = stem_image(x)
     assert wp <= xp.shape[2]
     ws = cached(conv, "stemrows", [w], lambda: ops.gemm_split_weights(ops.stem_rows_weights(w)))
+    y = ops.conv_rows_pool_gemm_split(xp, ws, pool_shift, 7, st, 3, wo) if pool_shift is not None else None
+    if pool_or_plain:
+        return (y, True) if y is not None else (ops.conv_rows_gemm_split(xp, ws, bias, N.ACT_NONE, 7, st, 3, wo), False)
+    if pool_shift is not None:
+        return y
     return ops.conv_rows_gemm_split(xp, ws, bias, N.ACT_NONE, 7, st, 3, wo)
 
 
@@ -308,18 +314,22 @@
         y = enc.maxpool(y)
     else:
         w, shift = folded_conv_bn(enc.conv1, enc.bn1)
-        y = _stem_rows(x, enc.conv1, w)
-        y = y.permute(0, 3, 1, 2) if y is not None else F.conv2d(x.contiguous(memory_format=CL), w, None, enc.conv1.stride, enc.conv1.padding)
         mp = enc.maxpool
-        if (y.is_cuda and y.dtype == torch.float32 and y.is_contiguous(memory_format=CL) and y.shape[1] % 4 == 0
-                and _pair(mp.kernel_size) == (3, 3) and _pair(mp.stride) == (2, 2) and _pair(mp.padding) == (1, 1)
-                and _pair(mp.dilation) == (1, 1) and not mp.ceil_mode):
-            y = ops.maxpool3x3s2_nhwc(nhwc_view(y), shift=shift).permute(0, 3, 1, 2)
+        pool_ok = (_pair(mp.kernel_size) == (3, 3) and _pair(mp.stride) == (2, 2) and _pair(mp.padding) == (1, 1)
+                   and _pair(mp.dilation) == (1, 1) and not mp.ceil_mode)
+        want_pool = ops.STEM_POOL and pool_ok and enc.conv1.stride == (2, 2)
+        y, pooled = _stem_rows(x, enc.conv1, w, pool_shift=shift if want_pool else None, pool_or_plain=True)
+        if pooled:
+            y = y.permute(0, 3, 1, 2)
         else:
-            y = mp(y)
-            if not y.is_contiguous(memory_format=CL):
-                y = y.contiguous(memory_format=CL)
-            ops.bias_act_nhwc_(y.permute(0, 2, 3, 1), shift, None, N.ACT_RELU)
+            y = y.permute(0, 3, 1, 2) if y is not None else F.conv2d(x.contiguous(memory_format=CL), w, None, enc.conv1.stride, enc.conv1.padding)
+            if y.is_cuda and y.dtype == torch.float32 and y.is_contiguous(memory_format=CL) and y.shape[1] % 4 == 0 and pool_ok:
+                y = ops.maxpool3x3s2_nhwc(nhwc_view(y), shift=shift).permute(0, 3, 1, 2)
+            else:
+                y = mp(y)
+                if not y.is_contiguous(memory_format=CL):
+                    y = y.contiguous(memory_format=CL)
+                ops.bias_act_nhwc_(y.permute(0, 2, 3, 1), shift, None, N.ACT_RELU)
         feats.append(None)
     for layer in (enc.layer1, enc.layer2, enc.layer3, enc.layer4):
         for blk in layer:
diff --git a/adverse_weather_semantic_segmentation_robustness_benchmark_amd/ops.py b/adverse_weather_semantic_segmentation_robustness_benchmark_amd/ops.py
--- a/adverse_weather_semantic_segmentation_robustness_benchmark_amd/ops.py
+++ b/adverse_weather_semantic_segmentation_robustness_benchmark_amd/ops.py
@@ -1435,6 +1435,26 @@
     return out if rc == 0 else None
 
 
+STEM_POOL = os.environ.get("AWSEG_STEM_POOL", "0") != "0"
+
+
+def conv_rows_pool_gemm_split(x_padded: torch.Tensor, w_split: torch.Tensor, shift: torch.Tensor, kernel_h: int, stride: int, pad_y: int,
+                              out_width: int) -> Optional[torch.Tensor]:
+    b, h, wp, pf = x_padded.shape
+    n, k = w_split.shape[1], w_split.shape[2]
+    if k != kernel_h * 32 or not x_padded.is_contiguous():
+        raise N.AwsegError("conv_rows_pool_gemm_split: weights must be [N, kernel_h * 32] and the image contiguous")
+    if not _split_weights_intact(w_split, n, k):
+        raise N.AwsegError("w_split lost its 16-byte trailer (weight exponent): pass the tensor gemm_split_weights returned, not a copy")
+    if shift.shape != (n,) or shift.dtype != torch.float32:
+        raise N.AwsegError("conv_rows_pool_gemm_split: shift must be float32 [N]")
+    ho = (h + 2 * pad_y - kernel_h) // stride + 1
+    out = torch.empty(b, (ho - 1) // 2 + 1, (out_width - 1) // 2 + 1, n, dtype=torch.float32, device=x_padded.device)
+    rc = N.try_call("awseg_conv_rows_pool_gemm_split", N.ptr(x_padded), b, h, wp, pf, kernel_h, stride, pad_y, out_width,
+                    N.ptr(w_split), N.ptr(shift.contiguous()), N.ptr(out), n, N.stream())
+    return out if rc == 0 else None
+
+
 CONV_GATHER = os.environ.get("AWSEG_CONV_GATHER", "1") != "0"
 
 
@@ -1465,20 +1485,24 @@
 
 
 def gemm_split_pieces(pieces, w_split: torch.Tensor, bias: Optional[torch.Tensor], act: int = 0, residual: Optional[torch.Tensor] = None,
-                      out: Optional[torch.Tensor] = None) -> Optional[torch.Tensor]:
+                      out: Optional[torch.Tensor] = None, rows_per_image: int = 0) -> Optional[torch.Tensor]:
     import ctypes
     pieces = [p_.contiguous() for p_ in pieces]
     m, kp = pieces[0].shape
     n = w_split.shape[1]
     if any(p_.shape != (m, kp) for p_ in pieces) or w_split.shape[2] != kp * len(pieces):
         raise N.AwsegError("gemm_split_pieces: the pieces must be equally shaped and the weights [N, pieces * k]")
+    if rows_per_image:
+        if bias is None or rows_per_image < 0 or bias.shape != ((m + rows_per_image - 1) // rows_per_image, n) or bias.dtype != torch.float32:
+            raise N.AwsegError("gemm_split_pieces: a per-image bias must be float32 [ceil(M / rows_per_image), N]")
+        bias = bias.contiguous()
     if not _split_weights_intact(w_split, n, kp * len(pieces)):
         raise N.AwsegError("w_split lost its 16-byte trailer (weight exponent): pass the tensor gemm_split_weights returned, not a copy")
     if out is None:
         out = torch.empty(m, n, dtype=torch.float32, device=pieces[0].device)
     arr = (ctypes.c_void_p * len(pieces))(*[p_.data_ptr() for p_ in pieces])
     rc = N.try_call("awseg_gemm_split_pieces_bias_act", ctypes.cast(arr, ctypes.c_void_p), len(pieces), kp, N.ptr(w_split), N.ptr(bias),
-                    N.ptr(residual), act, N.ptr(out), m, n, N.stream())
+                    N.ptr(residual), act, N.ptr(out), m, n, int(rows_per_image), N.stream())
     return out if rc == 0 else None
 
 
diff --git a/include/awseg.h b/include/awseg.h
--- a/include/awseg.h
+++ b/include/awseg.h
@@ -228,7 +228,8 @@
                                       const float* w2, const float* b2, float* out, awseg_stream_t stream);
 
 int awseg_gemm_split_pieces_bias_act(const float* const* pieces, int n_pieces, int k_piece, const uint16_t* w_split, const float* bias,
-                                     const float* residual, int act, float* out, int64_t m, int n, awseg_stream_t stream);
+                                     const float* residual, int act, float* out, int64_t m, int n, int64_t rows_per_image,
+                                     awseg_stream_t stream);
 
 int awseg_gemm_split_dual_bias_act(const float* x, int k1, const float* x2, int k2, int64_t batch, int x2_height, int x2_width,
                                    int x2_stride, const uint16_t* w_split, const float* bias, const float* residual, int act,
@@ -243,6 +244,10 @@
                                         int kernel_h, int stride, int pad_y, int out_width, const uint16_t* w_split,
                                         const float* bias, const float* residual, int act, float* out, int n,
                                         awseg_stream_t stream);
+
+int awseg_conv_rows_pool_gemm_split(const float* x, int64_t batch, int height, int width_padded, int pixel_floats, int kernel_h,
+                                    int stride, int pad_y, int out_width, const uint16_t* w_split, const float* shift, float* out,
+                                    int n, awseg_stream_t stream);
 
 int64_t awseg_gemm_bf16_weight_halfs(int n, int k);
 int awseg_gemm_bf16_weights(const float* w, int n, int k, uint16_t* w_bf16, awseg_stream_t stream);
@@ -254,6 +259,8 @@
 int awseg_attention_d32_bf16(const float* q, const float* k, const float* v, float* out, int batch, int heads,
                              int n_queries, int n_keys, float scale, awseg_stream_t stream);
 int64_t awseg_attention_d32_split_workspace(int batch, int heads, int n_keys);
+int awseg_attention_d32_kv_image(const float* k, const float* v, int kv_pitch, int batch, int heads, int n_keys, void* workspace,
+                                 int splits, awseg_stream_t stream);
 int awseg_attention_d32_split_ws(const float* q, const float* k, const float* v, int kv_pitch, float* out, int batch, int heads,
                                  int n_queries, int n_keys, float scale, void* workspace, awseg_stream_t stream);
 
```

Result: no change. 233.7, median of 6 (+0.3%).
